# lunarlab-gatech/SLIDE_SLAM

Hardware: AMD Instinct MI355X
Metric: pose-graph updates/sec + ms/Gauss-Newton iter, 8-robot 10k-landmark graph (higher is better)
Workload: dtype f64

## Files before the change

### slide_slam_amd/csrc/capi.hip

```cpp
#include <unistd.h>
#include <algorithm>
#include <cmath>
#include <cstring>
#include <memory>
#include <utility>
#include <vector>

#include "delaunay.hpp"
#include "host_backend.hpp"

using namespace sl;

struct slide_graph {
  HostGraph g;
  explicit slide_graph(const slide_params_t& p) : g(p) {}
};
struct slide_backend {
  HostBackend b;
  slide_graph_t* gview = nullptr;
  explicit slide_backend(const slide_params_t& p) : b(p) {}
};

static thread_local std::string t_err;

// ... 351 lines not shown
  return g->g.dist_pass_local(d_buf);
}

int slide_dense_spd_solve(const double* A, int n, const double* b, double* x, int repeats, double* ms_out) {
  return slide_dense_spd_solve_ex(A, n, b, x, repeats, ms_out, 0);
}
int slide_dense_spd_solve_ex(const double* A, int n, const double* b, double* x, int repeats, double* ms_out, int method) {
  if (slide_device_check(-1) != SLIDE_OK) return SLIDE_ERR_HIP;
  if (n <= 0 || repeats < 1 || method < 0 || method > 2) return SLIDE_ERR_INVALID;
  const int T = (n + NB - 1) / NB;
  const size_t ld = (size_t)(T + 1) * NB, ncol = (size_t)T * NB;
  std::vector<double> S(ld * ncol, 0.0);
  for (int j = 0; j < n; ++j)
    for (int i = j; i < n; ++i) S[(size_t)j * ld + i] = A[(size_t)j * n + i];
  for (size_t i = n; i < ncol; ++i) S[i * ld + i] = 1.0;
  for (int j = 0; j < n; ++j) S[(size_t)j * ld + ncol] = b[j];
  Tmp Tm;
  double* dS0 = Tm.up(S.data(), S.size());
  double* dS = Tm.up<double>(nullptr, S.size());
  double* dW = Tm.up<double>(nullptr, (size_t)T * NB * NB);
  double* dWi = Tm.up<double>(nullptr, (size_t)T * 1024);
  double* dy = Tm.up<double>(nullptr, ncol);
  double* dx = Tm.up<double>(nullptr, ncol);
  int* dst = Tm.up<int>(nullptr, 8);
  int* dctr = Tm.up<int>(nullptr, (size_t)T + 2);
  int* dtick = Tm.up<int>(nullptr, CHOL_STEP_BATCH_MAX);
  if (!dS0 || !dS || !dW || !dWi || !dy || !dx || !dst || !dctr || !dtick) { g_last_error = "hipMalloc/hipMemcpy failed"; return SLIDE_ERR_HIP; }
  SL_HIP(hipMemset(dtick, 0, CHOL_STEP_BATCH_MAX * sizeof(int)));
  SL_HIP(hipMemset(dst, 0, 8 * sizeof(int)));
  SL_HIP(hipMemset(dctr, 0, ((size_t)T + 2) * sizeof(int)));
  hipEvent_t e0, e1;
  SL_HIP(hipEventCreate(&e0));
  SL_HIP(hipEventCreate(&e1));
  float total = 0.f;
  CholSystem cs{};
  cs.S = dS; cs.ld = (int)ld; cs.T = T; cs.Ld = dW; cs.Winv = dWi; cs.yv = dy; cs.dp = dx; cs.status = dst;
  CholLLPlan* plan = method == 1 ? chol_ll_plan_create(&cs, 1) : nullptr;
  if (method == 1 && !plan) { g_last_error = "hipMalloc failed (left-looking plan)"; return SLIDE_ERR_HIP; }
  for (int r = 0; r < repeats; ++r) {
    SL_HIP(hipMemcpyAsync(dS, dS0, S.size() * sizeof(double), hipMemcpyDeviceToDevice, nullptr));
    SL_HIP(hipEventRecord(e0, nullptr));
    if (plan) {
      int* trace = nullptr;
      const int nt = chol_ll_plan_tasks(plan);
      static const bool want_trace = getenv("SLIDE_LL_TRACE") && getenv("SLIDE_LL_TRACE")[0] == '1';
      if (want_trace && hipHostMalloc(reinterpret_cast<void**>(&trace), (size_t)nt * 16 * sizeof(int), hipHostMallocMapped) == hipSuccess)
        memset(trace, 0, (size_t)nt * 16 * sizeof(int));
      launch_chol_ll(plan, &cs, 1, nullptr, trace);
      if (trace) {
        hipEvent_t done;
        SL_HIP(hipEventCreate(&done));
        SL_HIP(hipEventRecord(done, nullptr));
        int waited = 0;
        while (hipEventQuery(done) == hipErrorNotReady && waited < 8000) { usleep(1000); ++waited; }
        if (hipEventQuery(done) == hipErrorNotReady) {
          fprintf(stderr, "k_chol_ll still running after %d ms; tasks (ticket: stage kind k row | barrier-1 waves, barrier-2 waves):\n", waited);
          for (int t = 0; t < nt; ++t)
            if (trace[16 * t] != 5) fprintf(stderr, "  %4d: stage %d kind %d k %d row %d | %03x %03x\n", t, trace[16 * t], trace[16 * t + 1], trace[16 * t + 2], trace[16 * t + 3], trace[16 * t + 4], trace[16 * t + 5]);
          fflush(stderr);
          _exit(3);
        }
        (void)hipEventDestroy(done);
        if (const char* path = getenv("SLIDE_LL_TRACE_FILE")) {
          if (FILE* f = fopen(path, "wb")) { fwrite(trace, sizeof(int), (size_t)nt * 16, f); fclose(f); }
        }
        (void)hipHostFree(trace);
      }
      launch_chol_bwd_all(dS, (int)ld, T, dW, dWi, dy, dx, dst, nullptr, nullptr);
    } else if (method == 2) {
      launch_chol_batch(&cs, 1, dctr, nullptr, nullptr, false, 100, dtick);
      launch_chol_bwd_all(dS, (int)ld, T, dW, dWi, dy, dx, dst, nullptr, nullptr);
    } else {
      chol_factor_solve(dS, (int)ld, T, dW, dWi, dy, dx, dst, dctr, nullptr);
    }
    SL_HIP(hipEventRecord(e1, nullptr));
    SL_HIP(hipEventSynchronize(e1));
    float ms = 0.f;
    SL_HIP(hipEventElapsedTime(&ms, e0, e1));
    total += ms;
  }
  if (plan) { (void)hipDeviceSynchronize(); chol_ll_plan_destroy(plan); }
  SL_HIP(hipGetLastError());
  (void)hipEventDestroy(e0);
  (void)hipEventDestroy(e1);
  int st[8];
  SL_HIP(hipMemcpy(st, dst, sizeof(st), hipMemcpyDeviceToHost));
  std::vector<double> xs(ncol);
  SL_HIP(hipMemcpy(xs.data(), dx, ncol * sizeof(double), hipMemcpyDeviceToHost));
  for (int i = 0; i < n; ++i) x[i] = xs[i];
  if (ms_out) *ms_out = total;
  if (st[1] & 1) { g_last_error = "matrix not positive definite"; return SLIDE_ERR_NOT_SPD; }
  st[0] = 0;
  return decode_status(st);
}

int slide_debug_chol_bordered(const double* S_in, int ld, int T, int nbr, const int* prof, const int* bfirst, const int* ord, int b0, int kofs,
                              int n_copies, int method, double* S_out, double* Ld_out, double* Winv_out, int* status_out, double* max_copy_diff) {
  if (slide_device_check(-1) != SLIDE_OK) return SLIDE_ERR_HIP;
  if (!S_in || T < 1 || nbr < 0 || n_copies < 1 || n_copies > CHOL_STEP_BATCH_MAX || (method != 0 && method != 2)) return SLIDE_ERR_INVALID;
  const int B0 = b0 > 0 ? b0 : T;
  if (ld < (B0 + nbr + 1) * NB) return SLIDE_ERR_INVALID;
  const size_t len = (size_t)ld * T * NB;
  Tmp Tm;
  std::vector<CholSystem> sys(n_copies);
  std::vector<double*> dS(n_copies);
  int* d_ord = ord ? Tm.up(ord, (size_t)nbr) : nullptr;
  int* d_ctr = Tm.up<int>(nullptr, (size_t)T + 3);
  if ((ord && !d_ord) || !d_ctr) { g_last_error = "hipMalloc/hipMemcpy failed"; return SLIDE_ERR_HIP; }
  SL_HIP(hipMemset(d_ctr, 0, ((size_t)T + 3) * sizeof(int)));
  for (int c = 0; c < n_copies; ++c) {
    dS[c] = Tm.up(S_in, len);
    CholSystem cs{};
    cs.S = dS[c]; cs.ld = ld; cs.T = T;
    cs.Ld = Tm.up<double>(nullptr, (size_t)T * NB * NB); cs.Winv = Tm.up<double>(nullptr, (size_t)T * 1024);
    cs.yv = Tm.up<double>(nullptr, (size_t)T * NB); cs.dp = Tm.up<double>(nullptr, (size_t)T * NB);
    cs.status = Tm.up<int>(nullptr, 8);
    if (!cs.S || !cs.Ld || !cs.Winv || !cs.yv || !cs.dp || !cs.status) { g_last_error = "hipMalloc/hipMemcpy failed"; return SLIDE_ERR_HIP; }
    SL_HIP(hipMemset(cs.status, 0, 8 * sizeof(int)));
    SL_HIP(hipMemset(cs.Ld, 0, (size_t)T * NB * NB * sizeof(double)));
    cs.h_prof = prof; cs.nbr = nbr; cs.h_bfirst = bfirst; cs.b0 = b0; cs.kofs = kofs; cs.ord = d_ord;
    sys[c] = cs;
  }
  int* d_tick = Tm.up<int>(nullptr, CHOL_STEP_BATCH_MAX);
  if (!d_tick) { g_last_error = "hipMalloc failed"; return SLIDE_ERR_HIP; }
  SL_HIP(hipMemset(d_tick, 0, CHOL_STEP_BATCH_MAX * sizeof(int)));
  launch_chol_batch(sys.data(), n_copies, d_ctr, nullptr, nullptr, false, 100, method == 2 ? d_tick : nullptr);
  if (method == 2) {
    int tk[CHOL_STEP_BATCH_MAX];
    SL_HIP(hipMemcpy(tk, d_tick, sizeof(tk), hipMemcpyDeviceToHost));
    for (int c = 0; c < CHOL_STEP_BATCH_MAX; ++c)
      if (tk[c] != 0) { g_last_error = "pair kernel: a ticket counter was left at " + std::to_string(tk[c]); return SLIDE_ERR_HIP; }
  }
  SL_HIP(hipDeviceSynchronize());
  SL_HIP(hipGetLastError());
  std::vector<double> ref(len), other;
  SL_HIP(hipMemcpy(ref.data(), dS[0], len * sizeof(double), hipMemcpyDeviceToHost));
  double worst = 0.0;
  for (int c = 1; c < n_copies; ++c) {
    other.resize(len);
    SL_HIP(hipMemcpy(other.data(), dS[c], len * sizeof(double), hipMemcpyDeviceToHost));
    for (size_t i = 0; i < len; ++i) {
      const double d = std::fabs(other[i] - ref[i]);
      if (!(d <= worst)) worst = std::isnan(d) ? (std::isnan(ref[i]) && std::isnan(other[i]) ? worst : INFINITY) : d;
    }
  }
  if (S_out) std::memcpy(S_out, ref.data(), len * sizeof(double));
  if (Ld_out) SL_HIP(hipMemcpy(Ld_out, sys[0].Ld, (size_t)T * NB * NB * sizeof(double), hipMemcpyDeviceToHost));
  if (Winv_out) SL_HIP(hipMemcpy(Winv_out, sys[0].Winv, (size_t)T * 1024 * sizeof(double), hipMemcpyDeviceToHost));
  if (status_out) SL_HIP(hipMemcpy(status_out, sys[0].status, 8 * sizeof(int), hipMemcpyDeviceToHost));
  if (max_copy_diff) *max_copy_diff = worst;
  return SLIDE_OK;
}


static int run_single_class(int cls_kind , int n_cur, const double* det_world, int det_stride,
                            const int32_t* label, int n_map, const float* cloud, const double* model, const int32_t* mlabel,
                            const double* qpos, int K, double thresh, double best_init, int label_gate, int32_t* out_sub,
                            int32_t* out_submap, int* out_k) {
  if (slide_device_check(-1) != SLIDE_OK) return SLIDE_ERR_HIP;
  const bool gate = cloud != nullptr;
  if (!gate && n_cur == 0) return SLIDE_OK;
  Tmp T;
  std::vector<double> det((size_t)std::max(n_cur, 0) * (cls_kind == 0 ? 7 : 12), 0.0);
  for (int i = 0; i < n_cur; ++i) {
    if (cls_kind == 0) std::memcpy(&det[7 * (size_t)i], det_world + (size_t)det_stride * i, 7 * sizeof(double));
    else {
      double* o = &det[12 * (size_t)i];
      o[0] = o[4] = o[8] = 1.0;
      o[9] = det_world[(size_t)det_stride * i]; o[10] = det_world[(size_t)det_stride * i + 1]; o[11] = det_world[(size_t)det_stride * i + 2];
    }
  }
  double pose12[12] = {1, 0, 0, 0, 1, 0, 0, 0, 1, 0, 0, 0};
  if (gate) { pose12[9] = qpos[0]; pose12[10] = qpos[1]; pose12[11] = qpos[2]; }
  AssocFrameDev F[3];
  std::memset(F, 0, sizeof(F));
  AssocFrameDev& C = F[0];
  size_t lds = 0;
  if (!assoc_plan(n_map, K, gate ? 1 : 0, cls_kind == 0 ? 7 : 3, &C.Kp, &C.cached, &C.staged, &lds)) {
    g_last_error = "K-NN gate: K exceeds the on-chip sort buffer (16384 neighbours)";
    return SLIDE_ERR_CAPACITY;
  }
  C.gate = gate ? 1 : 0;
  if (gate) {
    std::vector<float> soa(3 * (size_t)std::max(n_map, 1));
    for (int i = 0; i < n_map; ++i) { soa[i] = cloud[3 * (size_t)i]; soa[(size_t)n_map + i] = cloud[3 * (size_t)i + 1]; soa[2 * (size_t)n_map + i] = cloud[3 * (size_t)i + 2]; }
    const float* d = T.up(soa.data(), soa.size());
    if (!d) { g_last_error = "hipMalloc/hipMemcpy failed"; return SLIDE_ERR_HIP; }
    C.cx = d; C.cy = d + n_map; C.cz = d + 2 * (size_t)n_map;
  }
  C.model = T.up(model, (size_t)(cls_kind == 0 ? 7 : 3) * n_map);
  C.label = T.up(mlabel, n_map);
  C.n = n_map; C.K = K; C.thresh = thresh; C.best_init = best_init; C.label_gate = label_gate; C.is_cyl = cls_kind == 0;
  C.det = T.up(det.data(), det.size());
  C.det_label = T.up(label, n_cur);
  C.n_det = n_cur;
  C.det_world = T.up<double>(nullptr, det.size());
  C.match_sub = T.up<int32_t>(nullptr, n_cur);
  C.match_map = T.up<int32_t>(nullptr, n_cur);
  C.submap = gate ? T.up<int32_t>(nullptr, std::max(std::min(K, n_map), 1)) : nullptr;
  int32_t* nsub = T.up<int32_t>(nullptr, 4);
  C.n_sub = nsub;
  F[1] = C; F[1].n_det = 0; F[1].n = 0; F[1].n_sub = nsub + 1; F[1].submap = nullptr;
  F[2] = C; F[2].n_det = 0; F[2].n = 0; F[2].n_sub = nsub + 2; F[2].submap = nullptr;
  AssocFrameDev* dF = T.up(F, 3);
  double* dpose = T.up(pose12, 12);
  if (!C.model || !C.label || !C.det || !C.det_label || !C.det_world || !C.match_sub || !C.match_map || (gate && !C.submap) ||
      !nsub || !dF || !dpose) {
    g_last_error = "hipMalloc/hipMemcpy failed";
    return SLIDE_ERR_HIP;
  }
  launch_assoc_frame(dF, lds, dpose, nullptr);
  SL_HIP(hipDeviceSynchronize());
  SL_HIP(hipGetLastError());
  int k = 0;
  SL_HIP(hipMemcpy(&k, nsub, sizeof(int), hipMemcpyDeviceToHost));
  if (out_k) *out_k = k;
  if (out_submap && k && gate) SL_HIP(hipMemcpy(out_submap, C.submap, k * sizeof(int32_t), hipMemcpyDeviceToHost));
  if (out_sub && n_cur) SL_HIP(hipMemcpy(out_sub, C.match_sub, n_cur * sizeof(int32_t), hipMemcpyDeviceToHost));
  return SLIDE_OK;
}

int slide_submap_knn(const float* cloud_xyz, uint64_t n, const double query_xyz[3], int K, int32_t* out_idx, int* out_k) {
  if (n > (uint64_t)INT32_MAX || (n > 0 && !cloud_xyz)) return SLIDE_ERR_INVALID;
  if (n == 0) {
    if (slide_device_check(-1) != SLIDE_OK) return SLIDE_ERR_HIP;
    if (out_k) *out_k = 0;
    return SLIDE_OK;
  }
  std::vector<double> model(3 * (size_t)std::max<uint64_t>(n, 1), 0.0);
  std::vector<int32_t> lab(std::max<uint64_t>(n, 1), 0);
  return run_single_class(2, 0, nullptr, 3, nullptr, (int)n, cloud_xyz, model.data(), lab.data(), query_xyz, K, 0.0, 1000.0, 1,
                          nullptr, out_idx, out_k);
}

int slide_assoc_match_cylinders(int n_cur, const double* root, const double* ray, const int32_t* label, int n_map,
                                const double* map_root, const double* map_ray, const int32_t* map_label, double thresh,
                                int32_t* out_idx) {
  std::vector<double> det(7 * (size_t)n_cur), model(7 * (size_t)n_map);
  for (int i = 0; i < n_cur; ++i) { for (int k = 0; k < 3; ++k) { det[7 * i + k] = root[3 * i + k]; det[7 * i + 3 + k] = ray[3 * i + k]; } det[7 * i + 6] = 0; }
  for (int i = 0; i < n_map; ++i) { for (int k = 0; k < 3; ++k) { model[7 * i + k] = map_root[3 * i + k]; model[7 * i + 3 + k] = map_ray[3 * i + k]; } model[7 * i + 6] = 0; }
  const double q[3] = {0, 0, 0};
  return run_single_class(0, n_cur, det.data(), 7, label, n_map, nullptr, model.data(), map_label, q, std::max(n_map, 1), thresh,
                          thresh + 100, 2, out_idx, nullptr, nullptr);
}
int slide_assoc_match_boxes(int cls, int n_cur, const double* xyz, const int32_t* label, int n_map, const double* map_xyz,
                            const int32_t* map_label, double thresh, int32_t* out_idx) {
  if (cls != SLIDE_CLS_CUBE && cls != SLIDE_CLS_ELLIPSOID) return SLIDE_ERR_INVALID;
  const double q[3] = {0, 0, 0};
  const bool cube = cls == SLIDE_CLS_CUBE;
  return run_single_class(cube ? 1 : 2, n_cur, xyz, 3, label, n_map, nullptr, map_xyz, map_label, q, std::max(n_map, 1), thresh,
                          cube ? 30.0 : 1000.0, cube ? 0 : 1, out_idx, nullptr, nullptr);
}

int slide_assoc_sweep_batch_device(const float* d_cloud_x, const float* d_cloud_y, const float* d_cloud_z, const double* d_model_xyz,
                                   const int32_t* d_label, int n_map, const double* d_query_pos, const double* d_obs_xyz,
                                   const int32_t* d_obs_label, int n_query, int n_obs, int K, double thresh, int32_t* d_out_map_idx,
                                   void* stream) {
  if (n_query <= 0) return SLIDE_OK;
  if (n_map < 0 || n_obs < 0 || K <= 0) return SLIDE_ERR_INVALID;
  if (launch_assoc_sweep(d_cloud_x, d_cloud_y, d_cloud_z, d_model_xyz, d_label, n_map, d_query_pos, d_obs_xyz, d_obs_label, n_query,
                         n_obs, K, thresh, d_out_map_idx, (hipStream_t)stream) != 0) {
    g_last_error = "K-NN gate: K exceeds the on-chip sort buffer (16384 neighbours)";
    return SLIDE_ERR_CAPACITY;
  }
  SL_HIP(hipGetLastError());
  return SLIDE_OK;
}

int slide_assoc_sweep_batch(const float* cloud_xyz, const double* model_xyz, const int32_t* label, int n_map, const double* query_pos,
                            const double* obs_xyz, const int32_t* obs_label, int n_query, int n_obs, int K, double thresh,
                            int32_t* out_map_idx, int repeats, double* ms_out) {
  if (slide_device_check(-1) != SLIDE_OK) return SLIDE_ERR_HIP;
  if (n_map < 0 || n_obs < 0 || n_query < 0 || K <= 0) return SLIDE_ERR_INVALID;
  if (ms_out) *ms_out = 0.0;
  if (n_query == 0) return SLIDE_OK;
  Tmp T;
  std::vector<float> soa(3 * (size_t)std::max(n_map, 1));
  for (int i = 0; i < n_map; ++i) { soa[i] = cloud_xyz[3 * (size_t)i]; soa[(size_t)n_map + i] = cloud_xyz[3 * (size_t)i + 1]; soa[2 * (size_t)n_map + i] = cloud_xyz[3 * (size_t)i + 2]; }
  const float* dc = T.up(soa.data(), soa.size());
  const double* dm = T.up(model_xyz, 3 * (size_t)std::max(n_map, 1));
  const int32_t* dl = T.up(label, (size_t)std::max(n_map, 1));
  const double* dq = T.up(query_pos, 3 * (size_t)n_query);
  const double* dox = T.up(obs_xyz, 3 * (size_t)n_query * std::max(n_obs, 1));
  const int32_t* dol = T.up(obs_label, (size_t)n_query * std::max(n_obs, 1));
  int32_t* dout = T.up<int32_t>(nullptr, (size_t)n_query * std::max(n_obs, 1));
  if (!dc || !dm || !dl || !dq || !dox || !dol || !dout) { g_last_error = "hipMalloc/hipMemcpy failed"; return SLIDE_ERR_HIP; }
  hipEvent_t e0, e1;
  SL_HIP(hipEventCreate(&e0));
  SL_HIP(hipEventCreate(&e1));
  int rc = slide_assoc_sweep_batch_device(dc, dc + n_map, dc + 2 * (size_t)n_map, dm, dl, n_map, dq, dox, dol, n_query, n_obs, K, thresh, dout, nullptr);
  if (rc == SLIDE_OK) {
    SL_HIP(hipEventRecord(e0, nullptr));
    for (int r = 0; r < std::max(repeats, 1) && rc == SLIDE_OK; ++r)
      rc = slide_assoc_sweep_batch_device(dc, dc + n_map, dc + 2 * (size_t)n_map, dm, dl, n_map, dq, dox, dol, n_query, n_obs, K, thresh, dout, nullptr);
    SL_HIP(hipEventRecord(e1, nullptr));
    SL_HIP(hipEventSynchronize(e1));
    float ms = 0.f;
    SL_HIP(hipEventElapsedTime(&ms, e0, e1));
    if (ms_out) *ms_out = ms;
  }
  (void)hipEventDestroy(e0);
  (void)hipEventDestroy(e1);
  if (rc != SLIDE_OK) return rc;
  SL_HIP(hipGetLastError());
  if (n_obs) SL_HIP(hipMemcpy(out_map_idx, dout, (size_t)n_query * n_obs * sizeof(int32_t), hipMemcpyDeviceToHost));
  return SLIDE_OK;
// ... 1421 lines not shown
```

### slide_slam_amd/csrc/chol_kernels.hip

```cpp
#include <hip/hip_runtime.h>
#include <stdlib.h>
#include <algorithm>
#include <type_traits>
#include <utility>
#include <vector>

#include "graph_dev.hpp"
#include "kernels.hpp"

namespace sl {

typedef double v4d __attribute__((ext_vector_type(4)));
constexpr int CHOL_BATCH_MAX = 8;
__device__ inline v4d mfma_f64(double a, double b, v4d c) { return __builtin_amdgcn_mfma_f64_16x16x4f64(a, b, c, 0, 0, 0); }

__device__ inline double rsqrt_nr(double d) {
#ifdef SLIDE_RSQRT_OLD
  double y = __builtin_amdgcn_rsq(d);
  y = y * (1.5 - 0.5 * d * y * y);
  y = y * (1.5 - 0.5 * d * y * y);
  return y;
#else
  double y = __builtin_amdgcn_rsq(d);
  double t = d * y, h = 0.5 * y;
// ... 205 lines not shown
      double mop = 0.0;
      mop = s00 ? i0 : mop;  mop = s11 ? i1 : mop;  mop = s10 ? m10 : mop;  mop = s22 ? i2 : mop;  mop = s21 ? m21 : mop;
      mop = s20 ? m20 : mop; mop = s33 ? i3 : mop;  mop = s32 ? m32 : mop;  mop = s31 ? m31 : mop;  mop = s30 ? m30 : mop;
      L.mop[n][lane] = mop;
      const double xd = mfma_f64(mop, Dt[s], zero)[0];
      Dt[s] = xd;
      const double xm = (lr > 4 * s + 3) ? xd : 0.0;
      L.xm[n][lane] = xm;
      lds_post(&L.it_done, n + 1, lane);
      if (n < 4) STAMPW(32 + n);
      if (s < 3) Dt = mfma_f64(-xm, xm, Dt);
      if (s == 3 && JQ < 3) {
        STAMPW(3 + 2 * JQ + 1);
        lds_wait(&L.d_ready[JQ + 1], 1);
        STAMPW(3 + 2 * JQ + 2);
        const double x3 = mfma_f64(mop, L.Dh3[JQ][lane], zero)[0];
#pragma unroll
        for (int r = 0; r < 4; ++r) Dnext[r] = L.Dh[JQ][r][lane];
        Dnext = mfma_f64(-x3, x3, Dnext);
      }
    }
  }
  STAMPW(10);
  if (!ok && lane == 0 && ia == 0) atomicOr(&status[1], 1);
}

template <int W, int NPAN>
__device__ __forceinline__ void a_worker_wave(int ia, double* __restrict__ Ld, double* __restrict__ Winv, ALds& L, int lane,
                                              v4d (&R)[W + 1]) {
  const int lr = lane & 15, lk = lane >> 4;
  const v4d zero = v4d{0.0, 0.0, 0.0, 0.0};
  if (NPAN > 0) {
    v4d e[W + 1];
#pragma unroll
    for (int J = 0; J <= W; ++J) e[J] = zero;
#pragma unroll
    for (int ks = 0; ks < 16 * NPAN; ks += 2) {
      const double w0 = L.Pk[4 * ks + lk][16 * W + lr], w1 = L.Pk[4 * ks + 4 + lk][16 * W + lr];
#pragma unroll
      for (int J = 0; J <= W; ++J) {
        R[J] = mfma_f64(-L.Pk[4 * ks + lk][16 * J + lr], w0, R[J]);
        e[J] = mfma_f64(-L.Pk[4 * ks + 4 + lk][16 * J + lr], w1, e[J]);
      }
    }
#pragma unroll
    for (int J = 0; J <= W; ++J) {
      R[J] += e[J];
      pin(R[J]);
    }
  }
  if (W == 1) STAMPW(37);
  v4d Wt = zero;
#pragma unroll
  for (int JQ = 0; JQ < W; ++JQ) {
    if (W == WT) {
#pragma unroll
      for (int r = 0; r < 4; ++r) Wt[r] = (lr == lk + 4 * r) ? 1.0 : 0.0;
    }
#pragma unroll
    for (int s = 0; s < 4; ++s) {
      const int n = 4 * JQ + s;
      lds_wait(&L.it_done, n + 1);
      if (W == 1 && n == 3) STAMPW(11);
      if (W == 1 && n < 3) STAMPW(16 + n);
      if (W == 2 && n < 12) STAMPW(20 + n);
      const double mop = L.mop[n][lane], xm = L.xm[n][lane];
      const double x = mfma_f64(mop, R[JQ][s], zero)[0];
      double xw = 0.0;
      if (W == WT) xw = mfma_f64(mop, Wt[s], zero)[0];
      R[JQ][s] = x;
      if (W == WT) Wt[s] = xw;
      if (s < 3) {
        R[JQ] = mfma_f64(-xm, x, R[JQ]);
        if (W == WT) Wt = mfma_f64(-xm, xw, Wt);
      }
      R[W] = mfma_f64(-R[JQ][s], R[JQ][s], R[W]);
#pragma unroll
      for (int J = 0; J <= W; ++J) pin(R[J]);
      if (W == WT) pin(Wt);
      if (JQ == W - 1 && s == 2) {
#pragma unroll
        for (int r = 0; r < 4; ++r) L.Dh[W - 1][r][lane] = R[W][r];
        L.Dh3[W - 1][lane] = R[JQ][3];
        lds_post(&L.d_ready[W], 1, lane);
        if (W == 1) STAMPW(13);
        if (W == 2) STAMPW(36);
      }
    }
#pragma unroll
    for (int r = 0; r < 4; ++r) {
      L.Lt[oidx(W, JQ)][r][lane] = R[JQ][r];
      if (ia == 0) Ld[(size_t)(16 * JQ + lk + 4 * r) * NB + 16 * W + lr] = R[JQ][r];
    }
    lds_post(&L.col_done[W], JQ + 1, lane);
    if (W == 1) STAMPW(12);
#pragma unroll
    for (int J = JQ + 1; J < W; ++J) {
      lds_wait(&L.col_done[J], JQ + 1);
#pragma unroll
      for (int ks = 0; ks < 4; ++ks) R[J] = mfma_f64(-L.Lt[oidx(J, JQ)][ks][lane], R[JQ][ks], R[J]);
    }
    if (W == WT) {
#pragma unroll
      for (int r = 0; r < 4; ++r) {
        const double v = (lk + 4 * r >= lr) ? Wt[r] : 0.0;
        L.Wi[JQ][lr * 16 + lk + 4 * r] = v;
        if (ia == 0) Winv[(size_t)JQ * 256 + lr * 16 + lk + 4 * r] = v;
      }
      lds_post(&L.w_done, JQ + 1, lane);
    }
  }
  static_assert(W >= 1 && W <= 3, "worker index");
  if (W == WT) {
#pragma unroll
    for (int JQ = WT; JQ < 4; ++JQ) {
#pragma unroll
      for (int r = 0; r < 4; ++r) Wt[r] = (lr == lk + 4 * r) ? 1.0 : 0.0;
#pragma unroll
      for (int s = 0; s < 4; ++s) {
        const int n = 4 * JQ + s;
        lds_wait(&L.it_done, n + 1);
        const double mop = L.mop[n][lane], xm = L.xm[n][lane];
        const double xw = mfma_f64(mop, Wt[s], zero)[0];
        Wt[s] = xw;
        if (s < 3) Wt = mfma_f64(-xm, xw, Wt);
      }
#pragma unroll
      for (int r = 0; r < 4; ++r) {
        const double v = (lk + 4 * r >= lr) ? Wt[r] : 0.0;
        L.Wi[JQ][lr * 16 + lk + 4 * r] = v;
        if (ia == 0) Winv[(size_t)JQ * 256 + lr * 16 + lk + 4 * r] = v;
      }
      lds_post(&L.w_done, JQ + 1, lane);
    }
  }
}

template <int NPAN>
__device__ __forceinline__ void panel_load(const double* __restrict__ S, int ld, int k, int it, int q, int lr, int lk,
                                           v4d (&Tq)[4], double (&tb)[16]) {
  const double* tcol = S + (size_t)(k * NB) * ld + (size_t)it * NB + 16 * q + lr;
#pragma unroll
  for (int b = 0; b < 4; ++b)
#pragma unroll
    for (int r = 0; r < 4; ++r) Tq[b][r] = tcol[(size_t)(16 * b + lk + 4 * r) * ld];
  if (NPAN > 0) {
    const double* pi = S + (size_t)((k - NPAN) * NB) * ld + (size_t)it * NB + 16 * q + lr;
#pragma unroll
    for (int ks = 0; ks < 16 * NPAN; ++ks) tb[ks] = pi[(size_t)(4 * ks + lk) * ld];
  }
}
template <int NPAN, bool EARLY>
__device__ __forceinline__ void panel_rows(double* __restrict__ S, int ld, int k, int it, int q, int gate, int lane, ALds& L, v4d (&Tq)[4],
                                           const double (&tb)[16], float* __restrict__ L32t) {
  const int lr = lane & 15, lk = lane >> 4;
  double* tcol = S + (size_t)(k * NB) * ld + (size_t)it * NB + 16 * q + lr;
  float* pcol = L32t ? L32t + lk * NB + 16 * q + lr : nullptr;
  v4d xt[4], t[4];
#define PANEL_YIELD() do { __builtin_amdgcn_sched_barrier(0); __builtin_amdgcn_s_sleep(1); __builtin_amdgcn_sched_barrier(0); } while (0)
#pragma unroll
  for (int b = 0; b < 4; ++b) {
    if (b == 0) {
      if (NPAN > 0 && EARLY) {
        if (gate == 1) lds_wait(&L.d_ready[1], 1);
        if (gate == 2) lds_wait(&L.d_ready[2], 1);
#pragma unroll
        for (int ks = 0; ks < 16 * NPAN; ++ks) {
#pragma unroll
          for (int bb = 0; bb < 4; ++bb) Tq[bb] = mfma_f64(-L.Pk[4 * ks + lk][16 * bb + lr], tb[ks], Tq[bb]);
        }
#pragma unroll
        for (int bb = 0; bb < 4; ++bb) pin(Tq[bb]);
      }
      lds_wait(&L.it_done, 4);
      if (NPAN > 0 && !EARLY) {
#pragma unroll
        for (int ks = 0; ks < 16 * NPAN; ++ks) {
          Tq[0] = mfma_f64(-L.Pk[4 * ks + lk][lr], tb[ks], Tq[0]);
          if ((ks & 3) == 3) PANEL_YIELD();
        }
      }
      t[0] = Tq[0];
    }
    lds_wait(&L.w_done, b + 1);
    v4d x = v4d{0.0, 0.0, 0.0, 0.0};
#pragma unroll
    for (int s4 = 0; s4 < 4; ++s4) x = mfma_f64(L.Wi[b][(4 * s4 + lk) * 16 + lr], t[b][s4], x);
    xt[b] = x;
#pragma unroll
    for (int r = 0; r < 4; ++r) tcol[(size_t)(16 * b + lk + 4 * r) * ld] = x[r];
    if (pcol) {
#pragma unroll
      for (int r = 0; r < 4; ++r) pcol[(16 * b + 4 * r) * NB] = (float)x[r];
    }
    if (b < 3) {
      PANEL_YIELD();
      if (NPAN > 0 && !EARLY) {
#pragma unroll
        for (int ks = 0; ks < 16 * NPAN; ++ks) {
          Tq[b + 1] = mfma_f64(-L.Pk[4 * ks + lk][16 * (b + 1) + lr], tb[ks], Tq[b + 1]);
          if ((ks & 3) == 3) PANEL_YIELD();
        }
      }
      lds_wait(&L.col_done[b + 1], b + 1);
      v4d tn = Tq[b + 1];
#pragma unroll
      for (int c = 0; c <= b; ++c) {
#pragma unroll
        for (int s4 = 0; s4 < 4; ++s4) tn = mfma_f64(-L.Lt[oidx(b + 1, c)][s4][lane], xt[c][s4], tn);
        if (b < 2 || c < b) PANEL_YIELD();
      }
      t[b + 1] = tn;
      pin(t[b + 1]);
    }
  }
#undef PANEL_YIELD
}

template <int NPAN>
__device__ __forceinline__ void step_type_a_impl(double* __restrict__ S, int ld, int k, int ia, int it, int half, double* __restrict__ Ld,
                                                 double* __restrict__ Winv, int* status, ALds& L, float* __restrict__ L32t) {
  const int tid = threadIdx.x, lane = tid & 63;
  const int wave = __builtin_amdgcn_readfirstlane(tid >> 6);
  const int lr = lane & 15, lk = lane >> 4;
  STAMP(0);
  if (NPAN > 0) {
    constexpr int NC = 8 * (NPAN > 0 ? NPAN : 1);
    const double* pq = S + (size_t)((k - NPAN) * NB + NC * wave) * ld + (size_t)k * NB + lane;
    double stage[NC];
#pragma unroll
    for (int c = 0; c < NC; ++c) stage[c] = pq[(size_t)c * ld];
#pragma unroll
    for (int c = 0; c < NC; ++c) L.Pk[NC * wave + c][lane] = stage[c];
  }
  if (tid == 0) L.it_done = 0;
  if (tid < 4) { L.col_done[tid] = 0; L.d_ready[tid] = 0; }
  if (tid == 4) L.w_done = 0;
  if (wave == 1) STAMPW(38);
  if (wave < 4) {
    const double* dcol = S + (size_t)(k * NB) * ld + (size_t)k * NB + 16 * wave + lr;
    v4d R[4];
#pragma unroll
    for (int J = 0; J < 4; ++J)
#pragma unroll
      for (int r = 0; r < 4; ++r) R[J][r] = (J <= wave) ? dcol[(size_t)(16 * J + lk + 4 * r) * ld] : 0.0;
    v4d Tq[4];
    double tb[16];
    if (wave == 1 && half < 0) panel_load<NPAN>(S, ld, k, it, 0, lr, lk, Tq, tb);
    __syncthreads();
    if (wave == 1) STAMPW(39);
    if (wave == 0) __builtin_amdgcn_s_setprio(3); else __builtin_amdgcn_s_setprio(2);
    if (wave == 0) {
      a_chain_wave<NPAN>(ia, status, L, lane, R[0]);
    } else if (wave == 1) {
      v4d R1[2] = {R[0], R[1]};
      a_worker_wave<1, NPAN>(ia, Ld, Winv, L, lane, R1);
      if (half < 0) panel_rows<NPAN, false>(S, ld, k, it, 0, 0, lane, L, Tq, tb, L32t);
    } else if (wave == 2) {
      v4d R2[3] = {R[0], R[1], R[2]};
      a_worker_wave<2, NPAN>(ia, Ld, Winv, L, lane, R2);
    } else {
      a_worker_wave<3, NPAN>(ia, Ld, Winv, L, lane, R);
    }
    __builtin_amdgcn_s_setprio(0);
    __syncthreads();
    STAMP(1);
    STAMP(2);
  } else {
    const int q = half < 0 ? wave - 4 : (wave == 5 ? 2 * half : (wave == 6 ? 2 * half + 1 : -1));
    const bool rows = half < 0 ? q > 0 : q >= 0;
    v4d Tq[4];
    double tb[16];
    if (rows) panel_load<NPAN>(S, ld, k, it, q, lr, lk, Tq, tb);
    __syncthreads();
    if (rows) panel_rows<NPAN, true>(S, ld, k, it, q, wave - 4, lane, L, Tq, tb, L32t);
    STAMPW(14);
    __syncthreads();
    STAMP(1);
    STAMP(2);
  }
}
__device__ __forceinline__ void step_type_a(double* __restrict__ S, int ld, int k, int T, int TvA, int ia, int half, double* __restrict__ Ld,
                                            double* __restrict__ Winv, int* status, ALds& L, float* __restrict__ L32, int nbr, int nbA,
                                            const int* __restrict__ ord = nullptr) {
  const int vi = k + 1 + ia - TvA;
  const int it = vi < 0 ? k + 1 + ia : (vi < nbA ? T + (ord ? ord[vi] : vi) : T + nbr);
  float* L32t = (L32 && it < T) ? L32 + ((size_t)k * (T - 1) - (size_t)k * (k - 1) / 2 + (it - k - 1)) * (NB * NB) : nullptr;
  if (k > 0) step_type_a_impl<1>(S, ld, k, ia, it, half, Ld, Winv, status, L, L32t);
  else step_type_a_impl<0>(S, ld, k, ia, it, half, Ld, Winv, status, L, L32t);
}

__global__ __launch_bounds__(512) void k_chol_step(double* __restrict__ S, int ld, int k, int T, double* __restrict__ Ld,
                                                   double* __restrict__ Winv, int* status, int* __restrict__ ctr, int kb, int nP,
                                                   int g0, int g1, int nX, int a_joins, int a_split, float* __restrict__ L32,
                                                   int TvA, int TvB, int TvX, int nbr, int nbA, int nbB, int nbX) {
  __shared__ ALds L;
  __shared__ int s_g;
  const int nA = (TvA - k + nbA) << a_split;
  if (blockIdx.x == 0 && threadIdx.x == 0) ctr[k + 1] = 0;
  if ((int)blockIdx.x < nA) {
    step_type_a(S, ld, k, T, TvA, (int)blockIdx.x >> a_split, a_split ? (int)(blockIdx.x & 1) : -1, Ld, Winv, status, L, L32, nbr, nbA);
    if (!a_joins) return;
  }
  const int nR = g1 - g0, nItems = nR + nX;
  if (nItems <= 0) return;
  const long long nG = (long long)nP * (nP + 1) / 2;
  const int wave = __builtin_amdgcn_readfirstlane(threadIdx.x >> 6);
  for (;;) {
    __syncthreads();
    if (threadIdx.x == 0) s_g = atomicAdd(&ctr[k], 1);
    __syncthreads();
    const int g = __builtin_amdgcn_readfirstlane(s_g);
    if (g >= nItems) break;
    const BItem it = b_decode(g, nItems, nR, g0, k, kb, T, TvB, TvX, nP, nG, wave, nbr, nbB, nbX);
    if (!it.ok) continue;
    if (it.ks == 32) b_quadrant<32>(S, ld, it, wave & 3);
    else b_quadrant<16>(S, ld, it, wave & 3);
  }
}

struct CholBatchArgs {
  int n;
  double* S[CHOL_STEP_BATCH_MAX]; int ld[CHOL_STEP_BATCH_MAX]; int T[CHOL_STEP_BATCH_MAX];
  double* Ld[CHOL_STEP_BATCH_MAX]; double* Winv[CHOL_STEP_BATCH_MAX]; int* status[CHOL_STEP_BATCH_MAX];
  float* L32[CHOL_STEP_BATCH_MAX];
  int TvA[CHOL_STEP_BATCH_MAX], TvB[CHOL_STEP_BATCH_MAX], TvX[CHOL_STEP_BATCH_MAX];
  int nP[CHOL_STEP_BATCH_MAX], g0[CHOL_STEP_BATCH_MAX], g1[CHOL_STEP_BATCH_MAX], nX[CHOL_STEP_BATCH_MAX], a_split[CHOL_STEP_BATCH_MAX];
  int nbr[CHOL_STEP_BATCH_MAX];
  int nbA[CHOL_STEP_BATCH_MAX], nbB[CHOL_STEP_BATCH_MAX], nbX[CHOL_STEP_BATCH_MAX];
  int B0[CHOL_STEP_BATCH_MAX];
  const int* ord[CHOL_STEP_BATCH_MAX];
  int a_base[CHOL_STEP_BATCH_MAX + 1];
  int b_base[CHOL_STEP_BATCH_MAX + 1];
};
__device__ __forceinline__ int xcd_logical(int orig, int nwg) {
  const int q = nwg >> 3, r = nwg & 7, xcd = orig & 7;
  return (xcd < r ? xcd * (q + 1) : r * (q + 1) + (xcd - r) * q) + (orig >> 3);
}
__global__ __launch_bounds__(512) void k_chol_step_batched(CholBatchArgs A, int k, int kb, int* __restrict__ ctr, int a_joins, int xcd_map) {
  __shared__ ALds L;
  __shared__ int s_g;
  if (blockIdx.x == 0 && threadIdx.x == 0) ctr[k + 1] = 0;
  int bid = (int)blockIdx.x;
  if (xcd_map && bid < A.a_base[A.n]) bid = xcd_logical(bid, A.a_base[A.n]);
  if (bid < A.a_base[A.n]) {
    int r = 0;
    while (bid >= A.a_base[r + 1]) ++r;
    const int local = bid - A.a_base[r], sp = A.a_split[r];
    step_type_a(A.S[r], A.ld[r], k, A.B0[r], A.TvA[r], local >> sp, sp ? (local & 1) : -1, A.Ld[r] + (size_t)k * NB * NB,
                A.Winv[r] + (size_t)k * 1024, A.status[r], L, A.L32[r], A.nbr[r], A.nbA[r], A.ord[r]);
    if (!a_joins) return;
  }
  const int nItems = A.b_base[A.n];
  if (nItems <= 0) return;
  const int wave = __builtin_amdgcn_readfirstlane(threadIdx.x >> 6);
  for (;;) {
    __syncthreads();
    if (threadIdx.x == 0) s_g = atomicAdd(&ctr[k], 1);
    __syncthreads();
    const int g = __builtin_amdgcn_readfirstlane(s_g);
    if (g >= nItems) break;
    int r = 0;
    while (g >= A.b_base[r + 1]) ++r;
    const int gl = g - A.b_base[r], nR = A.g1[r] - A.g0[r];
    const long long nG = (long long)A.nP[r] * (A.nP[r] + 1) / 2;
    const BItem it = b_decode(gl, nR + A.nX[r], nR, A.g0[r], k, kb, A.B0[r], A.TvB[r], A.TvX[r], A.nP[r], nG, wave, A.nbr[r], A.nbB[r], A.nbX[r], A.ord[r]);
    if (!it.ok) continue;
    if (it.ks == 32) b_quadrant<32>(A.S[r], A.ld[r], it, wave & 3);
    else b_quadrant<16>(A.S[r], A.ld[r], it, wave & 3);
  }
}


constexpr int PAIR_THREADS = 768;
struct PLds {
  double Pk[2 * NB][PSTR];
  double Xs[16][4][64];
  double mop[16][64];
  double xm[16][64];
  double Lt[6][4][64];
  double Dh[3][4][64];
  double Dh3[3][64];
  double Wi[4][256];
  int it_done;
  int col_done[4];
  int d_ready[4];
  int w_done;
  int pend_done;
  int p1_done;
  int xs_done[4];
  int d2_ready[4];
  int sub_loaded;
  int store_flag;
};
__device__ int g_pair_timeouts;
__device__ __forceinline__ void lds_wait_p(int* f, int v) {
  const unsigned off = (unsigned)(size_t)f;
  int cur;
  for (int spin = 0; spin < (1 << 21); ++spin) {
    asm volatile("ds_read_b32 %0, %1\n\ts_waitcnt lgkmcnt(0)" : "=v"(cur) : "v"(off) : "memory");
    if (__builtin_amdgcn_readfirstlane(cur) >= v) return;
    __builtin_amdgcn_s_sleep(1);
  }
  if ((threadIdx.x & 63) == 0) atomicAdd(&g_pair_timeouts, 1);
}
__device__ __forceinline__ void lds_add1(int* f, int lane) {
  const unsigned off = (unsigned)(size_t)f;
  const int one = 1;
  __atomic_signal_fence(__ATOMIC_SEQ_CST);
  if (lane == 0) asm volatile("ds_add_u32 %0, %1" : : "v"(off), "v"(one) : "memory");
  __atomic_signal_fence(__ATOMIC_SEQ_CST);
}
__device__ __forceinline__ constexpr int didx(int I, int J) { return I * (I + 1) / 2 + J; }
typedef double (*D2Ptr)[4][64];
__device__ __forceinline__ double ldu(const double* ubase, unsigned boff) {
  asm("" : "+s"(ubase));
  return *reinterpret_cast<const double*>(reinterpret_cast<const char*>(ubase) + boff);
}
__device__ __forceinline__ void stu(double* ubase, unsigned boff, double v) {
  asm("" : "+s"(ubase));
  *reinterpret_cast<double*>(reinterpret_cast<char*>(ubase) + boff) = v;
}
__device__ __forceinline__ D2Ptr pair_d2(PLds& L) { return reinterpret_cast<D2Ptr>(&L.Pk[0][0]); }

template <int NPAN, int PH>
__device__ __forceinline__ void p_chain_wave(bool report, int* status, PLds& L, int lane, v4d Dt) {
  const int lr = lane & 15, lk = lane >> 4;
  const v4d zero = v4d{0.0, 0.0, 0.0, 0.0};
  const bool s00 = lr == 0 && lk == 0, s10 = lr == 1 && lk == 0, s11 = lr == 1 && lk == 1, s20 = lr == 2 && lk == 0,
             s21 = lr == 2 && lk == 1, s22 = lr == 2 && lk == 2, s30 = lr == 3 && lk == 0, s31 = lr == 3 && lk == 1,
             s32 = lr == 3 && lk == 2, s33 = lr == 3 && lk == 3;
  if (NPAN > 0) {
    v4d d1 = zero, d2 = zero, d3 = zero;
#pragma unroll
    for (int ks = 0; ks < 4 * NPAN; ++ks) {
      const double q0 = L.Pk[4 * ks + lk][lr], q1 = L.Pk[16 * NPAN + 4 * ks + lk][lr], q2 = L.Pk[32 * NPAN + 4 * ks + lk][lr],
                   q3 = L.Pk[48 * NPAN + 4 * ks + lk][lr];
      Dt = mfma_f64(-q0, q0, Dt);
      d1 = mfma_f64(-q1, q1, d1);
      d2 = mfma_f64(-q2, q2, d2);
      d3 = mfma_f64(-q3, q3, d3);
    }
    Dt = (Dt + d1) + (d2 + d3);
  }
  if (PH == 0) lds_add1(&L.pend_done, lane);
  bool ok = true;
  v4d Dnext = zero;
#pragma unroll
  for (int JQ = 0; JQ < 4; ++JQ) {
    if (JQ > 0) Dt = Dnext;
#pragma unroll
    for (int r = 0; r < 4; ++r)
      if (lr < lk + 4 * r) Dt[r] = 0.0;
#pragma unroll
    for (int s = 0; s < 4; ++s) {
      const int n = 4 * JQ + s;
      const double dv = Dt[s];
      const double P00 = bcast_lane(dv, 4 * s), P10 = bcast_lane(dv, 4 * s + 1), P20 = bcast_lane(dv, 4 * s + 2), P30 = bcast_lane(dv, 4 * s + 3);
      const double P11 = bcast_lane(dv, 4 * s + 1 + 16), P21 = bcast_lane(dv, 4 * s + 2 + 16), P31 = bcast_lane(dv, 4 * s + 3 + 16);
      const double P22 = bcast_lane(dv, 4 * s + 2 + 32), P32 = bcast_lane(dv, 4 * s + 3 + 32), P33 = bcast_lane(dv, 4 * s + 3 + 48);
      const double i0 = rsqrt_nr(P00);
      const double l10 = P10 * i0, l20 = P20 * i0, l30 = P30 * i0;
      const double d1 = P11 - l10 * l10;
      const double i1 = rsqrt_nr(d1);
      const double l21 = (P21 - l20 * l10) * i1, l31 = (P31 - l30 * l10) * i1;
      const double d2 = P22 - l20 * l20 - l21 * l21;
      const double i2 = rsqrt_nr(d2);
      const double l32 = (P32 - l30 * l20 - l31 * l21) * i2;
      const double d3 = P33 - l30 * l30 - l31 * l31 - l32 * l32;
      const double i3 = rsqrt_nr(d3);
      ok = ok && (P00 > 0.0) && (d1 > 0.0) && (d2 > 0.0) && (d3 > 0.0);
      const double m10 = -l10 * i0 * i1;
      const double m21 = -l21 * i1 * i2;
      const double m20 = -(l20 * i0 + l21 * m10) * i2;
      const double m32 = -l32 * i2 * i3;
      const double m31 = -(l31 * i1 + l32 * m21) * i3;
      const double m30 = -(l30 * i0 + l31 * m10 + l32 * m20) * i3;
      double mop = 0.0;
      mop = s00 ? i0 : mop;  mop = s11 ? i1 : mop;  mop = s10 ? m10 : mop;  mop = s22 ? i2 : mop;  mop = s21 ? m21 : mop;
      mop = s20 ? m20 : mop; mop = s33 ? i3 : mop;  mop = s32 ? m32 : mop;  mop = s31 ? m31 : mop;  mop = s30 ? m30 : mop;
      L.mop[n][lane] = mop;
      const double xd = mfma_f64(mop, Dt[s], zero)[0];
      Dt[s] = xd;
      const double xm = (lr > 4 * s + 3) ? xd : 0.0;
      L.xm[n][lane] = xm;
      lds_post(&L.it_done, 16 * PH + n + 1, lane);
      if (s < 3) Dt = mfma_f64(-xm, xm, Dt);
      if (s == 3 && JQ < 3) {
        lds_wait_p(&L.d_ready[JQ + 1], PH + 1);
        const double x3 = mfma_f64(mop, L.Dh3[JQ][lane], zero)[0];
#pragma unroll
        for (int r = 0; r < 4; ++r) Dnext[r] = L.Dh[JQ][r][lane];
        Dnext = mfma_f64(-x3, x3, Dnext);
      }
    }
  }
  if (!ok && lane == 0 && report) atomicOr(&status[1], 1);
}

template <int W, int NPAN, int PH>
__device__ __forceinline__ void p_worker_wave(bool store, double* __restrict__ Ld, double* __restrict__ Winv, PLds& L, int lane,
                                              v4d (&R)[W + 1], int nread) {
  const int lr = lane & 15, lk = lane >> 4;
// ... 903 lines not shown
      if (wave == 0) {
        ll_wait_cols(fk, nullptr, fr, k - 1, k, ctl, Y.status);
        ll_time(tr, 14);
      }
      __syncthreads();
      constexpr int NC = 8;
      const double* pq = S + (size_t)((k - 1) * NB + NC * wave) * ld + (size_t)k * NB + lane;
      double stage[NC];
#pragma unroll
      for (int c = 0; c < NC; ++c) stage[c] = pq[(size_t)c * ld];
#pragma unroll
      for (int c = 0; c < NC; ++c) L.Pk[NC * wave + c][lane] = stage[c];
    }
    ll_mark_or(tr, 4, 1 << wave);
    __syncthreads();
    if (wave == 0) ll_stage(tr, 3);
    if (wave == 0) __builtin_amdgcn_s_setprio(3); else __builtin_amdgcn_s_setprio(2);
    if (wave == 0) {
      a_chain_wave<NPAN>(ia, Y.status, L, lane, R[0]);
    } else if (wave == 1) {
      v4d R1[2] = {R[0], R[1]};
      ll_worker_wave<1, NPAN>(ia, Ld, Winv, L, lane, R1);
      if (NPAN > 0) {
        if (row_prev) lds_wait(&row_ok, 1);
        const double* pi = S + (size_t)((k - 1) * NB) * ld + (size_t)it * NB + lr;
#pragma unroll
        for (int ks = 0; ks < 16; ++ks) tb[ks] = row_prev ? pi[(size_t)(4 * ks + lk) * ld] : 0.0;
      }
      ll_panel_rows<NPAN, false>(S, ld, k, it, 0, 0, lane, L, Tq, tb, nullptr);
    } else if (wave == 2) {
      v4d R2[3] = {R[0], R[1], R[2]};
      ll_worker_wave<2, NPAN>(ia, Ld, Winv, L, lane, R2);
    } else {
      ll_worker_wave<3, NPAN>(ia, Ld, Winv, L, lane, R);
    }
    __builtin_amdgcn_s_setprio(0);
    __builtin_amdgcn_fence(__ATOMIC_RELEASE, "agent");
    ll_mark_or(tr, 5, 1 << wave);
    __syncthreads();
    if (wave == 0) ll_stage(tr, 4);
  } else {
    const int q = wave - 4;
    const bool rows = q > 0;
    v4d Tq[4];
    double tb[16];
    if (rows) ll_rows_load(S, ld, k, it, q, lr, lk, Tq);
    if (tk.clo_d < kold) {
      v4d Rdummy[4];
      __syncthreads();
      ll_chain_presum(S, ld, k, it, tk.clo_d, tk.clo0, kold, L, wave, lane, false, 0, rows, q, Rdummy, Tq);
    }
    if (NPAN > 0) {
      __syncthreads();
      constexpr int NC = 8;
      const double* pq = S + (size_t)((k - 1) * NB + NC * wave) * ld + (size_t)k * NB + lane;
      double stage[NC];
#pragma unroll
      for (int c = 0; c < NC; ++c) stage[c] = pq[(size_t)c * ld];
#pragma unroll
      for (int c = 0; c < NC; ++c) L.Pk[NC * wave + c][lane] = stage[c];
    }
    ll_mark_or(tr, 4, 1 << wave);
    __syncthreads();
    if (NPAN > 0 && row_prev && wave == 4) {
      ll_wait_cols(fi, nullptr, fr, k - 1, k, ctl, Y.status);
      lds_post(&row_ok, 1, lane);
    }
    if (NPAN > 0 && rows) {
      if (row_prev) lds_wait(&row_ok, 1);
      const double* pi = S + (size_t)((k - 1) * NB) * ld + (size_t)it * NB + 16 * q + lr;
#pragma unroll
      for (int ks = 0; ks < 16; ++ks) tb[ks] = row_prev ? pi[(size_t)(4 * ks + lk) * ld] : 0.0;
    }
    if (rows) ll_panel_rows<NPAN, true>(S, ld, k, it, q, wave - 4, lane, L, Tq, tb, nullptr);
    __builtin_amdgcn_fence(__ATOMIC_RELEASE, "agent");
    ll_mark_or(tr, 5, 1 << wave);
    __syncthreads();
  }
  if (tid == 0) {
    if (ia == 0) __hip_atomic_store(Y.flags + (size_t)k * fr + k, 1, __ATOMIC_RELAXED, __HIP_MEMORY_SCOPE_AGENT);
    __hip_atomic_store(Y.flags + (size_t)k * fr + it, 1, __ATOMIC_RELAXED, __HIP_MEMORY_SCOPE_AGENT);
  }
  if (wave == 0) ll_stage(tr, 5);
}

__global__ __launch_bounds__(512) void k_chol_ll(const LLSys* __restrict__ sysv, const LLTask* __restrict__ tasks, int n_tasks, int* ctl, int* trace) {
  __shared__ ALds L;
  __shared__ int s_t, s_row_ok;
  if (threadIdx.x == 0) s_t = atomicAdd(&ctl[0], 1);
  __syncthreads();
  const int t = __builtin_amdgcn_readfirstlane(s_t);
  if (t >= n_tasks) return;
  const LLTask tk = tasks[t];
  const LLSys Y = sysv[tk.sys];
  int* tr = trace ? trace + 16 * (size_t)t : nullptr;
  if (tr && threadIdx.x == 0) { ll_mark(tr, 1, tk.kind); ll_mark(tr, 2, tk.k); ll_mark(tr, 3, tk.it0); ll_stage(tr, 1); }
  if (tk.kind != 1) {
    if (tk.clo_d <= tk.k - 1) ll_chain_task<1>(Y, tk, L, s_row_ok, ctl, tr);
    else ll_chain_task<0>(Y, tk, L, s_row_ok, ctl, tr);
  } else {
    ll_tile_task(Y, tk, L, ctl, tr);
  }
}

extern "C" int slide_debug_pair_timeouts() {
  int v = -1;
  if (hipMemcpyFromSymbol(&v, HIP_SYMBOL(g_pair_timeouts), sizeof(int)) != hipSuccess) return -1;
  return v;
}
#ifdef SLIDE_STAMPS
extern "C" void slide_debug_stamps(unsigned long long* out) { (void)hipMemcpyFromSymbol(out, HIP_SYMBOL(g_stamps), sizeof(g_stamps)); }
extern "C" void slide_debug_chain_stamps(unsigned long long* out) { (void)hipMemcpyFromSymbol(out, HIP_SYMBOL(g_chain_stamps), sizeof(g_chain_stamps)); }
#endif

constexpr unsigned long long BWD_SENT = CHAIN_SENTINEL;

__global__ void k_chol_extract_y(const double* __restrict__ S, int ld, int T, int Tr, double* __restrict__ yv, double* __restrict__ dp, int* status,
                                 double* __restrict__ prev) {
  const int c = blockIdx.x * blockDim.x + threadIdx.x;
  if (c == 0) status[4] = 0;
  if (c < T * NB) {
    yv[c] = S[(size_t)c * ld + (size_t)Tr * NB];
    if (prev) prev[c] = dp[c];
    dp[c] = __longlong_as_double((long long)BWD_SENT);
  }
}

struct ExtractArgs { int n; const double* S[CHOL_STEP_BATCH_MAX]; int ld[CHOL_STEP_BATCH_MAX]; int T[CHOL_STEP_BATCH_MAX]; int Tr[CHOL_STEP_BATCH_MAX]; double* yv[CHOL_STEP_BATCH_MAX]; double* dp[CHOL_STEP_BATCH_MAX]; int* status[CHOL_STEP_BATCH_MAX]; };
__global__ void k_chol_extract_y_b(ExtractArgs A) {
  const int r = blockIdx.y;
  const int c = blockIdx.x * blockDim.x + threadIdx.x;
  if (c == 0) A.status[r][4] = 0;
  if (c < A.T[r] * NB) {
    A.yv[r][c] = A.S[r][(size_t)c * A.ld[r] + (size_t)A.Tr[r] * NB];
    A.dp[r][c] = __longlong_as_double((long long)BWD_SENT);
  }
}

constexpr int CHAIN_THREADS = 320;
struct alignas(16) ChainLds {
  alignas(16) double xs[2][NB];
  alignas(16) double ys[NB];
  alignas(16) double red[4][NB];
  alignas(16) double Lo[6][256];
  alignas(16) double Ws[4][256];
  alignas(16) double tmp[3][256];
  alignas(16) double Ms[NB][NB + 1];
};
template <bool F32, bool WFIRE = false>
__device__ __forceinline__ void bwd_chain_body(ChainLds& W, const double* __restrict__ S, int ld, int T, const double* __restrict__ Ld,
                                               const double* __restrict__ Winv, const double* __restrict__ yv, double* dp, int* status, int bidx,
                                               const float* __restrict__ L32, const int* __restrict__ prof,
                                               const double* __restrict__ wf_prev = nullptr, double wf_thr = 0.0, int wf_Tprev = 0,
                                               int* wf_lds = nullptr, int wf_lim = 0) {
  int dummy_state = 0;
  int& wf_state = WFIRE ? *wf_lds : dummy_state;
  auto& Ms = W.Ms; auto& Lo = W.Lo; auto& Ws = W.Ws; auto& tmp = W.tmp; auto& xs = W.xs; auto& ys = W.ys;
  const int tid = threadIdx.x;
  const bool worker = tid < 256;
  CSTAMP(0);
  const int c = T - 1 - bidx;
  if (WFIRE) {
    if (tid == 0) wf_state = 0;
    __syncthreads();
  }
  const int col = tid >> 2, part = tid & 3;
  const int jtop = prof ? prof[c] : T - 1;
  const int nj = jtop - c;
  constexpr int RB = F32 ? 6 : 3;
  typedef typename std::conditional<F32, float, double>::type tile_t;
  tile_t tr[RB][16];
  const double* tcol = S + (size_t)(c * NB + col) * ld + 16 * part;
  const float* pcol = F32 ? L32 + ((size_t)c * (T - 1) - (size_t)c * (c - 1) / 2) * (NB * NB) + col * NB + 16 * part : nullptr;
  auto tile_load = [&](tile_t (&dst)[16], int q) {
    if (F32) {
      const float4* tp = reinterpret_cast<const float4*>(pcol + (size_t)(nj - 1 - q) * (NB * NB));
#pragma unroll
      for (int r = 0; r < 4; ++r) {
        const float4 v = tp[r];
        dst[4 * r] = v.x; dst[4 * r + 1] = v.y; dst[4 * r + 2] = v.z; dst[4 * r + 3] = v.w;
      }
    } else {
      const double* tp = tcol + (size_t)(jtop - q) * NB;
#pragma unroll
      for (int r = 0; r < 16; ++r) dst[r] = tp[r];
    }
  };
  double y0 = 0.0;
  if (worker) {
#pragma unroll
    for (int q = 0; q < RB; ++q)
      if (q < nj) tile_load(tr[q], q);
    y0 = yv[c * NB + col];
  }
  if (worker) {
    const double* Ldk = Ld + (size_t)c * NB * NB;
    const double* Wk = Winv + (size_t)c * 1024;
#pragma unroll
    for (int b = 1; b < 4; ++b)
#pragma unroll
      for (int a = 0; a < b; ++a) Lo[b * (b - 1) / 2 + a][tid] = Ldk[(size_t)(16 * a + (tid >> 4)) * NB + 16 * b + (tid & 15)];
#pragma unroll
    for (int b = 0; b < 4; ++b) Ws[b][tid] = Wk[(size_t)b * 256 + tid];
  }
  __syncthreads();
  {
    const int r = tid & 15, cc = (tid >> 4) & 15;
    if (worker) {
#pragma unroll
      for (int b = 0; b < 4; ++b) Ms[16 * b + r][16 * b + cc] = Ws[b][cc * 16 + r];
    }
    __syncthreads();
#pragma unroll
    for (int d = 1; d < 4; ++d) {
#pragma unroll
      for (int a = 0; a + d < 4; ++a) {
        const int b = a + d;
        double t = 0.0;
#pragma unroll
        for (int m = a; m < b; ++m)
#pragma unroll
          for (int n = 0; n < 16; ++n) t += Lo[b * (b - 1) / 2 + m][n * 16 + r] * Ms[16 * m + n][16 * a + cc];
        if (worker) tmp[a][cc * 16 + r] = t;
      }
      __syncthreads();
#pragma unroll
      for (int a = 0; a + d < 4; ++a) {
        const int b = a + d;
        double v = 0.0;
#pragma unroll
        for (int n = 0; n < 16; ++n) v += Ws[b][n * 16 + r] * tmp[a][cc * 16 + n];
        if (worker) Ms[16 * b + r][16 * a + cc] = -v;
      }
      __syncthreads();
    }
  }
  double mreg[16];
#pragma unroll
  for (int r = 0; r < 16; ++r) mreg[r] = (worker && 16 * part + r >= col) ? Ms[16 * part + r][col] : 0.0;
  double acc = 0.0;
  bool wf_quiet = WFIRE && nj > 0 && c < wf_lim;
  bool wf_leave = false;
  CSTAMP(1);
  for (int q0 = 0; q0 < nj && !wf_leave; q0 += RB) {
#pragma unroll
    for (int qq = 0; qq < RB; ++qq) {
      const int q = q0 + qq;
      if (q < nj && !wf_leave) {
        const int j = jtop - q;
        if (q == nj - 1) CSTAMPP(2);
        if (!worker) {
          const int lane = tid - 256;
          double v;
          int spins = 0;
          bool stopped = false;
          for (;;) {
            v = __hip_atomic_load(dp + (size_t)j * NB + lane, __ATOMIC_RELAXED, __HIP_MEMORY_SCOPE_AGENT);
            if ((unsigned long long)__double_as_longlong(v) != BWD_SENT) break;
            if (WFIRE && (spins & 3) == 3 && __hip_atomic_load(status + 7, __ATOMIC_RELAXED, __HIP_MEMORY_SCOPE_AGENT) > c) { stopped = true; break; }
            if (++spins > (1 << 21)) {
              v = __builtin_nan("");
              atomicOr(&status[1], 2);
              break;
            }
            __builtin_amdgcn_s_sleep(1);
          }
          if (WFIRE) {
            stopped = __any(stopped);
            if (stopped) {
              if (lane == 0) wf_state = 1;
            } else {
              double dv = fabs(v - ((j < wf_Tprev) ? wf_prev[(size_t)j * NB + lane] : 1e300));
#pragma unroll
              for (int m = 32; m >= 1; m >>= 1) dv = fmax(dv, __shfl_xor(dv, m));
              wf_quiet = wf_quiet && (dv < wf_thr);
              if (q == nj - 1 && wf_quiet && lane == 0) wf_state = 2;
            }
          }
          xs[q & 1][lane] = v;
          if (q == nj - 1) CSTAMPP(3);
          if (q == nj - 2) CSTAMPP(7);
        }
        __syncthreads();
        if (WFIRE && wf_state == 1) { wf_leave = true; continue; }
        if (worker) {
#pragma unroll
          for (int r = 0; r < 16; ++r) acc += (double)tr[qq][r] * xs[q & 1][16 * part + r];
          if (q + RB < nj) tile_load(tr[qq], q + RB);
        }
      }
    }
  }
  CSTAMP(4);
  if (WFIRE && wf_state != 0) {
    if (tid < NB) __hip_atomic_store(dp + (size_t)c * NB + tid, wf_prev[(size_t)c * NB + tid], __ATOMIC_RELAXED, __HIP_MEMORY_SCOPE_AGENT);
    if (tid == 0) {
      if (wf_state == 2) atomicMax(status + 7, c);
      atomicAdd(status + 3, 1);
    }
    return;
  }
  acc += __shfl_xor(acc, 1);
  acc += __shfl_xor(acc, 2);
  if (worker && part == 0) ys[col] = y0 - acc;
  __syncthreads();
  CSTAMP(5);
  double x = 0.0;
#pragma unroll
  for (int r = 0; r < 16; ++r) x += mreg[r] * ys[16 * part + r];
  x += __shfl_xor(x, 1);
  x += __shfl_xor(x, 2);
  if (worker && part == 0) __hip_atomic_store(dp + (size_t)c * NB + col, x, __ATOMIC_RELAXED, __HIP_MEMORY_SCOPE_AGENT);
  CSTAMP(6);
}
__device__ __forceinline__ int bwd_ticket(int* ctr) {
  __shared__ int s_t;
  if (threadIdx.x == 0) s_t = atomicAdd(ctr, 1);
  __syncthreads();
  const int t = s_t;
  __syncthreads();
  return t;
}
__global__ __launch_bounds__(CHAIN_THREADS) void k_chol_bwd_chain(const double* __restrict__ S, int ld, int T, const double* __restrict__ Ld,
                                                        const double* __restrict__ Winv, const double* __restrict__ yv, double* dp, int* status,
                                                        const int* __restrict__ prof) {
  __shared__ ChainLds W;
  const int t = bwd_ticket(&status[4]);
  if (t >= T) return;
  bwd_chain_body<false>(W, S, ld, T, Ld, Winv, yv, dp, status, t, nullptr, prof);
}
__global__ __launch_bounds__(CHAIN_THREADS) void k_chol_bwd_chain_wf(const double* __restrict__ S, int ld, int T, const double* __restrict__ Ld,
                                                           const double* __restrict__ Winv, const double* __restrict__ yv, double* dp, int* status,
                                                           const int* __restrict__ prof, const double* __restrict__ prev, double thr, int Tprev, int lim) {
  __shared__ ChainLds W;
  __shared__ int s_wf;
  const int t = bwd_ticket(&status[4]);
  if (t >= T) return;
  bwd_chain_body<false, true>(W, S, ld, T, Ld, Winv, yv, dp, status, t, nullptr, prof, prev, thr, Tprev, &s_wf, lim);
}
constexpr int BWD_BATCH_MAX = 32;
struct BwdBatchArgs {
  int n;
  const double* S[BWD_BATCH_MAX]; int ld[BWD_BATCH_MAX]; int T[BWD_BATCH_MAX];
  const double* Ld[BWD_BATCH_MAX]; const double* Winv[BWD_BATCH_MAX]; const double* yv[BWD_BATCH_MAX]; double* dp[BWD_BATCH_MAX];
  int* status[BWD_BATCH_MAX];
  const int* prof[BWD_BATCH_MAX];
  int base[BWD_BATCH_MAX + 1];
  int Tmax;
};
__global__ __launch_bounds__(CHAIN_THREADS) void k_chol_bwd_chain_batched(BwdBatchArgs A) {
  __shared__ ChainLds W;
  for (;;) {
    const int t = bwd_ticket(&A.status[0][4]);
    if (t >= A.n * A.Tmax) return;
    const int r = t % A.n, b = t / A.n;
    if (b >= A.T[r]) continue;
    bwd_chain_body<false>(W, A.S[r], A.ld[r], A.T[r], A.Ld[r], A.Winv[r], A.yv[r], A.dp[r], A.status[r], b, nullptr, A.prof[r]);
    return;
  }
}


enum { TAB_MF = 0, TAB_MB = 1, TAB_PF = 2, TAB_PB = 3 };
struct ChainTabArgs {
  int n; int T[CHOL_BATCH_MAX]; const double* S[CHOL_BATCH_MAX]; int ld[CHOL_BATCH_MAX];
  const double* Ld[CHOL_BATCH_MAX]; const double* Winv[CHOL_BATCH_MAX]; const int* prof[CHOL_BATCH_MAX]; double* ctab[CHOL_BATCH_MAX];
};
__global__ __launch_bounds__(256) void k_chain_tables(ChainTabArgs A) {
  __shared__ ChainLds W;
  __shared__ double Ts[NB][NB];
  auto& Ms = W.Ms; auto& Lo = W.Lo; auto& Ws = W.Ws; auto& tmp = W.tmp;
  const int sys = blockIdx.y, c = blockIdx.x, tid = threadIdx.x;
  const int T = A.T[sys];
  if (c >= T) return;
  {
    const double* Ldk = A.Ld[sys] + (size_t)c * NB * NB;
    const double* Wk = A.Winv[sys] + (size_t)c * 1024;
#pragma unroll
    for (int b = 1; b < 4; ++b)
#pragma unroll
      for (int a = 0; a < b; ++a) Lo[b * (b - 1) / 2 + a][tid] = Ldk[(size_t)(16 * a + (tid >> 4)) * NB + 16 * b + (tid & 15)];
#pragma unroll
    for (int b = 0; b < 4; ++b) Ws[b][tid] = Wk[(size_t)b * 256 + tid];
  }
  for (int e = tid; e < NB * (NB + 1); e += 256) (&Ms[0][0])[e] = 0.0;
  __syncthreads();
  {
    const int r = tid & 15, cc = tid >> 4;
#pragma unroll
    for (int b = 0; b < 4; ++b) Ms[16 * b + r][16 * b + cc] = Ws[b][cc * 16 + r];
    __syncthreads();
#pragma unroll
    for (int d = 1; d < 4; ++d) {
#pragma unroll
      for (int a = 0; a + d < 4; ++a) {
        const int b = a + d;
        double t = 0.0;
#pragma unroll
        for (int m = a; m < b; ++m)
#pragma unroll
          for (int n = 0; n < 16; ++n) t += Lo[b * (b - 1) / 2 + m][n * 16 + r] * Ms[16 * m + n][16 * a + cc];
        tmp[a][cc * 16 + r] = t;
      }
      __syncthreads();
#pragma unroll
      for (int a = 0; a + d < 4; ++a) {
        const int b = a + d;
        double v = 0.0;
#pragma unroll
        for (int n = 0; n < 16; ++n) v += Ws[b][n * 16 + r] * tmp[a][cc * 16 + n];
        Ms[16 * b + r][16 * a + cc] = -v;
      }
      __syncthreads();
    }
  }
  const int i = tid >> 2, part = tid & 3;
  double* tab = A.ctab[sys] + (size_t)c * (NB * NB) + (size_t)tid * 16;
  const size_t tstride = (size_t)T * (NB * NB);
#pragma unroll
  for (int k = 0; k < 16; ++k) tab[TAB_MF * tstride + k] = Ms[i][16 * part + k];
#pragma unroll
  for (int r = 0; r < 16; ++r) tab[TAB_MB * tstride + r] = Ms[16 * part + r][i];
  const int ld = A.ld[sys];
  const int* prof = A.prof[sys];
  {
    double pf[16];
#pragma unroll
    for (int k = 0; k < 16; ++k) pf[k] = 0.0;
    const bool have = c >= 1 && (prof ? prof[c - 1] >= c : true);
    if (have) {
      const double* tp = A.S[sys] + (size_t)((c - 1) * NB) * ld + (size_t)c * NB;
      for (int e = tid; e < NB * NB; e += 256) Ts[e >> 6][e & 63] = tp[(size_t)(e >> 6) * ld + (e & 63)];
    }
    __syncthreads();
    if (have) {
      for (int m = 0; m <= i; ++m) {
        const double a = Ms[i][m];
#pragma unroll
        for (int k = 0; k < 16; ++k) pf[k] += a * Ts[16 * part + k][m];
      }
    }
#pragma unroll
    for (int k = 0; k < 16; ++k) tab[TAB_PF * tstride + k] = pf[k];
    __syncthreads();
  }
  {
    double pb[16];
#pragma unroll
    for (int r = 0; r < 16; ++r) pb[r] = 0.0;
    const bool have = c + 1 < T && (prof ? prof[c] >= c + 1 : true);
    if (have) {
      const double* tp = A.S[sys] + (size_t)(c * NB) * ld + (size_t)(c + 1) * NB;
      for (int e = tid; e < NB * NB; e += 256) Ts[e >> 6][e & 63] = tp[(size_t)(e >> 6) * ld + (e & 63)];
    }
    __syncthreads();
    if (have) {
      for (int m = i; m < NB; ++m) {
        const double a = Ms[m][i];
#pragma unroll
        for (int r = 0; r < 16; ++r) pb[r] += Ts[m][16 * part + r] * a;
      }
    }
#pragma unroll
    for (int r = 0; r < 16; ++r) tab[TAB_PB * tstride + r] = pb[r];
  }
}

struct alignas(16) TabLds {
  alignas(16) double xs[2][NB];
  alignas(16) double ys[NB];
  alignas(16) double red[4][NB];
};
template <bool FWD, bool F32>
__device__ __forceinline__ void tab_chain_body(TabLds& W, const double* __restrict__ S, int ld, int T, const float* __restrict__ L32,
                                               const double* __restrict__ ctab, const double* __restrict__ rin, double* xout, int* status, int c,
                                               const int* __restrict__ prof, const int* __restrict__ first, double* __restrict__ next_out) {
  auto& xs = W.xs; auto& ys = W.ys; auto& red = W.red;
  const int tid = threadIdx.x;
  const bool worker = tid < 256;
  if (next_out && !worker) next_out[(size_t)c * NB + (tid - 256)] = __longlong_as_double((long long)BWD_SENT);
  const int i = (tid >> 2) & 63, part = tid & 3;
  const int row = tid & 63, cp = (tid >> 6) & 3;
  const int jlo = FWD ? (first ? first[c] : 0) : c + 1;
  const int jhi = FWD ? c - 1 : (prof ? prof[c] : T - 1);
  const int nj = jhi - jlo + 1;
  const bool has_p = nj >= 1;
  const int nloop = has_p ? nj - 1 : 0;
  constexpr int RB = F32 ? 6 : 3;
  typedef typename std::conditional<F32, float, double>::type tile_t;
  tile_t tr[RB][16];
  auto tile_load = [&](tile_t (&dst)[16], int q) {
    const int j = FWD ? jlo + q : jhi - q;
    if (FWD) {
      if (F32) {
        const float* tp = L32 + ((size_t)j * (T - 1) - (size_t)j * (j - 1) / 2 + (c - j - 1)) * (NB * NB) + 16 * cp * NB + row;
#pragma unroll
        for (int r = 0; r < 16; ++r) dst[r] = tp[r * NB];
      } else {
        const double* tp = S + (size_t)(j * NB + 16 * cp) * ld + (size_t)c * NB + row;
#pragma unroll
        for (int r = 0; r < 16; ++r) dst[r] = tp[(size_t)r * ld];
      }
    } else {
      if (F32) {
        const float4* tp = reinterpret_cast<const float4*>(L32 + ((size_t)c * (T - 1) - (size_t)c * (c - 1) / 2 + (j - c - 1)) * (NB * NB) + i * NB + 16 * part);
#pragma unroll
        for (int r = 0; r < 4; ++r) {
          const float4 v = tp[r];
          dst[4 * r] = v.x; dst[4 * r + 1] = v.y; dst[4 * r + 2] = v.z; dst[4 * r + 3] = v.w;
        }
// ... 299 lines not shown
  const double *lpj = pj0, *lpi = pi0;
  v2d pa[RD], pb[RD];
  auto issue = [&](v2d& ra, v2d& rb) {
    while (rem == 0 && sg_next < nseg) {
      int a0 = c0, a1 = c1;
      if (st) {
        const int* sf = st + 1 + nseg + sg_next * (nbr + 1);
        a0 = max(sf[ib], sf[jb]);
        a1 = st[1 + sg_next];
      }
      ++sg_next;
      if (a0 < a1) {
        rem = (a1 - a0) * 16;
        lpj = pj0 + (size_t)a0 * NB * ld;
        lpi = pi0 + (size_t)a0 * NB * ld;
      }
    }
    ra = *(const v2d*)lpj;
    rb = *(const v2d*)lpi;
    lpj += (size_t)4 * ld;
    lpi += (size_t)4 * ld;
    --rem;
    ++issued;
  };
#pragma unroll
  for (int pre = 0; pre < RD - 1; ++pre)
    if (issued < total) issue(pa[pre], pb[pre]);
  v4d acc[2][2];
#pragma unroll
  for (int a = 0; a < 2; ++a)
#pragma unroll
    for (int e = 0; e < 4; ++e) {
      v2d c2;
      c2[0] = 0.0; c2[1] = 0.0;
      if (q == 0) c2 = *(const v2d*)(cin + (size_t)(8 * e + a) * ldin);
      acc[a][0][e] = c2[0]; acc[a][1][e] = c2[1];
    }
  for (int ks0 = 0; ks0 < total; ks0 += RD) {
#pragma unroll
    for (int u = 0; u < RD; ++u) {
      if (issued < total) issue(pa[(u + RD - 1) % RD], pb[(u + RD - 1) % RD]);
      __builtin_amdgcn_sched_barrier(0);
#pragma unroll
      for (int a = 0; a < 2; ++a) {
        const double na = -pa[u][a];
#pragma unroll
        for (int b = 0; b < 2; ++b) acc[a][b] = mfma_f64(na, pb[u][b], acc[a][b]);
      }
      __builtin_amdgcn_sched_barrier(0);
    }
  }
#pragma unroll
  for (int a = 0; a < 2; ++a)
#pragma unroll
    for (int e = 0; e < 4; ++e) {
      v2d c2;
      c2[0] = acc[a][0][e]; c2[1] = acc[a][1][e];
      *(v2d*)(cbh + (size_t)(8 * e + a) * ldb) = c2;
    }
}
__global__ __launch_bounds__(256) void k_border_syrk(SyrkArgs A) { border_syrk_body<16>(A); }
__global__ __launch_bounds__(256) void k_border_syrk_rd8(SyrkArgs A) { border_syrk_body<8>(A); }
__global__ __launch_bounds__(256) void k_border_syrk_rd4(SyrkArgs A) { border_syrk_body<4>(A); }
static void launch_syrk_kernel(dim3 grid, size_t lds, hipStream_t s, const SyrkArgs& A) {
  static const int rd = getenv("SLIDE_SYRK_RD") ? atoi(getenv("SLIDE_SYRK_RD")) : 16;
  if (rd == 4) hipLaunchKernelGGL(k_border_syrk_rd4, grid, dim3(256), lds, s, A);
  else if (rd == 8) hipLaunchKernelGGL(k_border_syrk_rd8, grid, dim3(256), lds, s, A);
  else hipLaunchKernelGGL(k_border_syrk, grid, dim3(256), lds, s, A);
}
__global__ __launch_bounds__(256) void k_border_syrk_reduce(double* __restrict__ bord, int ldb, int nbr, int ks, const double* __restrict__ scratch,
                                                            const int* __restrict__ bfirst, int T) {
  const int ib = blockIdx.x >> 4, jb = blockIdx.y;
  if (ib > nbr || jb >= nbr || ib < jb) return;
  int c0 = 0;
  if (bfirst) c0 = max(bfirst[ib], bfirst[jb]);
  const int len = (T - c0 + ks - 1) / ks;
  const int e = (blockIdx.x & 15) * 256 + threadIdx.x;
  const int col = e / NB, row = e - col * NB;
  double* dst = bord + (size_t)(jb * NB + col) * ldb + (size_t)ib * NB + row;
  double v = *dst;
  for (int q = 1; q < ks; ++q)
    if (c0 + q * len < T) v += scratch[((size_t)(jb * (nbr + 1) + ib) * (ks - 1) + (q - 1)) * (NB * NB) + (size_t)col * NB + row];
  *dst = v;
}
__global__ __launch_bounds__(256) void k_border_syrk_reduce2(double* __restrict__ bordA, int ldbA, const double* __restrict__ bordB, int ldbB, int nbr,
                                                             int ksA, int ksB, const double* __restrict__ scratchA, const double* __restrict__ scratchB,
                                                             int TA, int TB) {
  const int ib = blockIdx.x >> 4, jb = blockIdx.y;
  if (ib > nbr || jb >= nbr || ib < jb) return;
  const int e = (blockIdx.x & 15) * 256 + threadIdx.x;
  const int col = e / NB, row = e - col * NB;
  double* dst = bordA + (size_t)(jb * NB + col) * ldbA + (size_t)ib * NB + row;
  double va = *dst, vb = bordB[(size_t)(jb * NB + col) * ldbB + (size_t)ib * NB + row];
  const int lenA = (TA + ksA - 1) / ksA, lenB = (TB + ksB - 1) / ksB;
  for (int q = 1; q < ksA; ++q)
    if (q * lenA < TA) va += scratchA[((size_t)(jb * (nbr + 1) + ib) * (ksA - 1) + (q - 1)) * (NB * NB) + (size_t)col * NB + row];
  for (int q = 1; q < ksB; ++q)
    if (q * lenB < TB) vb += scratchB[((size_t)(jb * (nbr + 1) + ib) * (ksB - 1) + (q - 1)) * (NB * NB) + (size_t)col * NB + row];
  *dst = va + vb;
}
void launch_border_syrk(const CholSystem* d, int n, hipStream_t s, double* scratch, int ks) {
  SyrkArgs A{};
  A.n = n;
  int nb = 0;
  for (int i = 0; i < n; ++i) {
    A.S[i] = d[i].S; A.ld[i] = d[i].ld; A.T[i] = d[i].T; A.nbr[i] = d[i].nbr; A.bord[i] = d[i].bord; A.ldb[i] = d[i].ldb; A.bfirst[i] = d[i].bfirst; A.bsrc[i] = d[i].bord_src;
    A.segtab[i] = d[i].segtab; A.b0[i] = d[i].b0 > 0 ? d[i].b0 : d[i].T;
    nb = d[i].nbr > nb ? d[i].nbr : nb;
  }
  if (nb <= 0) return;
  if (scratch && n == 1 && ks > 1) {
    A.ks = ks; A.scratch = scratch;
    launch_syrk_kernel(dim3(nb + 1, nb, ks), 0, s, A);
    hipLaunchKernelGGL(k_border_syrk_reduce, dim3(16 * (nb + 1), nb), dim3(256), 0, s, d[0].bord, d[0].ldb, d[0].nbr, ks, scratch, d[0].bfirst, d[0].T);
    return;
  }
  A.ks = 1; A.scratch = nullptr;
  launch_syrk_kernel(dim3(nb + 1, nb, n), 0, s, A);
}
void launch_border_syrk_jobs(const CholSystem* d, int n, const int* jobs, int njobs, int lds_pad, hipStream_t s, double* scratch, int ks, int jb_end,
                             const int* ks_sys, bool fuse_add) {
  SyrkArgs A{};
  A.n = n;
  for (int i = 0; i < n; ++i) {
    A.S[i] = d[i].S; A.ld[i] = d[i].ld; A.T[i] = d[i].T; A.nbr[i] = d[i].nbr; A.bord[i] = d[i].bord; A.ldb[i] = d[i].ldb; A.bfirst[i] = d[i].bfirst; A.bsrc[i] = d[i].bord_src;
    A.segtab[i] = d[i].segtab; A.b0[i] = d[i].b0 > 0 ? d[i].b0 : d[i].T;
  }
  if (njobs <= 0) return;
  A.ks = 1; A.scratch = nullptr; A.jobs = jobs;
  if (scratch && n == 2 && fuse_add && d[0].nbr == d[1].nbr && !d[0].bfirst && !d[1].bfirst) {
    const int nb = d[0].nbr;
    const int ka = std::max(1, ks_sys ? ks_sys[0] : ks), kb = std::max(1, ks_sys ? ks_sys[1] : ks), km = std::max(ka, kb);
    A.ks = km; A.scratch = scratch; A.scratch_stride = std::max<size_t>(1, (size_t)(nb + 1) * nb * (km - 1) * NB * NB);
    A.ks_sys[0] = ka; A.ks_sys[1] = kb;
    launch_syrk_kernel(dim3(njobs, 1, km), lds_pad, s, A);
    hipLaunchKernelGGL(k_border_syrk_reduce2, dim3(16 * (nb + 1), jb_end >= 0 ? jb_end : nb), dim3(256), 0, s, d[0].bord, d[0].ldb, d[1].bord, d[1].ldb, nb,
                       ka, kb, scratch, scratch + A.scratch_stride, d[0].T, d[1].T);
    return;
  }
  if (scratch && n == 1 && ks > 1) {
    A.ks = ks; A.scratch = scratch;
    launch_syrk_kernel(dim3(njobs, 1, ks), lds_pad, s, A);
    const int nb = d[0].nbr;
    hipLaunchKernelGGL(k_border_syrk_reduce, dim3(16 * (nb + 1), jb_end >= 0 ? jb_end : nb), dim3(256), 0, s, d[0].bord, d[0].ldb, nb, ks, scratch, d[0].bfirst, d[0].T);
    return;
  }
  launch_syrk_kernel(dim3(njobs), lds_pad, s, A);
}
struct BorderApplyArgs {
  int n;
  const double* S[CHOL_BATCH_MAX]; int ld[CHOL_BATCH_MAX]; int T[CHOL_BATCH_MAX]; int nbr[CHOL_BATCH_MAX]; int b0[CHOL_BATCH_MAX];
  double* yv[CHOL_BATCH_MAX]; const double* x[CHOL_BATCH_MAX];
  const int* segtab[CHOL_BATCH_MAX];
};
__global__ __launch_bounds__(256) void k_border_apply(BorderApplyArgs A) {
  const int r = blockIdx.z;
  const int col = blockIdx.x * 4 + (threadIdx.x >> 6), lane = threadIdx.x & 63;
  if (col >= A.T[r] * NB) return;
  const int nrow = A.nbr[r] * NB;
  const double* w = A.S[r] + (size_t)col * A.ld[r] + (size_t)A.b0[r] * NB;
  const double* x = A.x[r];
  double acc = 0.0;
  const int* st = A.segtab[r];
  const int* msk = st ? st + 1 + st[0] + st[0] * (A.nbr[r] + 1) : nullptr;
  if (msk && msk[0] > 0) {
    const int c = col / NB;
    unsigned long long m = (unsigned long long)(unsigned)msk[1 + 2 * c] | ((unsigned long long)(unsigned)msk[2 + 2 * c] << 32);
    while (m) {
      const int t = __ffsll((long long)m) - 1;
      m &= m - 1;
      acc += w[t * NB + lane] * x[t * NB + lane];
    }
  } else {
    for (int q = lane; q < nrow; q += 64) acc += w[q] * x[q];
  }
#pragma unroll
  for (int m = 32; m >= 1; m >>= 1) acc += __shfl_xor(acc, m);
  if (lane == 0) A.yv[r][col] -= acc;
}
void launch_border_apply(const CholSystem* d, int n, const double* const* xloc, hipStream_t s) {
  BorderApplyArgs A{};
  A.n = n;
  int Tmax = 0;
  for (int i = 0; i < n; ++i) {
    A.S[i] = d[i].S; A.ld[i] = d[i].ld; A.T[i] = d[i].T; A.nbr[i] = d[i].nbr; A.yv[i] = d[i].yv; A.x[i] = xloc[i];
    A.b0[i] = d[i].b0 > 0 ? d[i].b0 : d[i].T;
    A.segtab[i] = d[i].segtab;
    Tmax = d[i].T > Tmax ? d[i].T : Tmax;
  }
  if (Tmax > 0) hipLaunchKernelGGL(k_border_apply, dim3(Tmax * NB / 4, 1, n), dim3(256), 0, s, A);
}

void launch_chol_bwd_all(const double* S, int ld, int T, const double* Ld, const double* Winv, double* yv, double* dp,
                         int* status, const int* prof, hipStream_t s, const double* wf_prev, double wf_thr, int wf_Tprev, int wf_lim);
void launch_chol_extract_y(const double* S, int ld, int T, double* yv, double* dp, int* status, hipStream_t s, int nbr, int b0, double* prev) {
  hipLaunchKernelGGL(k_chol_extract_y, dim3((T * NB + 255) / 256), dim3(256), 0, s, S, ld, T, (b0 > 0 ? b0 : T) + nbr, yv, dp, status, prev);
}
struct StepPlan { int kb, nP, g0, g1, nX, TvA, TvB, TvX, nbA, nbB, nbX; long long nA, nB; };
static int chol_n_cu() {
  static int n_cu = 0;
  if (!n_cu) {
    int dev = 0;
    hipDeviceProp_t pr;
    if (hipGetDevice(&dev) == hipSuccess && hipGetDeviceProperties(&pr, dev) == hipSuccess) n_cu = pr.multiProcessorCount;
    if (n_cu <= 0) n_cu = 256;
  }
  return n_cu;
}
static StepPlan plan_step(int k, int T, const int* prof, int nbr = 0, const int* bfirst = nullptr, int kofs = 0) {
  static const double frac = getenv("SLIDE_CHOL_FRAC") ? atof(getenv("SLIDE_CHOL_FRAC")) : 0.5;
  StepPlan p{};
  p.kb = k & ~1;
  p.TvA = p.TvB = p.TvX = T;
  if (prof && k < T) {
    p.TvA = prof[k] + 1;
    if (p.kb >= 1) p.TvB = prof[p.kb - 1] + 1;
    if (k >= 1) p.TvX = prof[k - 1] + 1;
  }
  auto active = [&](int upto) { int c = 0; while (c < nbr && (!bfirst || bfirst[c] <= upto + kofs)) ++c; return c; };
  p.nbA = active(k); p.nbB = active(p.kb - 1); p.nbX = active(k - 1);
  p.nA = k < T ? p.TvA - k + p.nbA : 0;
  if (k >= 2 && k < T) {
    p.nP = p.TvB + p.nbB > p.kb ? (p.TvB + p.nbB - p.kb + 1) / 2 : 0;
    long long nG = (long long)p.nP * (p.nP + 1) / 2;
    if (nbr > 0) {
      const int ncol = p.TvB - 1 >= p.kb + 1 ? (p.TvB - 2 - p.kb) / 2 + 1 : 0;
      long long nv = 0;
      for (int bj = 0; bj < ncol && bj < p.nP; ++bj) nv += p.nP - bj;
      nG = nv;
    }
    long long first = (long long)(frac * (double)nG + 0.5);
    if (first < p.nP) first = p.nP;
    if (first > nG) first = nG;
    if (k & 1) { p.g0 = (int)(2 * first); p.g1 = (int)(2 * nG); } else { p.g0 = 0; p.g1 = (int)(2 * first); }
  }
  p.nX = (k & 1) && k + 1 < p.TvX ? (p.TvX + p.nbX - k + 1) / 2 : 0;
  p.nB = p.g1 - p.g0 + p.nX;
  return p;
}
void launch_chol_step(double* S, int ld, int k, int T, double* Ld, double* Winv, int* status, int* ctr, float* L32, const int* h_prof,
                      hipStream_t s, int nbr) {
  const int n_cu = chol_n_cu();
  const StepPlan p = plan_step(k, T, h_prof, nbr, nullptr);
  const long long nA = p.nA, nB = p.nB;
  static const int split_pct = getenv("SLIDE_CHOL_ASPLIT") ? atoi(getenv("SLIDE_CHOL_ASPLIT")) : 100;
  const int a_split = (k > 0 && (2 * nA + nB) * 100 <= (long long)n_cu * split_pct) ? 1 : 0;
  const long long nAw = nA << a_split;
  const long long extra = nB < n_cu ? nB : n_cu;
  const long long free_cu = n_cu - nAw > 8 ? n_cu - nAw : 8;
  static const int join_mul = getenv("SLIDE_CHOL_JOIN") ? atoi(getenv("SLIDE_CHOL_JOIN")) : 1;
  const int a_joins = nB > join_mul * free_cu ? 1 : 0;
  hipLaunchKernelGGL(k_chol_step, dim3((unsigned)(nAw + extra)), dim3(512), 0, s, S, ld, k, T, Ld, Winv, status, ctr, p.kb, p.nP,
                     p.g0, p.g1, p.nX, a_joins, a_split, L32, p.TvA, p.TvB, p.TvX, nbr, p.nbA, p.nbB, p.nbX);
}
struct PairPlan { int ncols, Tv0, Tv1, nb0, nb1, TvB, nbB, nP; long long nA, nB; };
static PairPlan plan_pair(int k, int T, const int* prof, int nbr, const int* bfirst, int kofs) {
  PairPlan p{};
  p.ncols = T - k >= 2 ? 2 : (T - k == 1 ? 1 : 0);
  if (p.ncols == 0) return p;
  auto active = [&](int upto) { int c = 0; while (c < nbr && (!bfirst || bfirst[c] <= upto + kofs)) ++c; return c; };
  p.Tv0 = prof ? prof[k] + 1 : T;
  p.Tv1 = p.ncols == 2 ? (prof ? prof[k + 1] + 1 : T) : p.Tv0;
  p.nb0 = active(k);
  p.nb1 = p.ncols == 2 ? active(k + 1) : p.nb0;
  const int TvL = p.ncols == 2 ? p.Tv1 : p.Tv0, nbL = p.ncols == 2 ? p.nb1 : p.nb0;
  p.nA = (long long)(TvL - (k + p.ncols)) + nbL + 1;
  if (k >= 2) {
    const int kbE = k + 1;
    p.TvB = prof ? prof[k - 1] + 1 : T;
    p.nbB = active(k - 1);
    p.nP = p.TvB + p.nbB > kbE ? (p.TvB + p.nbB - kbE + 1) / 2 : 0;
    long long nG = (long long)p.nP * (p.nP + 1) / 2;
    if (nbr > 0) {
      const int ncol = p.TvB - 1 >= kbE + 1 ? (p.TvB - 2 - kbE) / 2 + 1 : 0;
      long long nv = 0;
      for (int bj = 0; bj < ncol && bj < p.nP; ++bj) nv += p.nP - bj;
      nG = nv;
    }
    p.nB = 2 * nG;
  }
  return p;
}
static void launch_chol_pair_steps(const CholSystem* d, int n, int* ctr, int* tickets, hipStream_t s) {
  const int n_cu = chol_n_cu();
  int Tmax = 0;
  for (int i = 0; i < n; ++i) Tmax = d[i].T > Tmax ? d[i].T : Tmax;
  for (int k = 0; k < Tmax; k += 2) {
    CholPairArgs A{};
    A.n = n;
    A.a_base[0] = A.b_base[0] = 0;
    for (int i = 0; i < n; ++i) {
      const PairPlan p = plan_pair(k, d[i].T, d[i].h_prof, d[i].nbr, d[i].h_bfirst, d[i].kofs);
      A.S[i] = d[i].S; A.ld[i] = d[i].ld; A.Ld[i] = d[i].Ld; A.Winv[i] = d[i].Winv; A.status[i] = d[i].status;
      A.ncols[i] = p.ncols; A.Tv0[i] = p.Tv0; A.Tv1[i] = p.Tv1; A.nb0[i] = p.nb0; A.nb1[i] = p.nb1;
      A.TvB[i] = p.TvB; A.nbB[i] = p.nbB; A.nP[i] = p.nP;
      A.nbr[i] = d[i].nbr; A.B0[i] = d[i].b0 > 0 ? d[i].b0 : d[i].T; A.ord[i] = d[i].ord;
      A.a_base[i + 1] = A.a_base[i] + (int)(2 * p.nA);
      A.b_base[i + 1] = A.b_base[i] + (int)p.nB;
    }
    const long long nAw = A.a_base[n], nB = A.b_base[n];
    if (nAw <= 0) continue;
    const long long extra = nB < n_cu ? nB : n_cu;
    const long long free_cu = n_cu - nAw > 8 ? n_cu - nAw : 8;
    const int a_joins = nB > free_cu ? 1 : 0;
    hipLaunchKernelGGL(k_chol_pair_batched, dim3((unsigned)(nAw + extra)), dim3(PAIR_THREADS), 0, s, A, k, ctr, tickets, a_joins);
  }
}
bool chol_pair_supported(const CholSystem* d, int n) {
  if (n < 1 || n > CHOL_STEP_BATCH_MAX) return false;
  for (int i = 0; i < n; ++i)
    if (d[i].L32) return false;
  return true;
}
void launch_chol_batch(const CholSystem* d, int n, int* ctr, hipStream_t s, hipEvent_t after_steps, bool solve, int cu_share, int* pair_tickets) {
  const bool pair = pair_tickets != nullptr;
  const int n_cu = chol_n_cu();
  int Tmax = 0;
  for (int i = 0; i < n; ++i) Tmax = d[i].T > Tmax ? d[i].T : Tmax;
  static const bool verify = getenv("SLIDE_PAIR_VERIFY") && getenv("SLIDE_PAIR_VERIFY")[0] == '1';
  if (pair && chol_pair_supported(d, n) && verify) {
    (void)hipStreamSynchronize(s);
    std::vector<CholSystem> cp(d, d + n);
    std::vector<size_t> len(n);
    std::vector<void*> tmp;
    auto dmal = [&](size_t bytes) { void* p = nullptr; (void)hipMalloc(&p, bytes); tmp.push_back(p); return p; };
    for (int i = 0; i < n; ++i) {
      const int B0 = d[i].b0 > 0 ? d[i].b0 : d[i].T;
      len[i] = (size_t)d[i].ld * ((size_t)d[i].T * NB - 1) + (size_t)(B0 + d[i].nbr + 1) * NB;
      cp[i].S = (double*)dmal(len[i] * sizeof(double));
      cp[i].Ld = (double*)dmal((size_t)d[i].T * NB * NB * sizeof(double));
      cp[i].Winv = (double*)dmal((size_t)d[i].T * 1024 * sizeof(double));
      cp[i].status = (int*)dmal(8 * sizeof(int));
      cp[i].yv = (double*)dmal((size_t)d[i].T * NB * sizeof(double));
      cp[i].dp = (double*)dmal((size_t)d[i].T * NB * sizeof(double));
      (void)hipMemset(cp[i].status, 0, 8 * sizeof(int));
      (void)hipMemcpy(cp[i].S, d[i].S, len[i] * sizeof(double), hipMemcpyDeviceToDevice);
    }
    int* vctr = (int*)dmal(((size_t)Tmax + 3) * sizeof(int));
    (void)hipMemset(vctr, 0, ((size_t)Tmax + 3) * sizeof(int));
    launch_chol_batch(cp.data(), n, vctr, s, nullptr, false, cu_share, nullptr);
    launch_chol_pair_steps(d, n, ctr, pair_tickets, s);
    (void)hipStreamSynchronize(s);
    int printed = 0;
    for (int i = 0; i < n; ++i) {
      std::vector<double> a(len[i]), b(len[i]);
      (void)hipMemcpy(a.data(), cp[i].S, len[i] * sizeof(double), hipMemcpyDeviceToHost);
      (void)hipMemcpy(b.data(), d[i].S, len[i] * sizeof(double), hipMemcpyDeviceToHost);
      const int ld = d[i].ld, T = d[i].T, B0 = d[i].b0 > 0 ? d[i].b0 : T, rows = B0 + d[i].nbr + 1;
      for (int c = 0; c < T; ++c)
        for (int r = c; r < rows; ++r) {
          if (c == T - 1 && r > B0 + d[i].nbr) continue;
          double worst = 0.0, ref = 0.0;
          for (int x = 0; x < NB; ++x)
            for (int y = 0; y < NB; ++y) {
              if (r == c) continue;
              const size_t o = (size_t)(c * NB + x) * ld + (size_t)r * NB + y;
              if (o >= len[i]) continue;
              const double dd = std::fabs(a[o] - b[o]);
              if (!(dd <= worst)) worst = dd;
              ref = std::max(ref, std::fabs(a[o]));
            }
          if (worst > 1e-9 * std::max(ref, 1.0) && printed < 40) {
            ++printed;
            fprintf(stderr, "[pair verify] system %d (T %d, nbr %d, b0 %d, kofs %d): tile (%d, %d) differs by %.3e (step kernels' max |value| %.3e)\n", i, T, d[i].nbr, d[i].b0,
                    d[i].kofs, r, c, worst, ref);
          }
        }
    }
    if (!printed) fprintf(stderr, "[pair verify] %d systems (Tmax %d): identical within 1e-9\n", n, Tmax);
    for (void* p : tmp) (void)hipFree(p);
    Tmax = Tmax > 0 ? -Tmax : 0;
  } else if (pair && chol_pair_supported(d, n)) { launch_chol_pair_steps(d, n, ctr, pair_tickets, s); Tmax = Tmax > 0 ? -Tmax : 0; }
  for (int k = 0; k < Tmax; ++k) {
    CholBatchArgs A{};
    A.n = n;
    long long nA2 = 0, nBt = 0;
    StepPlan pl[CHOL_STEP_BATCH_MAX];
    for (int i = 0; i < n; ++i) { pl[i] = plan_step(k, d[i].T, d[i].h_prof, d[i].nbr, d[i].h_bfirst, d[i].kofs); nA2 += 2 * pl[i].nA; nBt += pl[i].nB; }
    static const int env_share = getenv("SLIDE_CHOL_BSPLIT") ? atoi(getenv("SLIDE_CHOL_BSPLIT")) : -1;
    const int share = env_share >= 0 ? env_share : cu_share;
    const int a_split = (k > 0 && (nA2 + nBt) * 100 <= (long long)n_cu * share) ? 1 : 0;
    A.a_base[0] = A.b_base[0] = 0;
    for (int i = 0; i < n; ++i) {
      A.S[i] = d[i].S; A.ld[i] = d[i].ld; A.T[i] = d[i].T; A.Ld[i] = d[i].Ld; A.Winv[i] = d[i].Winv; A.status[i] = d[i].status;
      A.L32[i] = d[i].L32;
      A.TvA[i] = pl[i].TvA; A.TvB[i] = pl[i].TvB; A.TvX[i] = pl[i].TvX;
      A.nP[i] = pl[i].nP; A.g0[i] = pl[i].g0; A.g1[i] = pl[i].g1; A.nX[i] = pl[i].nX; A.a_split[i] = a_split;
      A.nbr[i] = d[i].nbr; A.nbA[i] = pl[i].nbA; A.nbB[i] = pl[i].nbB; A.nbX[i] = pl[i].nbX;
      A.B0[i] = d[i].b0 > 0 ? d[i].b0 : d[i].T;
      A.ord[i] = d[i].ord;
      A.a_base[i + 1] = A.a_base[i] + (int)(pl[i].nA << a_split);
      A.b_base[i + 1] = A.b_base[i] + (int)pl[i].nB;
    }
    const long long nAw = A.a_base[n], nB = A.b_base[n];
    const long long extra = nB < n_cu ? nB : n_cu;
    const long long free_cu = n_cu - nAw > 8 ? n_cu - nAw : 8;
    const int a_joins = nB > free_cu ? 1 : 0;
    static const int xcd_map = getenv("SLIDE_CHOL_XCD") ? atoi(getenv("SLIDE_CHOL_XCD")) : 0;
    hipLaunchKernelGGL(k_chol_step_batched, dim3((unsigned)(nAw + extra)), dim3(512), 0, s, A, k, k & ~1, ctr, a_joins, (xcd_map && n > 1) ? 1 : 0);
  }
  if (Tmax < 0) Tmax = -Tmax;
  if (after_steps) (void)hipEventRecord(after_steps, s);
  if (!solve) {
    ExtractArgs E{};
    E.n = n;
    for (int i = 0; i < n; ++i) {
      E.S[i] = d[i].S; E.ld[i] = d[i].ld; E.T[i] = d[i].T; E.Tr[i] = (d[i].b0 > 0 ? d[i].b0 : d[i].T) + d[i].nbr;
      E.yv[i] = d[i].yv; E.dp[i] = d[i].dp; E.status[i] = d[i].status;
    }
    if (Tmax > 0) hipLaunchKernelGGL(k_chol_extract_y_b, dim3((Tmax * NB + 255) / 256, n), dim3(256), 0, s, E);
    return;
  }
  launch_chain_tables(d, n, s);
  const double* yin[CHOL_BATCH_MAX];
  double* xout[CHOL_BATCH_MAX];
  for (int i = 0; i < n; ++i) {
    launch_chol_extract_y(d[i].S, d[i].ld, d[i].T, d[i].yv, d[i].dp, d[i].status, s, d[i].nbr);
    yin[i] = d[i].yv; xout[i] = d[i].dp;
  }
  if (chain_has_tables(d, n)) {
    launch_chain_batch(d, n, yin, xout, false, false, true, nullptr, s);
    return;
  }
  launch_chol_bwd_batch(d, n, s);
}
void launch_chol_bwd_batch(const CholSystem* d, int n, hipStream_t s) {
  if (n > BWD_BATCH_MAX) {
    for (int lo = 0; lo < n; lo += BWD_BATCH_MAX) launch_chol_bwd_batch(d + lo, n - lo < BWD_BATCH_MAX ? n - lo : BWD_BATCH_MAX, s);
    return;
  }
  BwdBatchArgs B{};
  B.n = n;
  B.base[0] = 0;
  int Tmax = 0;
  for (int i = 0; i < n; ++i) {
    B.S[i] = d[i].S; B.ld[i] = d[i].ld; B.T[i] = d[i].T; B.Ld[i] = d[i].Ld; B.Winv[i] = d[i].Winv; B.yv[i] = d[i].yv; B.dp[i] = d[i].dp;
    B.status[i] = d[i].status;
    B.prof[i] = d[i].prof;
    B.base[i + 1] = B.base[i] + d[i].T;
    Tmax = d[i].T > Tmax ? d[i].T : Tmax;
  }
  B.Tmax = Tmax;
  if (B.base[n] <= 0) return;
  hipLaunchKernelGGL(k_chol_bwd_chain_batched, dim3(B.base[n]), dim3(CHAIN_THREADS), 0, s, B);
}
void launch_chol_solve_bwd(const CholSystem& cs, hipStream_t s) {
  if (chain_has_tables(&cs, 1)) {
    launch_chain_tables(&cs, 1, s);
    const double* yin = cs.yv;
    double* xout = cs.dp;
    launch_chain_batch(&cs, 1, &yin, &xout, false, false, true, nullptr, s);
    return;
  }
  launch_chol_bwd_all(cs.S, cs.ld, cs.T, cs.Ld, cs.Winv, cs.yv, cs.dp, cs.status, cs.prof, s);
}
void launch_chol_bwd_all(const double* S, int ld, int T, const double* Ld, const double* Winv, double* yv, double* dp,
                         int* status, const int* prof, hipStream_t s, const double* wf_prev, double wf_thr, int wf_Tprev, int wf_lim) {
  if (wf_lim < 0 || wf_lim > wf_Tprev) wf_lim = wf_Tprev;
  if (wf_prev && wf_thr > 0.0 && wf_Tprev > 0 && wf_lim > 0)
    hipLaunchKernelGGL(k_chol_bwd_chain_wf, dim3(T), dim3(CHAIN_THREADS), 0, s, S, ld, T, Ld, Winv, yv, dp, status, prof, wf_prev, wf_thr, wf_Tprev, wf_lim);
  else
    hipLaunchKernelGGL(k_chol_bwd_chain, dim3(T), dim3(CHAIN_THREADS), 0, s, S, ld, T, Ld, Winv, yv, dp, status, prof);
}

struct CholLLPlan {
  LLSys* d_sys = nullptr; LLTask* d_tasks = nullptr; int* d_ints = nullptr;
  int n_sys = 0, n_tasks = 0, n_ints = 0, n_chain = 0, max_cols = 0;
};
CholLLPlan* chol_ll_plan_create(const CholSystem* d, int n, const int* const* h_ord, hipStream_t up) {
  static const int ll_mode = getenv("SLIDE_LL_MODE") ? atoi(getenv("SLIDE_LL_MODE")) : 0;
  std::vector<LLSys> sys(n);
  std::vector<std::vector<int>> first(n), bf(n), bphys(n), profv(n);
  size_t n_ints = 16;
  int Tmax = 0;
  for (int i = 0; i < n; ++i) {
    const CholSystem& c = d[i];
    LLSys& y = sys[i];
    y.S = c.S; y.Ld = c.Ld; y.Winv = c.Winv; y.status = c.status; y.ld = c.ld; y.T = c.T; y.B0 = c.b0 > 0 ? c.b0 : c.T; y.nbr = c.nbr;
    y.frows = y.B0 + y.nbr + 1;
    y.flags = reinterpret_cast<int*>(n_ints);
    n_ints += (size_t)y.T * y.frows;
    Tmax = c.T > Tmax ? c.T : Tmax;
    profv[i].resize(c.T);
    for (int k = 0; k < c.T; ++k) profv[i][k] = c.h_prof ? std::min(c.h_prof[k], c.T - 1) : c.T - 1;
    first[i].assign(c.T, 0);
    for (int r = 0, col = 0; r < c.T; ++r) {
      while (col < r && profv[i][col] < r) ++col;
      first[i][r] = col;
    }
    for (int j = 0; j < c.nbr; ++j) {
      long long f = c.h_bfirst ? (long long)c.h_bfirst[j] - c.kofs : 0;
      if (c.h_bfirst && j > 0 && c.h_bfirst[j] < c.h_bfirst[j - 1]) f = (long long)1 << 40;
      if (f >= c.T) break;
      bf[i].push_back(f < 0 ? 0 : (int)f);
      bphys[i].push_back(y.B0 + ((h_ord && h_ord[i]) ? h_ord[i][j] : j));
    }
  }
  std::vector<LLTask> tasks;
  int n_chain = 0;
  for (int k = 0; k < Tmax; ++k) {
    for (int pass = 0; pass < 2; ++pass)
      for (int i = 0; i < n; ++i) {
        const LLSys& y = sys[i];
        if (k >= y.T) continue;
        const int fk = first[i][k];
        std::vector<std::pair<int, int>> rows;
        for (int r = k + 1; r <= profv[i][k]; ++r) rows.emplace_back(r, std::max(first[i][r], fk));
        for (size_t j = 0; j < bf[i].size() && bf[i][j] <= k; ++j) rows.emplace_back(bphys[i][j], std::max(bf[i][j], fk));
        rows.emplace_back(y.B0 + y.nbr, fk);
        if (pass == 0) {
          tasks.push_back(LLTask{i, k, 0, rows[0].first, -1, fk, rows[0].second, k});
          ++n_chain;
        } else if (ll_mode == 1 || (ll_mode == 2 && (d[i].h_prof != nullptr || d[i].T <= 8))) {
          for (size_t r = 1; r < rows.size(); ++r) tasks.push_back(LLTask{i, k, 2, rows[r].first, -1, fk, rows[r].second, k});
        } else if (ll_mode == 3) {
          const size_t nband = (size_t)std::max(0, profv[i][k] - k);
          size_t r = 1;
          for (; r < rows.size() && r <= nband; ++r) tasks.push_back(LLTask{i, k, 2, rows[r].first, -1, fk, rows[r].second, k});
          for (; r < rows.size(); r += 2) {
            const bool two = r + 1 < rows.size();
            tasks.push_back(LLTask{i, k, 1, rows[r].first, two ? rows[r + 1].first : -1, fk, rows[r].second, two ? rows[r + 1].second : k});
          }
        } else {
          for (size_t r = 1; r < rows.size(); r += 2) {
            const bool two = r + 1 < rows.size();
            tasks.push_back(LLTask{i, k, 1, rows[r].first, two ? rows[r + 1].first : -1, fk, rows[r].second, two ? rows[r + 1].second : k});
          }
        }
      }
  }
  {
    std::vector<std::vector<char>> fl(n);
    for (int i = 0; i < n; ++i) fl[i].assign((size_t)sys[i].T * sys[i].frows, 0);
    auto need = [&](const LLTask& t, int c, int row) {
      const LLSys& y = sys[t.sys];
      if (c < 0 || c >= y.T || row < 0 || row >= y.frows || !fl[t.sys][(size_t)c * y.frows + row]) {
        fprintf(stderr, "slide_slam_amd: left-looking plan: task (system %d, column %d, kind %d, rows %d %d) waits for tile (%d, %d) that no earlier task produces\n",
                t.sys, t.k, t.kind, t.it0, t.it1, row, c);
        return false;
      }
      return true;
    };
    auto raise = [&](const LLTask& t, int row) {
      const LLSys& y = sys[t.sys];
      char& f = fl[t.sys][(size_t)t.k * y.frows + row];
      if (f) { fprintf(stderr, "slide_slam_amd: left-looking plan: tile (%d, %d) of system %d is produced twice\n", row, t.k, t.sys); return false; }
      f = 1;
      return true;
    };
    bool good = true;
    for (const LLTask& t : tasks) {
      if (t.kind != 1) {
        for (int c = t.clo_d; c < t.k && good; ++c) good = need(t, c, t.k);
        for (int c = t.clo0; c < t.k && good; ++c) good = need(t, c, t.it0) && need(t, c, t.k);
        good = good && t.clo_d >= 0 && t.clo0 >= t.clo_d && (t.kind != 0 || raise(t, t.k)) && raise(t, t.it0);
      } else {
        for (int sl = 0; sl < 2 && good; ++sl) {
          const int it = sl ? t.it1 : t.it0, clo = sl ? t.clo1 : t.clo0;
          if (it < 0) continue;
          for (int c = clo; c < t.k && good; ++c) good = need(t, c, it) && need(t, c, t.k);
          good = good && clo >= t.clo_d && need(t, t.k, t.k);
        }
        good = good && raise(t, t.it0) && (t.it1 < 0 || raise(t, t.it1));
      }
      if (!good) break;
    }
    if (!good) return nullptr;
  }
  CholLLPlan* p = new CholLLPlan();
  p->n_sys = n; p->n_tasks = (int)tasks.size(); p->n_ints = (int)n_ints; p->n_chain = n_chain; p->max_cols = Tmax;
  bool ok = hipMalloc(reinterpret_cast<void**>(&p->d_ints), n_ints * sizeof(int)) == hipSuccess &&
            hipMalloc(reinterpret_cast<void**>(&p->d_sys), std::max<size_t>(1, sys.size()) * sizeof(LLSys)) == hipSuccess &&
            hipMalloc(reinterpret_cast<void**>(&p->d_tasks), std::max<size_t>(1, tasks.size()) * sizeof(LLTask)) == hipSuccess;
  if (ok) {
    for (LLSys& y : sys) y.flags = p->d_ints + reinterpret_cast<size_t>(y.flags);
    ok = hipMemcpyAsync(p->d_sys, sys.data(), sys.size() * sizeof(LLSys), hipMemcpyHostToDevice, up) == hipSuccess &&
         hipMemcpyAsync(p->d_tasks, tasks.data(), tasks.size() * sizeof(LLTask), hipMemcpyHostToDevice, up) == hipSuccess &&
         hipMemsetAsync(p->d_ints, 0, n_ints * sizeof(int), up) == hipSuccess && hipStreamSynchronize(up) == hipSuccess;
  }
  if (!ok) { chol_ll_plan_destroy(p); return nullptr; }
  return p;
}
void chol_ll_plan_destroy(CholLLPlan* p) {
  if (!p) return;
  if (p->d_ints) (void)hipFree(p->d_ints);
  if (p->d_sys) (void)hipFree(p->d_sys);
  if (p->d_tasks) (void)hipFree(p->d_tasks);
  delete p;
}
int chol_ll_plan_tasks(const CholLLPlan* p) { return p ? p->n_tasks : 0; }
// ... 33 lines not shown
```

### slide_slam_amd/csrc/host_graph.hip

```cpp
#include <chrono>

#include "host_graph.hpp"

#include <algorithm>
#include <cmath>
#include <cstdio>
#include <cstdlib>
#include <map>
#include <unordered_map>

namespace sl {

static inline int lam_ks_cap(int nl) {
  const int tiles = (nl + 1) * nl;
  if (tiles <= 0) return 1;
  return tiles <= 32 ? 16 : std::max(1, std::min(16, 256 / tiles));
}

thread_local std::string g_last_error;
void thread_capture_mode_local() {
  thread_local bool done = false;
  if (done) return;
  hipStreamCaptureMode m = hipStreamCaptureModeThreadLocal;
  (void)hipThreadExchangeStreamCaptureMode(&m);
// ... 937 lines not shown
      SL_HIP(hipMemcpyAsync(d_sep_jobs2, codes2.data(), codes2.size() * sizeof(int), hipMemcpyHostToDevice, master)); SL_HIP(hipStreamSynchronize(master));
    }
    if (sep_ks > 1) {
      const size_t len = 2 * (size_t)(nb + 1) * nb * (sep_ks - 1) * NB * NB * sizeof(double);
      SL_HIP(hipMalloc(reinterpret_cast<void**>(&sep_scratch), len));
      SL_HIP(hipMemsetAsync(sep_scratch, 0, len, master)); SL_HIP(hipStreamSynchronize(master));
    }
    for (double** p : {&sep_top2, &sep_bord2}) if (*p) { SL_HIP(hipFree(*p)); *p = nullptr; }
    sep_ld2 = (Tt + sep_nl + 1) * NB;
    SL_HIP(hipMalloc(reinterpret_cast<void**>(&sep_top2), (size_t)sep_ld2 * Tt * NB * sizeof(double)));
    SL_HIP(hipMemsetAsync(sep_top2, 0, (size_t)sep_ld2 * Tt * NB * sizeof(double), master));
    if (sep_nl > 0) {
      const size_t nb2 = (size_t)(sep_nl + 1) * NB * sep_nl * NB;
      SL_HIP(hipMalloc(reinterpret_cast<void**>(&sep_bord2), nb2 * sizeof(double)));
      SL_HIP(hipMemsetAsync(sep_bord2, 0, nb2 * sizeof(double), master));
    }
    SL_HIP(hipStreamSynchronize(master));
    sep_mask_b = 0;
    unsigned mask_a = 0;
    for (int i = 0; i < n && i < 8; ++i) {
      const std::vector<int>& mp = graphs[i]->h_sep_map;
      for (int g = 0; g < TL * NB && g < sep_m && g < (int)mp.size(); ++g)
        if (mp[g] >= 0) { if (g < Ta * NB) mask_a |= 1u << i; else sep_mask_b |= 1u << i; }
    }
    if (mask_a & sep_mask_b) { g_last_error = "separator blocks: a robot holds coordinates of both leaves"; return SLIDE_ERR_INVALID; }
    std::vector<int> cover(h_sep_prof);
    for (int c = 0; c < TL; ++c) cover[c] = sep_Ts - 1;
    SL_HIP(hipMemcpyAsync(d_sep_prof, cover.data(), (size_t)sep_Ts * sizeof(int), hipMemcpyHostToDevice, master)); SL_HIP(hipStreamSynchronize(master));
  }
  {
    std::vector<int> tm(sep_Ts + sep_nl, 0);
    for (int i = 0; i < n && i < 32; ++i) {
      const std::vector<int>& mp = graphs[i]->h_sep_map;
      for (int g = 0; g < sep_m + sep_lam && g < (int)mp.size(); ++g)
        if (mp[g] >= 0) tm[g < sep_m ? g / NB : sep_Ts + (g - sep_m) / NB] |= 1 << i;
    }
    if (d_sep_tmask) { SL_HIP(hipStreamSynchronize(master)); SL_HIP(hipFree(d_sep_tmask)); d_sep_tmask = nullptr; }
    if (n <= 32 && !tm.empty()) {
      SL_HIP(hipMalloc(reinterpret_cast<void**>(&d_sep_tmask), tm.size() * sizeof(int)));
      SL_HIP(hipMemcpyAsync(d_sep_tmask, tm.data(), tm.size() * sizeof(int), hipMemcpyHostToDevice, master)); SL_HIP(hipStreamSynchronize(master));
    }
  }
  if (d_sep_off) { SL_HIP(hipFree(d_sep_off)); d_sep_off = nullptr; }
  SL_HIP(hipMalloc(reinterpret_cast<void**>(&d_sep_off), off.size() * sizeof(int)));
  SL_HIP(hipMemcpyAsync(d_sep_off, off.data(), off.size() * sizeof(int), hipMemcpyHostToDevice, master)); SL_HIP(hipStreamSynchronize(master));
  free_ll_sep_plans();
  if (chol_ll_enabled() && sep_Ts > 0) {
    const CholSystem top = sep_top_system();
    bool ok = true;
    if (chol_ll_mask() & 8) { ll_top = chol_ll_plan_create(&top, 1, nullptr, master); ok = ll_top != nullptr; }
    if (sep_dissected() && (chol_ll_mask() & 4)) {
      CholSystem lv[2];
      sep_leaf_systems(lv);
      ll_leaves = chol_ll_plan_create(lv, 2, nullptr, master);
      ll_leaf_own[0] = chol_ll_plan_create(&lv[0], 1, nullptr, master);
      ll_leaf_own[1] = chol_ll_plan_create(&lv[1], 1, nullptr, master);
      ok = ok && ll_leaves && ll_leaf_own[0] && ll_leaf_own[1];
    }
    if (!ok) { g_last_error = "exact joint step: the left-looking factorisation's tables could not be allocated"; return SLIDE_ERR_HIP; }
  }
  return SLIDE_OK;
}
int CholBatch::enqueue_ghost_refresh(double* const* d_bufs, int part) {
  const int ng = hG[0].n_gslots;
  for (int i = 1; i < n; ++i)
    if (hG[i].n_gslots != ng) { g_last_error = "batched pass: the graphs disagree on the ghost slots"; return SLIDE_ERR_INVALID; }
  if (ng <= 0) return SLIDE_OK;
  const bool whole = part < 0;
  if (whole) { launch_ghost_refresh_local(d_Gs, n, ng, master); return SLIDE_OK; }
  if (whole || part == 20) {
    launch_ghost_exchange_batched(d_Gs, n, ng, 0, d_bufs, master);
    launch_sum_bcast(d_bufs, n, 12 * ng, master);
  }
  if (whole || part == 0) {
    if (!whole) launch_bcast(d_bufs, n, 12 * ng, master);
    launch_ghost_exchange_batched(d_Gs, n, ng, 1, d_bufs, master);
  }
  return SLIDE_OK;
}
int CholBatch::enqueue_arrow(double* const* d_bufs, int part, hipEvent_t e0, hipEvent_t e1) {
  const bool whole = part < 0;
  if (part == 20) return enqueue_ghost_refresh(d_bufs, part);
  auto mark = [&](int i) { if (prof_ev[0]) (void)hipEventRecord(prof_ev[i], master); };
  const int* maps[CHOL_BATCH_HOST_MAX];
  double* xloc[CHOL_BATCH_HOST_MAX];
  for (int i = 0; i < n; ++i) { maps[i] = graphs[i]->d_sep_map.d; xloc[i] = graphs[i]->d_xloc.d; }
  const int ld_s = (sep_Ts + sep_nl + 1) * NB;
  const SepLayout Y = sep_layout();
  CholSystem lv[2];
  const int sTa = sep_leafT[0], sTL = sTa + sep_leafT[1], sTt = sep_Ts - sTL;
  if (sep_dissected()) sep_leaf_systems(lv);
  const bool owned = !whole && sep_dissected() && sep_owner >= 0;
  const int own = owned ? sep_owner : 0, own_t0 = own ? sTa : 0, own_T = sep_leafT[own];
  CholSystem top{};
  top.S = sepS + (owned ? (size_t)own_t0 * NB * ld_s : 0); top.ld = ld_s; top.T = owned ? own_T : sTL; top.b0 = sTL; top.nbr = sTt + sep_nl;
  top.bord = sepS + (size_t)sTL * NB * ld_s + (size_t)sTL * NB; top.ldb = ld_s;
  if (part == 1) {
    if (!owned) return SLIDE_OK;
    if (sep_leader) launch_sep_unpack(Y, master, sTL, sep_Ts + sep_nl);
    launch_sep_unpack(Y, master, own_t0, own_t0 + own_T);
    if (ll_leaf_own[own]) launch_chol_ll(ll_leaf_own[own], &lv[own], 1, master);
    else launch_chol_batch(&lv[own], 1, sep_ctr2, master, nullptr, false, 100, (chol_pair_mask() & 4) ? pair_tickets(10) : nullptr);
    if (sep_leader) {
      launch_border_syrk_jobs(&top, 1, d_sep_jobs, n_sep_jobs, 0, master, sep_scratch, sep_ks, sTt);
      if (sep_nl > 0) {
        CholSystem sl{};
        sl.S = sepS + (size_t)own_t0 * NB * ld_s; sl.ld = ld_s; sl.T = own_T; sl.b0 = sep_Ts; sl.nbr = sep_nl; sl.bord = sep_bord; sl.ldb = (sep_nl + 1) * NB;
        const int ks = std::max(1, std::min(lam_ks_cap(sep_nl), own_T / 2));
        launch_border_syrk(&sl, 1, master, lam_scratch, ks);
      }
      launch_sep_unpack(Y, master, sTL, sep_Ts + sep_nl, true);
    }
    return SLIDE_OK;
  }
  if (whole || part == 0) {
    launch_status_clear(d_Gs, n, master, sep_status, sep_nl > 0 ? lam_status : nullptr);
    const int rg = enqueue_ghost_refresh(d_bufs, part);
    if (rg != SLIDE_OK) return rg;
    launch_phase0_batched(d_Gs, hG.data(), n, d_bufs, master, false);
    launch_phase3_arrow_batched(d_Gs, hG.data(), n, master);
    {
      int nq[CHOL_BATCH_HOST_MAX];
      for (int i = 0; i < n; ++i) nq[i] = graphs[i]->n_sep_poses;
      launch_sep_extract_batched(d_Gs, hG.data(), n, nq, master);
    }
    if (e0) (void)hipEventRecord(e0, master);
    mark(0);
    if (ll_seg) {
      launch_chol_ll(ll_seg, seg_sys.data(), (int)seg_sys.size(), master);
      last_groups = 1;
      if (e1) (void)hipEventRecord(e1, master);
    } else {
      const int rc = factor_all(e1);
      if (rc != SLIDE_OK) return rc;
    }
    mark(1);
    if (n_syrk_jobs > 0) launch_border_syrk_jobs(sys.data(), n, d_syrk_jobs, n_syrk_jobs, syrk_lds_pad, master);
    else launch_border_syrk(sys.data(), n, master);
    mark(6);
    if (!l2_sys.empty()) {
      if (ll_l2) launch_chol_ll(ll_l2, l2_sys.data(), (int)l2_sys.size(), master);
      else launch_chol_batch(l2_sys.data(), (int)l2_sys.size(), d_ctr2, master, nullptr, false, 100, (chol_pair_mask() & 2) ? pair_tickets(8) : nullptr);
      if (n_l2_jobs > 0) launch_border_syrk_jobs(l2_sys.data(), (int)l2_sys.size(), d_l2_jobs, n_l2_jobs, 0, master);
      else launch_border_syrk(l2_sys.data(), (int)l2_sys.size(), master);
    }
    mark(2);
    static const bool env_canon = !(getenv("SLIDE_SEP_CANONICAL") && getenv("SLIDE_SEP_CANONICAL")[0] == '0');
    const bool canon = whole && sep_dissected() && env_canon && n <= 8;
    if (canon) launch_sep_gather(hG.data(), n, maps, Y, false, master, d_sep_tmask, sTL * NB, sep_mask_b, sep_top2, sep_ld2, sep_bord2);
    else launch_sep_gather(hG.data(), n, maps, Y, !whole, master, d_sep_tmask);
    mark(3);
  }
  if (whole || part == 2) {
    if (!whole && !owned) launch_sep_unpack(Y, master);
    if (owned) launch_sep_unpack(Y, master, sTL, sep_Ts + sep_nl);
    if (sep_dissected()) {
      const int TL = sTL, Tt = sTt;
      static const bool env_canon2 = !(getenv("SLIDE_SEP_CANONICAL") && getenv("SLIDE_SEP_CANONICAL")[0] == '0');
      const bool canon2 = whole && env_canon2 && n <= 8;
      if (!owned) {
        if (ll_leaves) launch_chol_ll(ll_leaves, lv, 2, master);
        else launch_chol_batch(lv, 2, sep_ctr2, master, nullptr, false, 100, (chol_pair_mask() & 4) ? pair_tickets(9) : nullptr);
        if (canon2) {
          CholSystem tp2[2] = {top, top};
          for (int hh = 0; hh < 2; ++hh) {
            tp2[hh].S = sepS + (size_t)(hh ? sTa : 0) * NB * ld_s; tp2[hh].T = sep_leafT[hh]; tp2[hh].b0 = sTL;
            if (hh) { tp2[hh].bord = sep_top2; tp2[hh].ldb = sep_ld2; }
          }
          CholSystem sl2[2];
          int ks_lam[2] = {1, 1};
          for (int hh = 0; hh < 2 && sep_nl > 0; ++hh) {
            CholSystem sl{};
            sl.S = sepS + (size_t)(hh ? sTa : 0) * NB * ld_s; sl.ld = ld_s; sl.T = sep_leafT[hh]; sl.b0 = sep_Ts; sl.nbr = sep_nl;
            sl.bord = hh ? sep_bord2 : sep_bord; sl.ldb = (sep_nl + 1) * NB;
            ks_lam[hh] = std::max(1, std::min(lam_ks_cap(sep_nl), sep_leafT[hh] / 2));
            sl2[hh] = sl;
          }
          if (sep_scratch && (sep_nl == 0 || (lam_scratch && d_lam_jobs2))) {
            launch_border_syrk_jobs(tp2, 2, d_sep_jobs2, n_sep_jobs2, 0, master, sep_scratch, sep_ks, Tt, nullptr, true);
            if (sep_nl > 0) launch_border_syrk_jobs(sl2, 2, d_lam_jobs2, n_lam_jobs2, 0, master, lam_scratch, 1, -1, ks_lam, true);
          } else {
            for (int hh = 0; hh < 2; ++hh) {
              launch_border_syrk_jobs(&tp2[hh], 1, d_sep_jobs, n_sep_jobs, 0, master, sep_scratch, sep_ks, Tt);
              if (sep_nl > 0) launch_border_syrk(&sl2[hh], 1, master, lam_scratch, ks_lam[hh]);
            }
            launch_sep_top_add(Y, sTL, sep_top2, sep_ld2, sep_bord2, master);
          }
        } else {
          launch_border_syrk_jobs(&top, 1, d_sep_jobs, n_sep_jobs, 0, master, sep_scratch, sep_ks, Tt);
        }
      }
      if (ll_top) {
        const CholSystem ts = sep_top_system();
        launch_chol_ll(ll_top, &ts, 1, master);
      } else if ((chol_pair_mask() & 8) && d_pair_tickets) {
        const CholSystem ts = sep_top_system();
        launch_chol_batch(&ts, 1, sep_ctr, master, nullptr, false, 100, pair_tickets(11));
      } else {
        double* St = sepS + (size_t)TL * NB * ld_s + (size_t)TL * NB;
        for (int k = 0; k < Tt; ++k)
          launch_chol_step(St, ld_s, k, Tt, sep_Ld + (size_t)(TL + k) * NB * NB, sep_Winv + (size_t)(TL + k) * 1024, sep_status, sep_ctr, nullptr, nullptr, master, sep_nl);
        launch_chol_extract_y(St, ld_s, Tt, sep_yv + (size_t)TL * NB, sep_dp + (size_t)TL * NB, sep_status, master, sep_nl);
      }
    } else if (ll_top) {
      const CholSystem ts = sep_top_system();
      launch_chol_ll(ll_top, &ts, 1, master);
    } else if ((chol_pair_mask() & 8) && d_pair_tickets) {
      const CholSystem ts = sep_top_system();
      launch_chol_batch(&ts, 1, sep_ctr, master, nullptr, false, 100, pair_tickets(11));
    } else {
      for (int k = 0; k < sep_Ts; ++k)
        launch_chol_step(sepS, ld_s, k, sep_Ts, sep_Ld + (size_t)k * NB * NB, sep_Winv + (size_t)k * 1024, sep_status, sep_ctr, nullptr,
                         sep_prof_on ? h_sep_prof.data() : nullptr, master, sep_nl);
      launch_chol_extract_y(sepS, ld_s, sep_Ts, sep_yv, sep_dp, sep_status, master, sep_nl);
    }
    if (sep_nl > 0) {
      CholSystem ss{};
      ss.S = sepS; ss.ld = ld_s; ss.T = sep_Ts; ss.yv = sep_yv; ss.nbr = sep_nl; ss.bord = sep_bord; ss.ldb = (sep_nl + 1) * NB; ss.bfirst = nullptr;
      CholSystem sr = ss;
      static const bool env_canon3 = !(getenv("SLIDE_SEP_CANONICAL") && getenv("SLIDE_SEP_CANONICAL")[0] == '0');
      if (owned || (whole && sep_dissected() && env_canon3 && n <= 8)) { sr.S = sepS + (size_t)sTL * NB * ld_s; sr.T = sTt; sr.b0 = sep_Ts; }
      const int ks = std::max(1, std::min(lam_ks_cap(sep_nl), sr.T / 2));
      launch_border_syrk(&sr, 1, master, lam_scratch, ks);
      launch_lam_prepare(sep_bord, sep_nl, sep_lam, lamS, master);
      const int ld_l = (sep_nl + 1) * NB;
      for (int k = 0; k < sep_nl; ++k)
        launch_chol_step(lamS, ld_l, k, sep_nl, lam_Ld + (size_t)k * NB * NB, lam_Winv + (size_t)k * 1024, lam_status, lam_ctr, nullptr, nullptr, master);
      launch_chol_extract_y(lamS, ld_l, sep_nl, lam_yv, lam_dp, lam_status, master);
      launch_chol_bwd_all(lamS, ld_l, sep_nl, lam_Ld, lam_Winv, lam_yv, lam_dp, lam_status, nullptr, master);
      const double* xl = lam_dp;
      if (!owned) launch_border_apply(&ss, 1, &xl, master);
      else {
        CholSystem ap2[2] = {ss, ss};
        ap2[0].S = sepS + (size_t)own_t0 * NB * ld_s; ap2[0].T = own_T; ap2[0].b0 = sep_Ts; ap2[0].yv = sep_yv + (size_t)own_t0 * NB;
        ap2[1].S = sepS + (size_t)sTL * NB * ld_s; ap2[1].T = sTt; ap2[1].b0 = sep_Ts; ap2[1].yv = sep_yv + (size_t)sTL * NB;
        const double* xl2[2] = {xl, xl};
        launch_border_apply(ap2, 2, xl2, master);
      }
    }
    if (sep_dissected()) {
      double* St = sepS + (size_t)sTL * NB * ld_s + (size_t)sTL * NB;
      launch_chol_bwd_all(St, ld_s, sTt, sep_Ld + (size_t)sTL * NB * NB, sep_Winv + (size_t)sTL * 1024, sep_yv + (size_t)sTL * NB, sep_dp + (size_t)sTL * NB,
                          sep_status, nullptr, master);
      launch_ints_clear(sep_status + 4, 1, master);
      CholSystem ap[2] = {lv[0], lv[1]};
      ap[0].nbr = ap[1].nbr = sTt;
      const double* xt[2] = {sep_dp + (size_t)sTL * NB, sep_dp + (size_t)sTL * NB};
      if (!owned) {
        launch_border_apply(ap, 2, xt, master);
        launch_chol_bwd_batch(lv, 2, master);
      } else {
        launch_border_apply(&ap[own], 1, xt, master);
        launch_chol_bwd_batch(&lv[own], 1, master);
      }
    } else {
      launch_chol_bwd_all(sepS, ld_s, sep_Ts, sep_Ld, sep_Winv, sep_yv, sep_dp, sep_status, sep_prof_on ? d_sep_prof : nullptr, master);
    }
    mark(4);
    launch_sep_xloc(n, maps, sep_m, sep_lam, sep_dp, lam_dp, xloc, master);
    if (!l2_sys.empty()) {
      const double* x2[CHOL_BATCH_HOST_MAX];
      for (size_t i = 0; i < l2_sys.size(); ++i) x2[i] = xloc[l2_graph[i]] + (size_t)hG[l2_graph[i]].nsep * NB;
      launch_border_apply(l2_sys.data(), (int)l2_sys.size(), x2, master);
      launch_chol_bwd_batch(l2_sys.data(), (int)l2_sys.size(), master);
      launch_ints_clear(l2_sys[0].status + 4, 1, master);
      {
        const double* src[CHOL_BATCH_HOST_MAX]; double* dst[CHOL_BATCH_HOST_MAX]; int cnt[CHOL_BATCH_HOST_MAX];
        for (size_t i = 0; i < l2_sys.size(); ++i) { src[i] = l2_sys[i].dp; dst[i] = xloc[l2_graph[i]]; cnt[i] = hG[l2_graph[i]].nsep * NB; }
        launch_copy_pairs(src, dst, cnt, (int)l2_sys.size(), master);
      }
    }
    launch_border_apply(sys.data(), n, xloc, master);
    launch_chol_bwd_batch(seg_sys.data(), (int)seg_sys.size(), master);
    launch_sep_pose_scatter_batched(d_Gs, hG.data(), n, xloc, master);
    launch_arrow_finish_batched(d_Gs, hG.data(), n, sep_dp, d_sep_off, master);
    launch_status_gather(d_Gs, n, d_status_all, master, sep_status, sep_nl > 0 ? lam_status : nullptr);
    mark(5);
  }
  return SLIDE_OK;
}
int CholBatch::profile_arrow(double* const* d_bufs, double* out6, int* n_sep_steps) {
  std::lock_guard<std::mutex> pl(pass_mtx);
  exact_serial = 0;
  bool same = false;
  int rc = begin_pass(d_bufs, &same);
  if (rc != SLIDE_OK) return rc;
  if (!(arrow && hG[0].n_slots > 0)) { g_last_error = "profile_arrow: the batch does not run exact joint passes"; return SLIDE_ERR_INVALID; }
  hipEvent_t start = nullptr;
  SL_HIP(hipEventCreate(&start));
  for (auto& e : prof_ev) SL_HIP(hipEventCreate(&e));
  (void)hipEventRecord(start, master);
  rc = enqueue_arrow(d_bufs, -1, nullptr, nullptr);
  const hipError_t es = hipStreamSynchronize(master);
  if (rc == SLIDE_OK && es == hipSuccess) {
    hipEvent_t seq[8] = {start, prof_ev[0], prof_ev[1], prof_ev[6], prof_ev[2], prof_ev[3], prof_ev[4], prof_ev[5]};
    float d[7] = {};
    for (int i = 0; i < 7; ++i)
      if (hipEventElapsedTime(&d[i], seq[i], seq[i + 1]) != hipSuccess) rc = SLIDE_ERR_HIP;
    out6[0] = d[0]; out6[1] = d[1] + d[3]; out6[2] = d[2]; out6[3] = d[4]; out6[4] = d[5]; out6[5] = d[6];
    if (n_sep_steps) *n_sep_steps = sep_Ts;
  } else if (rc == SLIDE_OK) rc = SLIDE_ERR_HIP;
  (void)hipEventDestroy(start);
  for (auto& e : prof_ev) { (void)hipEventDestroy(e); e = nullptr; }
  return rc == SLIDE_OK ? end_pass() : rc;
}
int CholBatch::enqueue_pass(double* const* d_bufs, hipEvent_t e0, hipEvent_t e1, int part) {
  static const bool batch_p3 = !(getenv("SLIDE_BATCH_PHASE3") && getenv("SLIDE_BATCH_PHASE3")[0] == '0');
  int rc = SLIDE_OK;
  auto each = [&](int phase) {
    if (hipEventRecord(ev_fork, master) != hipSuccess) { rc = SLIDE_ERR_HIP; return; }
    for (int i = 0; i < n && rc == SLIDE_OK; ++i) {
      HostGraph* g = graphs[i];
      if (hipStreamWaitEvent(g->stream, ev_fork, 0) != hipSuccess) { rc = SLIDE_ERR_HIP; break; }
      rc = g->enqueue_phase(phase, d_bufs[i]);
      if (rc == SLIDE_OK && (hipEventRecord(ev_in[i], g->stream) != hipSuccess || hipStreamWaitEvent(master, ev_in[i], 0) != hipSuccess))
        rc = SLIDE_ERR_HIP;
    }
  };
  const int n_slots = graphs[0]->G.n_slots;
  if (arrow && n_slots > 0) return enqueue_arrow(d_bufs, part, e0, e1);
  const bool whole = part < 0;
  const bool joint = pcg_iters > 0 && n_slots > 0;
  if (part == 20) return enqueue_ghost_refresh(d_bufs, part);
  if (whole || part == 0) {
    launch_status_clear(d_Gs, n, master);
    if ((rc = enqueue_ghost_refresh(d_bufs, part)) != SLIDE_OK) return rc;
    if (batch_p3) launch_phase0_batched(d_Gs, hG.data(), n, d_bufs, master);
    else each(0);
    if (rc == SLIDE_OK) launch_sum_bcast(d_bufs, n, 54 * n_slots, master);
  }
  if (whole || part == 1) {
    if (rc == SLIDE_OK && !whole) launch_bcast(d_bufs, n, 54 * n_slots, master);
    if (rc == SLIDE_OK) {
      if (batch_p3) launch_phase3_batched(d_Gs, hG.data(), n, d_bufs, master);
      else each(3);
    }
    if (rc == SLIDE_OK && joint && !batch_p3) rc = save_systems();
    if (rc == SLIDE_OK && e0) (void)hipEventRecord(e0, master);
    if (rc == SLIDE_OK) rc = factor_all(e1);
    if (rc == SLIDE_OK && joint) rc = enqueue_pcg_head(d_bufs);
  }
  if (joint) {
    for (int it = 0; it < pcg_iters && rc == SLIDE_OK; ++it) {
      const bool last = it == pcg_iters - 1;
      if (whole || (part == 10 && it == 0)) {
        if (!whole) launch_bcast(d_bufs, n, 9 * n_slots, master);
        rc = enqueue_pcg_mid(d_bufs, whole);
      }
      if (rc == SLIDE_OK && (whole || (part == 11 && it == 0 && !last) || (part == 12 && last))) {
        if (!whole) launch_bcast(d_bufs, n, 2, master);
        rc = enqueue_pcg_tail(d_bufs, last, whole);
      }
    }
  }
  if (whole || part == 1 || part == 12) {
    const bool here = whole || (part == 1 && !joint) || (part == 12 && joint);
    if (rc == SLIDE_OK && here) {
      if (batch_p3) launch_phase4_batched(d_Gs, hG.data(), n, d_bufs, master);
      else each(4);
    }
    if (rc == SLIDE_OK && here) launch_sum_bcast(d_bufs, n, 9 * n_slots, master);
  }
  if (whole || part == 2) {
    if (rc == SLIDE_OK && !whole) launch_bcast(d_bufs, n, 9 * n_slots, master);
    if (rc == SLIDE_OK) {
      if (batch_p3) launch_phase2_batched(d_Gs, hG.data(), n, d_bufs, master);
      else each(2);
    }
    if (rc == SLIDE_OK) launch_status_gather(d_Gs, n, d_status_all, master);
  }
  return rc;
}
static std::mutex g_capture_mtx;
int CholBatch::capture_pass(double* const* d_bufs, int part, hipGraphExec_t* exec) {
  std::lock_guard<std::mutex> cap(g_capture_mtx);
  if (*exec) { (void)hipGraphExecDestroy(*exec); *exec = nullptr; }
  hipGraph_t graph = nullptr;
  SL_HIP(hipStreamBeginCapture(master, hipStreamCaptureModeThreadLocal));
  g_last_error.clear();
  const int rc = enqueue_pass(d_bufs, nullptr, nullptr, part);
  std::string inner = g_last_error;
  {
    const hipError_t le = hipPeekAtLastError();
    if (le != hipSuccess) inner += std::string(inner.empty() ? "" : "; ") + "last launch error: " + hipGetErrorString(le);
  }
  const hipError_t e = hipStreamEndCapture(master, &graph);
  if (rc != SLIDE_OK || e != hipSuccess || graph == nullptr) {
    (void)hipGetLastError();
    if (graph) (void)hipGraphDestroy(graph);
    g_last_error = std::string("batched pass: stream capture failed (") + hipGetErrorString(e) + ", enqueue rc " + std::to_string(rc) + (inner.empty() ? "" : "; " + inner) + ")";
    return rc != SLIDE_OK ? rc : SLIDE_ERR_HIP;
  }
  const hipError_t ei = hipGraphInstantiate(exec, graph, nullptr, nullptr, 0);
  (void)hipGraphDestroy(graph);
  if (ei != hipSuccess) { *exec = nullptr; (void)hipGetLastError(); g_last_error = "batched pass: graph instantiation failed"; return SLIDE_ERR_HIP; }
  return SLIDE_OK;
}
int CholBatch::profile_pass(double* const* d_bufs, double* ms_steps, int* n_launches) {
  std::lock_guard<std::mutex> pl(pass_mtx);
  exact_serial = 0;
  {
    std::lock_guard<std::mutex> lk(mtx);
    for (int i = 0; i < n; ++i)
      if (!graphs[i] || !d_bufs[i]) { g_last_error = "batched pass: a slot of the batch is empty"; return SLIDE_ERR_INVALID; }
  }
  if (!master) {
    SL_HIP(hipStreamCreateWithFlags(&master, hipStreamNonBlocking));
    SL_HIP(hipEventCreateWithFlags(&ev_out, hipEventDisableTiming));
  }
  for (int i = 0; i < n; ++i) {
    HostGraph* g = graphs[i];
    std::lock_guard<std::mutex> gl(g->mtx);
    g->pred_valid = false; g->status_clean = false; g->cache_pose = -1;
    int rc = g->merge_pending();
    if (rc == SLIDE_OK) rc = g->upload_new();
    if (rc != SLIDE_OK) return rc;
    g->G.relin_thr = 0.0;
    SL_HIP(hipStreamSynchronize(g->stream));
  }
  int rc = prepare_pass();
  if (rc != SLIDE_OK) return rc;
  hipEvent_t e0 = nullptr, e1 = nullptr;
  SL_HIP(hipEventCreate(&e0));
  SL_HIP(hipEventCreate(&e1));
  rc = enqueue_pass(d_bufs, e0, e1, -1);
// ... 1417 lines not shown
```

### slide_slam_amd/csrc/kernels.hpp

```cpp
#pragma once
#include <hip/hip_runtime.h>
#include <stdint.h>

#include "graph_dev.hpp"

namespace sl {

void init_solver_kernels();
void launch_relin(const GraphDev& G, hipStream_t s);
void launch_linearize(const GraphDev& G, hipStream_t s);
void launch_landmark(const GraphDev& G, int mode, hipStream_t s);
void launch_pose(const GraphDev& G, hipStream_t s);
void launch_schur(const GraphDev& G, hipStream_t s);
void launch_backsub(const GraphDev& G, int mode, hipStream_t s);
void launch_shared_pack(const GraphDev& G, int what, double* buf, hipStream_t s);
void launch_shared_unpack(const GraphDev& G, int what, const double* buf, hipStream_t s);
void launch_estimate(const GraphDev& G, hipStream_t s);
void launch_estimate_predict(const GraphDev& G, hipStream_t s, int pose = -1, double* out17 = nullptr);
void launch_final_pack(const GraphDev& G, int pose, double* out16, hipStream_t s);
void launch_chi2(const GraphDev& G, double* out4, hipStream_t s);
void launch_pose_adj(const GraphDev& G, hipStream_t s);
void launch_scatter(const void* stage, unsigned desc_off, int nseg, hipStream_t s);
void launch_gather(void* stage, unsigned desc_off, int nseg, hipStream_t s);
void launch_gather_args(void* stage, const void* segs, int nseg, hipStream_t s);
void launch_sum_bcast(double* const* bufs, int n, int count, hipStream_t s);
void launch_bcast(double* const* bufs, int n, int count, hipStream_t s);
void launch_phase0_batched(const GraphDev* d, const GraphDev* h, int n, double* const* bufs, hipStream_t s, bool pack = true);
void launch_phase4_batched(const GraphDev* d, const GraphDev* h, int n, double* const* bufs, hipStream_t s);
void launch_phase2_batched(const GraphDev* d, const GraphDev* h, int n, double* const* bufs, hipStream_t s);
void launch_phase3_batched(const GraphDev* d, const GraphDev* h, int n, double* const* bufs, hipStream_t s);
void launch_ghost_exchange(const GraphDev& G, int what, double* buf, hipStream_t s);
void launch_ghost_exchange_batched(const GraphDev* d, int n, int n_gslots, int what, double* const* bufs, hipStream_t s);
void launch_border_assemble_batched(const GraphDev* d, const GraphDev* h, int n, hipStream_t s);
void launch_sep_extract_batched(const GraphDev* d, const GraphDev* h, int n, const int* n_sep_poses, hipStream_t s);
void launch_sep_pose_scatter_batched(const GraphDev* d, const GraphDev* h, int n, double* const* xloc, hipStream_t s);
struct SepLayout { double* sys; double* bord; double* packed; int Ts, nl, ms, lam; int gap[4]; int hTa, hTL; };
void launch_ghost_refresh_local(const GraphDev* d, int n, int n_gslots, hipStream_t s);
void launch_copy_pairs(const double* const* src, double* const* dst, const int* count, int n, hipStream_t s);
void launch_sep_gather(const GraphDev* h, int n, const int* const* maps, const SepLayout& Y, bool packed, hipStream_t s, const int* tmask = nullptr,
                       int split_col = -1, unsigned mask_b = 0, double* sys2 = nullptr, int ld2 = 0, double* bord2 = nullptr);
void launch_sep_top_add(const SepLayout& Y, int c0, const double* sys2, int ld2, const double* bord2, hipStream_t s);
void launch_sep_unpack(const SepLayout& Y, hipStream_t s, int c0 = 0, int c1 = -1, bool to_packed = false);
void launch_lam_prepare(const double* bord, int nl, int lam, double* out, hipStream_t s);
void launch_sep_xloc(int n, const int* const* maps, int ms, int lam, const double* xs, const double* xl, double* const* xloc, hipStream_t s);
void launch_arrow_finish_batched(const GraphDev* d, const GraphDev* h, int n, const double* xs, const int* sep_off, hipStream_t s);
void launch_phase3_arrow_batched(const GraphDev* d, const GraphDev* h, int n, hipStream_t s);

void launch_chol_step(double* S, int ld, int k, int T, double* Ld, double* Winv, int* status, int* ctr, float* L32, const int* h_prof, hipStream_t s, int nbr = 0);
void launch_chol_extract_y(const double* S, int ld, int T, double* yv, double* dp, int* status, hipStream_t s, int nbr = 0, int b0 = 0, double* prev = nullptr);
constexpr unsigned long long CHAIN_SENTINEL = 0x7FF8DEADBEEF0BADull;
struct CholSystem { double* S; int ld, T; double* Ld; double* Winv; double* yv; double* dp; int* status;
                    float* L32;
                    const int* h_prof;
                    const int* prof; const int* first;
                    double* ctab;
                    int nbr;
                    double* bord; int ldb;
                    const double* bord_src;
                    const int* bfirst;
                    const int* h_bfirst;
                    int b0;
                    int kofs;
                    const int* ord;
                    const int* segtab; };
constexpr int CHOL_STEP_BATCH_MAX = 32;
void launch_chol_batch(const CholSystem* d, int n, int* ctr, hipStream_t s, hipEvent_t after_steps = nullptr, bool solve = true, int cu_share = 100, int* pair_tickets = nullptr);
bool chol_pair_supported(const CholSystem* d, int n);
void launch_chol_bwd_batch(const CholSystem* d, int n, hipStream_t s);
struct CholLLPlan;
CholLLPlan* chol_ll_plan_create(const CholSystem* d, int n, const int* const* h_ord = nullptr, hipStream_t upload_stream = nullptr);
void chol_ll_plan_destroy(CholLLPlan* p);
int chol_ll_plan_tasks(const CholLLPlan* p);
int chol_ll_plan_columns(const CholLLPlan* p);
void launch_chol_ll(const CholLLPlan* p, const CholSystem* d, int n, hipStream_t s, int* trace = nullptr);
void launch_border_syrk(const CholSystem* d, int n, hipStream_t s, double* scratch = nullptr, int ks = 1);
void launch_border_syrk_jobs(const CholSystem* d, int n, const int* jobs, int njobs, int lds_pad, hipStream_t s, double* scratch = nullptr, int ks = 1, int jb_end = -1,
                             const int* ks_sys = nullptr, bool fuse_add = false);
void launch_border_apply(const CholSystem* d, int n, const double* const* xloc, hipStream_t s);
void launch_chain_batch(const CholSystem* d, int n, const double* const* in, double* const* out, bool fwd, bool f32, bool prepared,
                        double* const* next_out, hipStream_t s);
void launch_chain_tables(const CholSystem* d, int n, hipStream_t s);
void launch_chol_bwd_all(const double* S, int ld, int T, const double* Ld, const double* Winv, double* yv, double* dp, int* status, const int* prof, hipStream_t s,
                         const double* wf_prev = nullptr, double wf_thr = 0.0, int wf_Tprev = 0, int wf_lim = -1);
void launch_pose_covariance(const double* S, int ld, int T, const double* Ld, const double* Winv, double* Y, int row0, double* cov36,
                            hipStream_t s);
void launch_selected_inverse(const double* S, int ld, int T, const double* Ld, const double* Winv, const int* prof, const int* d_prof,
                             double* Sg, double* Z, hipStream_t s);
void launch_pose_blocks(const double* Sg, int ld, const int* poses, int n, double* out, hipStream_t s, const int* prow = nullptr);
void launch_landmark_covariances(const GraphDev& G, const double* Sg, int ld, const int* lids, int n, double* out, hipStream_t s,
                                 const int* prow = nullptr);
void launch_multi_solve(const double* S, int ld, int T, const double* Ld, const double* Winv, const int* prof, double* B, double* X,
                        int nrhs, hipStream_t s);
void launch_gram(const double* X, size_t ldx, int ncol, const int* rows, int nrows, double* M, hipStream_t s);
void launch_landmark_V(const GraphDev& G, const double* U, int nT, int ncol, const int* lids, int n, double* V, size_t ldv, hipStream_t s,
                       const int* prow = nullptr);
void launch_scatter(const int* rc, const double* val, int n, double* B, int nT, hipStream_t s);
constexpr int GAIN_MAX_STEPS = 64, GAIN_MAX_GRAMS = 4, GAIN_LDS_DIM = 96;
struct GainCandDev { int c0, nk, nsplit, pad; long long moff, poff, woff; };
int gain_gram_splits(int nk);
void launch_gram_blocks(const double* X, size_t ldx, const int* rows, int nrows, const GainCandDev* cand, int ncand, const int4* jobs,
                        int njobs, double* part, double* M, hipStream_t s);
int launch_woodbury_blocks(const double* U, size_t ldu, const GainCandDev* cand, int ncand, const int* jptr, const int* jrow,
                           const double* jval, const double* M, size_t msz, int nM, double* work, double* gains, int* flag, bool small,
                           bool big, hipStream_t s);
struct JSinvSys { const double* S; int ld, Tb; const double* B; int ldb; const double *Ld, *Winv, *Ld2, *Winv2; int neg0, col0;
                  double* Sg; double* Z; long long lds; };
constexpr int JSIG_ROBOTS_MAX = 8;
struct JSigGather { double* dst[JSIG_ROBOTS_MAX]; const int* map[JSIG_ROBOTS_MAX]; long long lds[JSIG_ROBOTS_MAX]; int o0[JSIG_ROBOTS_MAX], n[JSIG_ROBOTS_MAX];
                    const double* src; long long lds_src; };
void launch_jsinv_prep(const JSinvSys* d_sys, const int2* d_jobs, int njobs, int max_rows, const int* d_rp, const int* d_rows, hipStream_t s);
void launch_jsinv_step(const JSinvSys* d_sys, const int2* d_jobs, int njobs, int max_rows, const int* d_rp, const int* d_rows, hipStream_t s);
void launch_jsig_gather(const JSigGather& A, int n_robots, int max_n, hipStream_t s);
void launch_sym_blocks(const double* Sg, size_t ld, const int* row0, const int* dim, int n, double* out, hipStream_t s);
struct JMSum { const double* src[JSIG_ROBOTS_MAX]; double* dst; long long ld; };
void launch_jms_push(const JSinvSys* d_sys, const int4* d_jobs, int njobs, int max_list, const int* d_list, int ncol, bool bwd, hipStream_t s);
void launch_jms_pull(const JSinvSys* d_sys, const int4* d_jobs, int njobs, const int* d_list, int ncol, bool bwd, hipStream_t s);
void launch_jms_sum(const JMSum& A, const int* d_ptr, const int2* d_ent, int nrows, int ncol, hipStream_t s);
void launch_jms_gather(const JSigGather& A, int n_robots, int max_n, int ncol, hipStream_t s);
void launch_chol_solve_bwd(const CholSystem& cs, hipStream_t s);
int chol_factor_solve(double* S, int ld, int T, double* Ld, double* Winv, double* yv, double* dp, int* status, int* ctr, hipStream_t s);

enum { PCG_VEC_R = 0, PCG_VEC_U = 1, PCG_VEC_W = 2, PCG_VEC_P = 3, PCG_VEC_S = 4, PCG_VEC_X = 5, PCG_VEC_Y = 6, PCG_VEC_COUNT = 7 };
void launch_status_clear(const GraphDev* d, int n, hipStream_t s, int* x0 = nullptr, int* x1 = nullptr);
void launch_status_gather(const GraphDev* d, int n, int* out, hipStream_t s, const int* x0 = nullptr, const int* x1 = nullptr);
void launch_ints_clear(int* p, int n, hipStream_t s);
void launch_status_or(int* dst, const int* src, int n, hipStream_t s);
void launch_pcg_init(const GraphDev* d, const GraphDev* h, int n, hipStream_t s);
void launch_pcg_tl(const GraphDev* d, const GraphDev* h, int n, double* const* bufs, int vec, hipStream_t s);
void launch_pcg_matvec_dots(const GraphDev* d, const GraphDev* h, int n, double* const* bufs, int nsum, hipStream_t s);
void launch_pcg_update(const GraphDev* d, const GraphDev* h, int n, double* const* bufs, int nsum, hipStream_t s);
void launch_pcg_finish(const GraphDev* d, const GraphDev* h, int n, hipStream_t s);

struct AssocFrameDev {
  const float *cx, *cy, *cz;
  const double* model;
  const int32_t* label;
  int n;
  int K;
  int gate;
  int Kp, cached, staged;
  double thresh;
  double best_init;
  int label_gate;
  int is_cyl;
  const double* det;
  const int32_t* det_label;
  int n_det;
  double* det_world;
  int32_t* match_sub;
  int32_t* match_map;
  int32_t* submap;
  int32_t* n_sub;
};
bool assoc_plan(int n, int K, int gate, int model_stride, int* Kp, int* cached, int* staged, size_t* bytes);
void launch_assoc_frame(const AssocFrameDev* classes3, size_t lds_bytes , const double* pose12, hipStream_t s);
int launch_assoc_sweep(const float* cx, const float* cy, const float* cz, const double* model_xyz, const int32_t* label, int n_map,
                       const double* query_pos, const double* obs_xyz, const int32_t* obs_label, int n_query,
                       int n_obs, int K, double thresh, int32_t* out_map_idx, hipStream_t s);
void launch_map_refresh(double* cyl_model, int n_cyl, const int* cyl_lid, double* cube_xyz, int n_cube, const int* cube_lid,
                        double* ell_xyz, int n_ell, const int* ell_lid, const double* lm_est, hipStream_t s);
constexpr int ASSOC_MAX_K = 16384;
constexpr int ASSOC_LDS_BUDGET = 140 * 1024;

struct PlaceDev {
  const double* ref7; int nr;
  const double* qry7; int nq;
  const double* xs; const double* ys; const double* yaws;
  const int32_t* cell_x; const int32_t* cell_y;
  long long n_cells; int n_yaw;
  double thr_pos, thr_dim; int ignore_dim;
  int32_t* inliers;
  const double* rxy;
  const double* rdim;
  const double* qxy;
  const double* qdim;
  const int32_t* qrange;
  double v_crit;
};
void launch_place_sweep(const PlaceDev& P, hipStream_t s);
void launch_place_argmax(const int32_t* inliers, long long n, long long* best_idx, int32_t* best_val, hipStream_t s);
void launch_tri_prepare(const double* tri, int n, double* sdist, double* sxy, hipStream_t s);
void launch_tri_match(bool emit, const double* dm, const double* xm, int ntm, const double* dd, const double* xd, int ntd, double thr,
                      int* counts, const long long* offs, double* pts, double* diffs, hipStream_t s);
__device__ __forceinline__ int seg_of_row(const int* __restrict__ off, int n_seg, int row) {
  int lo = 0, hi = n_seg;
  while (hi - lo > 1) {
    const int mid = (lo + hi) >> 1;
    if (off[mid] <= row) lo = mid; else hi = mid;
  }
  return lo;
}
struct TriSeg { int tm0, td0, ntd; };
void launch_tri_match_seg(bool emit, const double* sd, const double* sx, const int* rowoff, const TriSeg* segs, int n_seg, int n_rows, double thr,
                          int* counts, const long long* offs, const long long* base, double* P1, double* P2, hipStream_t s);
void launch_seg_scan64(const int* cnt, const int* segoff, int n_seg, long long* out, long long* totals, hipStream_t s);
void launch_seg_scan_rowptr(const int* cnt, const int* segoff, int n_seg, int* rowptr, long long* totals, hipStream_t s);
struct ClqSolve {
  const int* rowptr; const int* col; const double* val; int n;
  const double* u0;
  double *u, *unew, *g, *gnew, *Mu, *Cu;
  double tol_u, tol_F, beta, eps;
  int maxin, maxol, maxls, rescale;
  double* out;
};
void launch_clq_solve_batch(const ClqSolve* d_jobs, int n_jobs, hipStream_t s);
bool launch_clq_solve_coop(const ClqSolve& A, double* priv, int* bar2, int n_wg, hipStream_t s);
void launch_clq_csr_count(const double* Mup, int n, int* rowcnt, hipStream_t s);
void launch_clq_csr_fill(const double* Mup, int n, const int* rowptr, int* col, double* val, hipStream_t s);
void launch_clq_solve(const int* rowptr, const int* col, const double* val, int n, const double* u0, double* work6n, double tol_u, double tol_F,
                      double beta, double eps, int maxin, int maxol, int maxls, int rescale, double* out4, hipStream_t s);
void launch_clipper_affinity(const double* D1, const double* D2, int dim, const int32_t* A, int m, double sigma, double eps,
                             double mindist, double affinityeps, double* M, hipStream_t s);
template <int DIM>
__device__ __forceinline__ double clipper_pair_score(int i0, int i1, int j0, int j1, const double* pi1, const double* pj1, const double* pi2,
                                                     const double* pj2, int dim, double sigma, double eps, double mindist, double affinityeps) {
  double out = 0.0;
  if (i0 != j0 && i1 != j1) {
    const int nd = DIM > 0 ? DIM : dim;
    double s1 = 0, s2 = 0;
    for (int k = 0; k < nd; ++k) {
      s1 += (pi1[k] - pj1[k]) * (pi1[k] - pj1[k]);
      s2 += (pi2[k] - pj2[k]) * (pi2[k] - pj2[k]);
    }
    const double l1 = sqrt(s1), l2 = sqrt(s2);
    if (!(mindist > 0 && (l1 < mindist || l2 < mindist))) {
      const double c = fabs(l1 - l2);
      const double scr = (c < eps) ? exp(-0.5 * c * c / (sigma * sigma)) : 0.0;
      if (scr > affinityeps) out = scr;
    }
  }
  return out;
// ... 12 lines not shown
```

Before: 3747.

## Fuse y-extraction into Cholesky step kernels and fold small clears/copies into neighbors

Result: slower. 3700 (-1.3%).

```diff
diff --git a/slide_slam_amd/csrc/capi.hip b/slide_slam_amd/csrc/capi.hip
--- a/slide_slam_amd/csrc/capi.hip
+++ b/slide_slam_amd/csrc/capi.hip
@@ -527,6 +527,75 @@
   return SLIDE_OK;
 }
 
+int slide_debug_step_extract(int n, const double* const* S_in, const int* ld, const int* T, const int* nbr, const int* const* prof, const int* const* bfirst,
+                             const int* const* ord, const int* b0, const int* kofs, int single, int guard, double guard_val, int solve,
+                             double* const* S_out, double* const* yv_out, double* const* dp_out, int* status_out, double* const* x_out) {
+  if (slide_device_check(-1) != SLIDE_OK) return SLIDE_ERR_HIP;
+  if (n < 1 || n > CHOL_STEP_BATCH_MAX || !S_in || !ld || !T || !nbr || guard < 0) return SLIDE_ERR_INVALID;
+  if (single && (n != 1 || (prof && prof[0]) || (b0 && b0[0] > 0) || (bfirst && bfirst[0]))) return SLIDE_ERR_INVALID;
+  Tmp Tm;
+  std::vector<CholSystem> sys(n);
+  int Tmax = 0;
+  for (int i = 0; i < n; ++i) {
+    const int Bi = b0 && b0[i] > 0 ? b0[i] : T[i];
+    if (T[i] < 1 || nbr[i] < 0 || ld[i] < (Bi + nbr[i] + 1) * NB) return SLIDE_ERR_INVALID;
+    Tmax = std::max(Tmax, T[i]);
+    const size_t nc = (size_t)T[i] * NB;
+    std::vector<double> fill(nc + guard, guard_val);
+    int st[8] = {0, 0, 0, 0, 77, 0, 0, 0};
+    CholSystem cs{};
+    cs.S = Tm.up(S_in[i], (size_t)ld[i] * nc); cs.ld = ld[i]; cs.T = T[i];
+    cs.Ld = Tm.up<double>(nullptr, nc * NB); cs.Winv = Tm.up<double>(nullptr, (size_t)T[i] * 1024);
+    cs.yv = Tm.up(fill.data(), fill.size()); cs.dp = Tm.up(fill.data(), fill.size());
+    cs.status = Tm.up(st, 8);
+    cs.ord = ord && ord[i] ? Tm.up(ord[i], (size_t)nbr[i]) : nullptr;
+    cs.prof = prof && prof[i] ? Tm.up(prof[i], (size_t)T[i]) : nullptr;
+    if (!cs.S || !cs.Ld || !cs.Winv || !cs.yv || !cs.dp || !cs.status || (ord && ord[i] && !cs.ord) || (prof && prof[i] && !cs.prof)) {
+      g_last_error = "hipMalloc/hipMemcpy failed";
+      return SLIDE_ERR_HIP;
+    }
+    SL_HIP(hipMemset(cs.Ld, 0, nc * NB * sizeof(double)));
+    cs.h_prof = prof ? prof[i] : nullptr; cs.nbr = nbr[i]; cs.h_bfirst = bfirst ? bfirst[i] : nullptr; cs.b0 = b0 ? b0[i] : 0; cs.kofs = kofs ? kofs[i] : 0;
+    sys[i] = cs;
+  }
+  int* d_ctr = Tm.up<int>(nullptr, (size_t)Tmax + 3);
+  if (!d_ctr) { g_last_error = "hipMalloc failed"; return SLIDE_ERR_HIP; }
+  SL_HIP(hipMemset(d_ctr, 0, ((size_t)Tmax + 3) * sizeof(int)));
+  if (single) {
+    const CholSystem& c = sys[0];
+    const bool fz = chol_pass_fused();
+    for (int k = 0; k < c.T; ++k)
+      launch_chol_step(c.S, c.ld, k, c.T, c.Ld + (size_t)k * NB * NB, c.Winv + (size_t)k * 1024, c.status, d_ctr, nullptr, nullptr, nullptr, c.nbr,
+                       fz ? c.yv : nullptr, fz ? c.dp : nullptr);
+    if (!fz) launch_chol_extract_y(c.S, c.ld, c.T, c.yv, c.dp, c.status, nullptr, c.nbr);
+  } else {
+    launch_chol_batch(sys.data(), n, d_ctr, nullptr, nullptr, false);
+  }
+  SL_HIP(hipDeviceSynchronize());
+  SL_HIP(hipGetLastError());
+  for (int i = 0; i < n; ++i) {
+    const size_t nc = (size_t)T[i] * NB;
+    if (S_out && S_out[i]) SL_HIP(hipMemcpy(S_out[i], sys[i].S, (size_t)ld[i] * nc * sizeof(double), hipMemcpyDeviceToHost));
+    if (yv_out && yv_out[i]) SL_HIP(hipMemcpy(yv_out[i], sys[i].yv, (nc + guard) * sizeof(double), hipMemcpyDeviceToHost));
+    if (dp_out && dp_out[i]) SL_HIP(hipMemcpy(dp_out[i], sys[i].dp, (nc + guard) * sizeof(double), hipMemcpyDeviceToHost));
+    if (status_out) SL_HIP(hipMemcpy(status_out + 8 * i, sys[i].status, 8 * sizeof(int), hipMemcpyDeviceToHost));
+  }
+  if (solve) {
+    if (single) launch_chol_bwd_all(sys[0].S, sys[0].ld, sys[0].T, sys[0].Ld, sys[0].Winv, sys[0].yv, sys[0].dp, sys[0].status, nullptr, nullptr);
+    else launch_chol_bwd_batch(sys.data(), n, nullptr);
+    SL_HIP(hipDeviceSynchronize());
+    SL_HIP(hipGetLastError());
+    for (int i = 0; i < n; ++i)
+      if (x_out && x_out[i]) SL_HIP(hipMemcpy(x_out[i], sys[i].dp, (size_t)T[i] * NB * sizeof(double), hipMemcpyDeviceToHost));
+    int st[8];
+    for (int i = 0; i < n; ++i) {
+      SL_HIP(hipMemcpy(st, sys[i].status, sizeof(st), hipMemcpyDeviceToHost));
+      if (st[1] & 2) { g_last_error = "backward substitution: a workgroup waited too long for the blocks it depends on"; return SLIDE_ERR_RUNTIME; }
+    }
+  }
+  return SLIDE_OK;
+}
+
 
 static int run_single_class(int cls_kind , int n_cur, const double* det_world, int det_stride,
                             const int32_t* label, int n_map, const float* cloud, const double* model, const int32_t* mlabel,
diff --git a/slide_slam_amd/csrc/chol_kernels.hip b/slide_slam_amd/csrc/chol_kernels.hip
--- a/slide_slam_amd/csrc/chol_kernels.hip
+++ b/slide_slam_amd/csrc/chol_kernels.hip
@@ -381,7 +381,7 @@
 }
 template <int NPAN, bool EARLY>
 __device__ __forceinline__ void panel_rows(double* __restrict__ S, int ld, int k, int it, int q, int gate, int lane, ALds& L, v4d (&Tq)[4],
-                                           const double (&tb)[16], float* __restrict__ L32t) {
+                                           const double (&tb)[16], float* __restrict__ L32t, double* __restrict__ ye, double* __restrict__ de) {
   const int lr = lane & 15, lk = lane >> 4;
   double* tcol = S + (size_t)(k * NB) * ld + (size_t)it * NB + 16 * q + lr;
   float* pcol = L32t ? L32t + lk * NB + 16 * q + lr : nullptr;
@@ -418,6 +418,13 @@
     xt[b] = x;
 #pragma unroll
     for (int r = 0; r < 4; ++r) tcol[(size_t)(16 * b + lk + 4 * r) * ld] = x[r];
+    if (ye && q == 0 && lr == 0) {
+#pragma unroll
+      for (int r = 0; r < 4; ++r) {
+        ye[16 * b + lk + 4 * r] = x[r];
+        de[16 * b + lk + 4 * r] = __longlong_as_double((long long)CHAIN_SENTINEL);
+      }
+    }
     if (pcol) {
 #pragma unroll
       for (int r = 0; r < 4; ++r) pcol[(16 * b + 4 * r) * NB] = (float)x[r];
@@ -448,7 +455,8 @@
 
 template <int NPAN>
 __device__ __forceinline__ void step_type_a_impl(double* __restrict__ S, int ld, int k, int ia, int it, int half, double* __restrict__ Ld,
-                                                 double* __restrict__ Winv, int* status, ALds& L, float* __restrict__ L32t) {
+                                                 double* __restrict__ Winv, int* status, ALds& L, float* __restrict__ L32t,
+                                                 double* __restrict__ ye, double* __restrict__ de) {
   const int tid = threadIdx.x, lane = tid & 63;
   const int wave = __builtin_amdgcn_readfirstlane(tid >> 6);
   const int lr = lane & 15, lk = lane >> 4;
@@ -484,7 +492,7 @@
     } else if (wave == 1) {
       v4d R1[2] = {R[0], R[1]};
       a_worker_wave<1, NPAN>(ia, Ld, Winv, L, lane, R1);
-      if (half < 0) panel_rows<NPAN, false>(S, ld, k, it, 0, 0, lane, L, Tq, tb, L32t);
+      if (half < 0) panel_rows<NPAN, false>(S, ld, k, it, 0, 0, lane, L, Tq, tb, L32t, ye, de);
     } else if (wave == 2) {
       v4d R2[3] = {R[0], R[1], R[2]};
       a_worker_wave<2, NPAN>(ia, Ld, Winv, L, lane, R2);
@@ -502,7 +510,7 @@
     double tb[16];
     if (rows) panel_load<NPAN>(S, ld, k, it, q, lr, lk, Tq, tb);
     __syncthreads();
-    if (rows) panel_rows<NPAN, true>(S, ld, k, it, q, wave - 4, lane, L, Tq, tb, L32t);
+    if (rows) panel_rows<NPAN, true>(S, ld, k, it, q, wave - 4, lane, L, Tq, tb, L32t, ye, de);
     STAMPW(14);
     __syncthreads();
     STAMP(1);
@@ -511,24 +519,29 @@
 }
 __device__ __forceinline__ void step_type_a(double* __restrict__ S, int ld, int k, int T, int TvA, int ia, int half, double* __restrict__ Ld,
                                             double* __restrict__ Winv, int* status, ALds& L, float* __restrict__ L32, int nbr, int nbA,
-                                            const int* __restrict__ ord = nullptr) {
+                                            const int* __restrict__ ord = nullptr, double* __restrict__ yv = nullptr, double* __restrict__ dp = nullptr) {
   const int vi = k + 1 + ia - TvA;
   const int it = vi < 0 ? k + 1 + ia : (vi < nbA ? T + (ord ? ord[vi] : vi) : T + nbr);
   float* L32t = (L32 && it < T) ? L32 + ((size_t)k * (T - 1) - (size_t)k * (k - 1) / 2 + (it - k - 1)) * (NB * NB) : nullptr;
-  if (k > 0) step_type_a_impl<1>(S, ld, k, ia, it, half, Ld, Winv, status, L, L32t);
-  else step_type_a_impl<0>(S, ld, k, ia, it, half, Ld, Winv, status, L, L32t);
+  const bool ex = yv && vi >= nbA && half <= 0;
+  double* ye = ex ? yv + (size_t)k * NB : nullptr;
+  double* de = ex ? dp + (size_t)k * NB : nullptr;
+  if (ex && k == 0 && threadIdx.x == 0) status[4] = 0;
+  if (k > 0) step_type_a_impl<1>(S, ld, k, ia, it, half, Ld, Winv, status, L, L32t, ye, de);
+  else step_type_a_impl<0>(S, ld, k, ia, it, half, Ld, Winv, status, L, L32t, ye, de);
 }
 
 __global__ __launch_bounds__(512) void k_chol_step(double* __restrict__ S, int ld, int k, int T, double* __restrict__ Ld,
                                                    double* __restrict__ Winv, int* status, int* __restrict__ ctr, int kb, int nP,
                                                    int g0, int g1, int nX, int a_joins, int a_split, float* __restrict__ L32,
-                                                   int TvA, int TvB, int TvX, int nbr, int nbA, int nbB, int nbX) {
+                                                   int TvA, int TvB, int TvX, int nbr, int nbA, int nbB, int nbX, double* __restrict__ yv,
+                                                   double* __restrict__ dp) {
   __shared__ ALds L;
   __shared__ int s_g;
   const int nA = (TvA - k + nbA) << a_split;
   if (blockIdx.x == 0 && threadIdx.x == 0) ctr[k + 1] = 0;
   if ((int)blockIdx.x < nA) {
-    step_type_a(S, ld, k, T, TvA, (int)blockIdx.x >> a_split, a_split ? (int)(blockIdx.x & 1) : -1, Ld, Winv, status, L, L32, nbr, nbA);
+    step_type_a(S, ld, k, T, TvA, (int)blockIdx.x >> a_split, a_split ? (int)(blockIdx.x & 1) : -1, Ld, Winv, status, L, L32, nbr, nbA, nullptr, yv, dp);
     if (!a_joins) return;
   }
   const int nR = g1 - g0, nItems = nR + nX;
@@ -550,18 +563,21 @@
 
 struct CholBatchArgs {
   int n;
-  double* S[CHOL_STEP_BATCH_MAX]; int ld[CHOL_STEP_BATCH_MAX]; int T[CHOL_STEP_BATCH_MAX];
+  double* S[CHOL_STEP_BATCH_MAX]; int ld[CHOL_STEP_BATCH_MAX];
   double* Ld[CHOL_STEP_BATCH_MAX]; double* Winv[CHOL_STEP_BATCH_MAX]; int* status[CHOL_STEP_BATCH_MAX];
   float* L32[CHOL_STEP_BATCH_MAX];
+  double* yv[CHOL_STEP_BATCH_MAX]; double* dp[CHOL_STEP_BATCH_MAX];
   int TvA[CHOL_STEP_BATCH_MAX], TvB[CHOL_STEP_BATCH_MAX], TvX[CHOL_STEP_BATCH_MAX];
-  int nP[CHOL_STEP_BATCH_MAX], g0[CHOL_STEP_BATCH_MAX], g1[CHOL_STEP_BATCH_MAX], nX[CHOL_STEP_BATCH_MAX], a_split[CHOL_STEP_BATCH_MAX];
-  int nbr[CHOL_STEP_BATCH_MAX];
-  int nbA[CHOL_STEP_BATCH_MAX], nbB[CHOL_STEP_BATCH_MAX], nbX[CHOL_STEP_BATCH_MAX];
+  int nP[CHOL_STEP_BATCH_MAX], g0[CHOL_STEP_BATCH_MAX], g1[CHOL_STEP_BATCH_MAX], nX[CHOL_STEP_BATCH_MAX];
+  unsigned char a_split[CHOL_STEP_BATCH_MAX];
+  unsigned short nbr[CHOL_STEP_BATCH_MAX];
+  unsigned short nbA[CHOL_STEP_BATCH_MAX], nbB[CHOL_STEP_BATCH_MAX], nbX[CHOL_STEP_BATCH_MAX];
   int B0[CHOL_STEP_BATCH_MAX];
   const int* ord[CHOL_STEP_BATCH_MAX];
   int a_base[CHOL_STEP_BATCH_MAX + 1];
   int b_base[CHOL_STEP_BATCH_MAX + 1];
 };
+static_assert(sizeof(CholBatchArgs) + 64 <= 4096, "k_chol_step_batched: kernel arguments beyond 4 KB");
 __device__ __forceinline__ int xcd_logical(int orig, int nwg) {
   const int q = nwg >> 3, r = nwg & 7, xcd = orig & 7;
   return (xcd < r ? xcd * (q + 1) : r * (q + 1) + (xcd - r) * q) + (orig >> 3);
@@ -577,7 +593,7 @@
     while (bid >= A.a_base[r + 1]) ++r;
     const int local = bid - A.a_base[r], sp = A.a_split[r];
     step_type_a(A.S[r], A.ld[r], k, A.B0[r], A.TvA[r], local >> sp, sp ? (local & 1) : -1, A.Ld[r] + (size_t)k * NB * NB,
-                A.Winv[r] + (size_t)k * 1024, A.status[r], L, A.L32[r], A.nbr[r], A.nbA[r], A.ord[r]);
+                A.Winv[r] + (size_t)k * 1024, A.status[r], L, A.L32[r], A.nbr[r], A.nbA[r], A.ord[r], A.yv[r], A.dp[r]);
     if (!a_joins) return;
   }
   const int nItems = A.b_base[A.n];
@@ -1787,7 +1803,7 @@
                                                const double* __restrict__ Winv, const double* __restrict__ yv, double* dp, int* status, int bidx,
                                                const float* __restrict__ L32, const int* __restrict__ prof,
                                                const double* __restrict__ wf_prev = nullptr, double wf_thr = 0.0, int wf_Tprev = 0,
-                                               int* wf_lds = nullptr, int wf_lim = 0) {
+                                               int* wf_lds = nullptr, int wf_lim = 0, double* __restrict__ dp2 = nullptr) {
   int dummy_state = 0;
   int& wf_state = WFIRE ? *wf_lds : dummy_state;
   auto& Ms = W.Ms; auto& Lo = W.Lo; auto& Ws = W.Ws; auto& tmp = W.tmp; auto& xs = W.xs; auto& ys = W.ys;
@@ -1946,6 +1962,7 @@
   x += __shfl_xor(x, 1);
   x += __shfl_xor(x, 2);
   if (worker && part == 0) __hip_atomic_store(dp + (size_t)c * NB + col, x, __ATOMIC_RELAXED, __HIP_MEMORY_SCOPE_AGENT);
+  if (dp2 && worker && part == 0) dp2[(size_t)c * NB + col] = x;
   CSTAMP(6);
 }
 __device__ __forceinline__ int bwd_ticket(int* ctr) {
@@ -1979,6 +1996,7 @@
   const double* S[BWD_BATCH_MAX]; int ld[BWD_BATCH_MAX]; int T[BWD_BATCH_MAX];
   const double* Ld[BWD_BATCH_MAX]; const double* Winv[BWD_BATCH_MAX]; const double* yv[BWD_BATCH_MAX]; double* dp[BWD_BATCH_MAX];
   int* status[BWD_BATCH_MAX];
+  double* dp2[BWD_BATCH_MAX];
   const int* prof[BWD_BATCH_MAX];
   int base[BWD_BATCH_MAX + 1];
   int Tmax;
@@ -1990,7 +2008,7 @@
     if (t >= A.n * A.Tmax) return;
     const int r = t % A.n, b = t / A.n;
     if (b >= A.T[r]) continue;
-    bwd_chain_body<false>(W, A.S[r], A.ld[r], A.T[r], A.Ld[r], A.Winv[r], A.yv[r], A.dp[r], A.status[r], b, nullptr, A.prof[r]);
+    bwd_chain_body<false>(W, A.S[r], A.ld[r], A.T[r], A.Ld[r], A.Winv[r], A.yv[r], A.dp[r], A.status[r], b, nullptr, A.prof[r], nullptr, 0.0, 0, nullptr, 0, A.dp2[r]);
     return;
   }
 }
@@ -2596,8 +2614,10 @@
   const double* S[CHOL_BATCH_MAX]; int ld[CHOL_BATCH_MAX]; int T[CHOL_BATCH_MAX]; int nbr[CHOL_BATCH_MAX]; int b0[CHOL_BATCH_MAX];
   double* yv[CHOL_BATCH_MAX]; const double* x[CHOL_BATCH_MAX];
   const int* segtab[CHOL_BATCH_MAX];
+  int* clr[2];
 };
 __global__ __launch_bounds__(256) void k_border_apply(BorderApplyArgs A) {
+  if (blockIdx.x == 0 && blockIdx.z == 0 && threadIdx.x < 2 && A.clr[threadIdx.x]) *A.clr[threadIdx.x] = 0;
   const int r = blockIdx.z;
   const int col = blockIdx.x * 4 + (threadIdx.x >> 6), lane = threadIdx.x & 63;
   if (col >= A.T[r] * NB) return;
@@ -2622,9 +2642,10 @@
   for (int m = 32; m >= 1; m >>= 1) acc += __shfl_xor(acc, m);
   if (lane == 0) A.yv[r][col] -= acc;
 }
-void launch_border_apply(const CholSystem* d, int n, const double* const* xloc, hipStream_t s) {
+void launch_border_apply(const CholSystem* d, int n, const double* const* xloc, hipStream_t s, int* clr0, int* clr1) {
   BorderApplyArgs A{};
   A.n = n;
+  A.clr[0] = clr0; A.clr[1] = clr1;
   int Tmax = 0;
   for (int i = 0; i < n; ++i) {
     A.S[i] = d[i].S; A.ld[i] = d[i].ld; A.T[i] = d[i].T; A.nbr[i] = d[i].nbr; A.yv[i] = d[i].yv; A.x[i] = xloc[i];
@@ -2632,7 +2653,9 @@
     A.segtab[i] = d[i].segtab;
     Tmax = d[i].T > Tmax ? d[i].T : Tmax;
   }
-  if (Tmax > 0) hipLaunchKernelGGL(k_border_apply, dim3(Tmax * NB / 4, 1, n), dim3(256), 0, s, A);
+  if (Tmax > 0) { hipLaunchKernelGGL(k_border_apply, dim3(Tmax * NB / 4, 1, n), dim3(256), 0, s, A); return; }
+  if (clr0) launch_ints_clear(clr0, 1, s);
+  if (clr1) launch_ints_clear(clr1, 1, s);
 }
 
 void launch_chol_bwd_all(const double* S, int ld, int T, const double* Ld, const double* Winv, double* yv, double* dp,
@@ -2682,8 +2705,12 @@
   p.nB = p.g1 - p.g0 + p.nX;
   return p;
 }
+bool chol_pass_fused() {
+  static const bool on = !(getenv("SLIDE_PASS_FUSED") && getenv("SLIDE_PASS_FUSED")[0] == '0');
+  return on;
+}
 void launch_chol_step(double* S, int ld, int k, int T, double* Ld, double* Winv, int* status, int* ctr, float* L32, const int* h_prof,
-                      hipStream_t s, int nbr) {
+                      hipStream_t s, int nbr, double* yv, double* dp) {
   const int n_cu = chol_n_cu();
   const StepPlan p = plan_step(k, T, h_prof, nbr, nullptr);
   const long long nA = p.nA, nB = p.nB;
@@ -2695,7 +2722,7 @@
   static const int join_mul = getenv("SLIDE_CHOL_JOIN") ? atoi(getenv("SLIDE_CHOL_JOIN")) : 1;
   const int a_joins = nB > join_mul * free_cu ? 1 : 0;
   hipLaunchKernelGGL(k_chol_step, dim3((unsigned)(nAw + extra)), dim3(512), 0, s, S, ld, k, T, Ld, Winv, status, ctr, p.kb, p.nP,
-                     p.g0, p.g1, p.nX, a_joins, a_split, L32, p.TvA, p.TvB, p.TvX, nbr, p.nbA, p.nbB, p.nbX);
+                     p.g0, p.g1, p.nX, a_joins, a_split, L32, p.TvA, p.TvB, p.TvX, nbr, p.nbA, p.nbB, p.nbX, yv, dp);
 }
 struct PairPlan { int ncols, Tv0, Tv1, nb0, nb1, TvB, nbB, nP; long long nA, nB; };
 static PairPlan plan_pair(int k, int T, const int* prof, int nbr, const int* bfirst, int kofs) {
@@ -2815,6 +2842,8 @@
     for (void* p : tmp) (void)hipFree(p);
     Tmax = Tmax > 0 ? -Tmax : 0;
   } else if (pair && chol_pair_supported(d, n)) { launch_chol_pair_steps(d, n, ctr, pair_tickets, s); Tmax = Tmax > 0 ? -Tmax : 0; }
+  bool fused = chol_pass_fused() && !solve && Tmax > 0;
+  for (int i = 0; i < n; ++i) fused = fused && d[i].T > 0 && d[i].yv && d[i].dp && d[i].nbr < 65536;
   for (int k = 0; k < Tmax; ++k) {
     CholBatchArgs A{};
     A.n = n;
@@ -2826,8 +2855,9 @@
     const int a_split = (k > 0 && (nA2 + nBt) * 100 <= (long long)n_cu * share) ? 1 : 0;
     A.a_base[0] = A.b_base[0] = 0;
     for (int i = 0; i < n; ++i) {
-      A.S[i] = d[i].S; A.ld[i] = d[i].ld; A.T[i] = d[i].T; A.Ld[i] = d[i].Ld; A.Winv[i] = d[i].Winv; A.status[i] = d[i].status;
+      A.S[i] = d[i].S; A.ld[i] = d[i].ld; A.Ld[i] = d[i].Ld; A.Winv[i] = d[i].Winv; A.status[i] = d[i].status;
       A.L32[i] = d[i].L32;
+      A.yv[i] = fused ? d[i].yv : nullptr; A.dp[i] = fused ? d[i].dp : nullptr;
       A.TvA[i] = pl[i].TvA; A.TvB[i] = pl[i].TvB; A.TvX[i] = pl[i].TvX;
       A.nP[i] = pl[i].nP; A.g0[i] = pl[i].g0; A.g1[i] = pl[i].g1; A.nX[i] = pl[i].nX; A.a_split[i] = a_split;
       A.nbr[i] = d[i].nbr; A.nbA[i] = pl[i].nbA; A.nbB[i] = pl[i].nbB; A.nbX[i] = pl[i].nbX;
@@ -2846,6 +2876,7 @@
   if (Tmax < 0) Tmax = -Tmax;
   if (after_steps) (void)hipEventRecord(after_steps, s);
   if (!solve) {
+    if (fused) return;
     ExtractArgs E{};
     E.n = n;
     for (int i = 0; i < n; ++i) {
@@ -2868,9 +2899,9 @@
   }
   launch_chol_bwd_batch(d, n, s);
 }
-void launch_chol_bwd_batch(const CholSystem* d, int n, hipStream_t s) {
+void launch_chol_bwd_batch(const CholSystem* d, int n, hipStream_t s, double* const* dp2) {
   if (n > BWD_BATCH_MAX) {
-    for (int lo = 0; lo < n; lo += BWD_BATCH_MAX) launch_chol_bwd_batch(d + lo, n - lo < BWD_BATCH_MAX ? n - lo : BWD_BATCH_MAX, s);
+    for (int lo = 0; lo < n; lo += BWD_BATCH_MAX) launch_chol_bwd_batch(d + lo, n - lo < BWD_BATCH_MAX ? n - lo : BWD_BATCH_MAX, s, dp2 ? dp2 + lo : nullptr);
     return;
   }
   BwdBatchArgs B{};
@@ -2880,6 +2911,7 @@
   for (int i = 0; i < n; ++i) {
     B.S[i] = d[i].S; B.ld[i] = d[i].ld; B.T[i] = d[i].T; B.Ld[i] = d[i].Ld; B.Winv[i] = d[i].Winv; B.yv[i] = d[i].yv; B.dp[i] = d[i].dp;
     B.status[i] = d[i].status;
+    B.dp2[i] = dp2 ? dp2[i] : nullptr;
     B.prof[i] = d[i].prof;
     B.base[i + 1] = B.base[i] + d[i].T;
     Tmax = d[i].T > Tmax ? d[i].T : Tmax;
diff --git a/slide_slam_amd/csrc/host_graph.hip b/slide_slam_amd/csrc/host_graph.hip
--- a/slide_slam_amd/csrc/host_graph.hip
+++ b/slide_slam_amd/csrc/host_graph.hip
@@ -1113,6 +1113,7 @@
     mark(3);
   }
   if (whole || part == 2) {
+    const bool fz = chol_pass_fused();
     if (!whole && !owned) launch_sep_unpack(Y, master);
     if (owned) launch_sep_unpack(Y, master, sTL, sep_Ts + sep_nl);
     if (sep_dissected()) {
@@ -1160,8 +1161,9 @@
       } else {
         double* St = sepS + (size_t)TL * NB * ld_s + (size_t)TL * NB;
         for (int k = 0; k < Tt; ++k)
-          launch_chol_step(St, ld_s, k, Tt, sep_Ld + (size_t)(TL + k) * NB * NB, sep_Winv + (size_t)(TL + k) * 1024, sep_status, sep_ctr, nullptr, nullptr, master, sep_nl);
-        launch_chol_extract_y(St, ld_s, Tt, sep_yv + (size_t)TL * NB, sep_dp + (size_t)TL * NB, sep_status, master, sep_nl);
+          launch_chol_step(St, ld_s, k, Tt, sep_Ld + (size_t)(TL + k) * NB * NB, sep_Winv + (size_t)(TL + k) * 1024, sep_status, sep_ctr, nullptr, nullptr, master, sep_nl,
+                           fz ? sep_yv + (size_t)TL * NB : nullptr, fz ? sep_dp + (size_t)TL * NB : nullptr);
+        if (!fz) launch_chol_extract_y(St, ld_s, Tt, sep_yv + (size_t)TL * NB, sep_dp + (size_t)TL * NB, sep_status, master, sep_nl);
       }
     } else if (ll_top) {
       const CholSystem ts = sep_top_system();
@@ -1172,8 +1174,8 @@
     } else {
       for (int k = 0; k < sep_Ts; ++k)
         launch_chol_step(sepS, ld_s, k, sep_Ts, sep_Ld + (size_t)k * NB * NB, sep_Winv + (size_t)k * 1024, sep_status, sep_ctr, nullptr,
-                         sep_prof_on ? h_sep_prof.data() : nullptr, master, sep_nl);
-      launch_chol_extract_y(sepS, ld_s, sep_Ts, sep_yv, sep_dp, sep_status, master, sep_nl);
+                         sep_prof_on ? h_sep_prof.data() : nullptr, master, sep_nl, fz ? sep_yv : nullptr, fz ? sep_dp : nullptr);
+      if (!fz) launch_chol_extract_y(sepS, ld_s, sep_Ts, sep_yv, sep_dp, sep_status, master, sep_nl);
     }
     if (sep_nl > 0) {
       CholSystem ss{};
@@ -1186,8 +1188,9 @@
       launch_lam_prepare(sep_bord, sep_nl, sep_lam, lamS, master);
       const int ld_l = (sep_nl + 1) * NB;
       for (int k = 0; k < sep_nl; ++k)
-        launch_chol_step(lamS, ld_l, k, sep_nl, lam_Ld + (size_t)k * NB * NB, lam_Winv + (size_t)k * 1024, lam_status, lam_ctr, nullptr, nullptr, master);
-      launch_chol_extract_y(lamS, ld_l, sep_nl, lam_yv, lam_dp, lam_status, master);
+        launch_chol_step(lamS, ld_l, k, sep_nl, lam_Ld + (size_t)k * NB * NB, lam_Winv + (size_t)k * 1024, lam_status, lam_ctr, nullptr, nullptr, master, 0,
+                         fz ? lam_yv : nullptr, fz ? lam_dp : nullptr);
+      if (!fz) launch_chol_extract_y(lamS, ld_l, sep_nl, lam_yv, lam_dp, lam_status, master);
       launch_chol_bwd_all(lamS, ld_l, sep_nl, lam_Ld, lam_Winv, lam_yv, lam_dp, lam_status, nullptr, master);
       const double* xl = lam_dp;
       if (!owned) launch_border_apply(&ss, 1, &xl, master);
@@ -1203,15 +1206,16 @@
       double* St = sepS + (size_t)sTL * NB * ld_s + (size_t)sTL * NB;
       launch_chol_bwd_all(St, ld_s, sTt, sep_Ld + (size_t)sTL * NB * NB, sep_Winv + (size_t)sTL * 1024, sep_yv + (size_t)sTL * NB, sep_dp + (size_t)sTL * NB,
                           sep_status, nullptr, master);
-      launch_ints_clear(sep_status + 4, 1, master);
+      int* const tick = fz ? sep_status + 4 : nullptr;
+      if (!fz) launch_ints_clear(sep_status + 4, 1, master);
       CholSystem ap[2] = {lv[0], lv[1]};
       ap[0].nbr = ap[1].nbr = sTt;
       const double* xt[2] = {sep_dp + (size_t)sTL * NB, sep_dp + (size_t)sTL * NB};
       if (!owned) {
-        launch_border_apply(ap, 2, xt, master);
+        launch_border_apply(ap, 2, xt, master, tick);
         launch_chol_bwd_batch(lv, 2, master);
       } else {
-        launch_border_apply(&ap[own], 1, xt, master);
+        launch_border_apply(&ap[own], 1, xt, master, tick);
         launch_chol_bwd_batch(&lv[own], 1, master);
       }
     } else {
@@ -1219,19 +1223,25 @@
     }
     mark(4);
     launch_sep_xloc(n, maps, sep_m, sep_lam, sep_dp, lam_dp, xloc, master);
+    int* tick2 = nullptr;
     if (!l2_sys.empty()) {
       const double* x2[CHOL_BATCH_HOST_MAX];
       for (size_t i = 0; i < l2_sys.size(); ++i) x2[i] = xloc[l2_graph[i]] + (size_t)hG[l2_graph[i]].nsep * NB;
       launch_border_apply(l2_sys.data(), (int)l2_sys.size(), x2, master);
-      launch_chol_bwd_batch(l2_sys.data(), (int)l2_sys.size(), master);
-      launch_ints_clear(l2_sys[0].status + 4, 1, master);
-      {
+      if (fz) {
+        double* head[CHOL_BATCH_HOST_MAX];
+        for (size_t i = 0; i < l2_sys.size(); ++i) head[i] = xloc[l2_graph[i]];
+        launch_chol_bwd_batch(l2_sys.data(), (int)l2_sys.size(), master, head);
+        tick2 = l2_sys[0].status + 4;
+      } else {
+        launch_chol_bwd_batch(l2_sys.data(), (int)l2_sys.size(), master);
+        launch_ints_clear(l2_sys[0].status + 4, 1, master);
         const double* src[CHOL_BATCH_HOST_MAX]; double* dst[CHOL_BATCH_HOST_MAX]; int cnt[CHOL_BATCH_HOST_MAX];
         for (size_t i = 0; i < l2_sys.size(); ++i) { src[i] = l2_sys[i].dp; dst[i] = xloc[l2_graph[i]]; cnt[i] = hG[l2_graph[i]].nsep * NB; }
         launch_copy_pairs(src, dst, cnt, (int)l2_sys.size(), master);
       }
     }
-    launch_border_apply(sys.data(), n, xloc, master);
+    launch_border_apply(sys.data(), n, xloc, master, tick2);
     launch_chol_bwd_batch(seg_sys.data(), (int)seg_sys.size(), master);
     launch_sep_pose_scatter_batched(d_Gs, hG.data(), n, xloc, master);
     launch_arrow_finish_batched(d_Gs, hG.data(), n, sep_dp, d_sep_off, master);
diff --git a/slide_slam_amd/csrc/kernels.hpp b/slide_slam_amd/csrc/kernels.hpp
--- a/slide_slam_amd/csrc/kernels.hpp
+++ b/slide_slam_amd/csrc/kernels.hpp
@@ -46,7 +46,9 @@
 void launch_arrow_finish_batched(const GraphDev* d, const GraphDev* h, int n, const double* xs, const int* sep_off, hipStream_t s);
 void launch_phase3_arrow_batched(const GraphDev* d, const GraphDev* h, int n, hipStream_t s);
 
-void launch_chol_step(double* S, int ld, int k, int T, double* Ld, double* Winv, int* status, int* ctr, float* L32, const int* h_prof, hipStream_t s, int nbr = 0);
+void launch_chol_step(double* S, int ld, int k, int T, double* Ld, double* Winv, int* status, int* ctr, float* L32, const int* h_prof, hipStream_t s, int nbr = 0,
+                      double* yv = nullptr, double* dp = nullptr);
+bool chol_pass_fused();
 void launch_chol_extract_y(const double* S, int ld, int T, double* yv, double* dp, int* status, hipStream_t s, int nbr = 0, int b0 = 0, double* prev = nullptr);
 constexpr unsigned long long CHAIN_SENTINEL = 0x7FF8DEADBEEF0BADull;
 struct CholSystem { double* S; int ld, T; double* Ld; double* Winv; double* yv; double* dp; int* status;
@@ -66,7 +68,7 @@
 constexpr int CHOL_STEP_BATCH_MAX = 32;
 void launch_chol_batch(const CholSystem* d, int n, int* ctr, hipStream_t s, hipEvent_t after_steps = nullptr, bool solve = true, int cu_share = 100, int* pair_tickets = nullptr);
 bool chol_pair_supported(const CholSystem* d, int n);
-void launch_chol_bwd_batch(const CholSystem* d, int n, hipStream_t s);
+void launch_chol_bwd_batch(const CholSystem* d, int n, hipStream_t s, double* const* dp2 = nullptr);
 struct CholLLPlan;
 CholLLPlan* chol_ll_plan_create(const CholSystem* d, int n, const int* const* h_ord = nullptr, hipStream_t upload_stream = nullptr);
 void chol_ll_plan_destroy(CholLLPlan* p);
@@ -76,7 +78,7 @@
 void launch_border_syrk(const CholSystem* d, int n, hipStream_t s, double* scratch = nullptr, int ks = 1);
 void launch_border_syrk_jobs(const CholSystem* d, int n, const int* jobs, int njobs, int lds_pad, hipStream_t s, double* scratch = nullptr, int ks = 1, int jb_end = -1,
                              const int* ks_sys = nullptr, bool fuse_add = false);
-void launch_border_apply(const CholSystem* d, int n, const double* const* xloc, hipStream_t s);
+void launch_border_apply(const CholSystem* d, int n, const double* const* xloc, hipStream_t s, int* clr0 = nullptr, int* clr1 = nullptr);
 void launch_chain_batch(const CholSystem* d, int n, const double* const* in, double* const* out, bool fwd, bool f32, bool prepared,
                         double* const* next_out, hipStream_t s);
 void launch_chain_tables(const CholSystem* d, int n, hipStream_t s);
```
